# NomaDamas/AutoRAG-Research

Hardware: AMD Instinct MI355X
Metric: queries/sec (higher is better)
Workload: dtype f32

## Files before the change

autorag_research_amd/_native.py:

```python

from __future__ import annotations

import ctypes
import os
from pathlib import Path

import numpy as np

_PKG_DIR = Path(__file__).resolve().parent
LIB_PATH = _PKG_DIR / "libmi355dr.so"

_lib: ctypes.CDLL | None = None

ABI_SYMBOLS = [
    "mi355dr_create", "mi355dr_destroy", "mi355dr_last_error", "mi355dr_version", "mi355dr_reserve",
    "mi355dr_add_rows", "mi355dr_add_rows_device", "mi355dr_size", "mi355dr_dim", "mi355dr_get_rows",
    "mi355dr_update_rows", "mi355dr_update_rows_device", "mi355dr_remove_rows", "mi355dr_live_rows", "mi355dr_compact",
    "mi355dr_search", "mi355dr_search_device", "mi355dr_search_device_async", "mi355dr_search_wait",
    "mi355dr_search_subset", "mi355dr_search_subset_device", "mi355dr_score_subset", "mi355dr_search_mmr", "mi355dr_search_mmr_device", "mi355dr_mmr_select", "mi355dr_merge_groups_device", "mi355dr_search_groups", "mi355dr_search_groups_device", "mi355dr_fuse_lists", "mi355dr_fuse_lists_device", "mi355dr_search_range", "mi355dr_search_range_device",
    "mi355dr_search_rows", "mi355dr_search_rows_device", "mi355dr_search_range_rows", "mi355dr_search_range_rows_device", "mi355dr_view_create", "mi355dr_add_multivec", "mi355dr_size_multivec",
    "mi355dr_search_maxsim", "mi355dr_search_maxsim_device", "mi355dr_search_maxsim_subset", "mi355dr_search_maxsim_subset_device", "mi355dr_maxsim_subset", "mi355dr_maxsim_subset_ex", "mi355dr_add_multivec_device", "mi355dr_gqr_refine", "mi355dr_gqr_refine_maxsim",
    "mi355dr_set_multivec", "mi355dr_set_multivec_device", "mi355dr_live_multivec",
    "mi355dr_add_sparse", "mi355dr_size_sparse", "mi355dr_sparse_df", "mi355dr_search_sparse", "mi355dr_search_sparse_device",
    "mi355dr_search_bm25", "mi355dr_search_bm25_device", "mi355dr_set_sparse", "mi355dr_remove_sparse", "mi355dr_live_sparse",
    "mi355dr_search_sparse_subset", "mi355dr_search_sparse_subset_device", "mi355dr_search_bm25_subset",
    "mi355dr_search_bm25_subset_device", "mi355dr_score_sparse_subset", "mi355dr_score_bm25_subset",
    "mi355dr_gqr_refine_scores", "mi355dr_merge_topk_device", "mi355dr_pack_topk_device",
    "mi355dr_merge_topk_packed_device", "mi355dr_comm_unique_id", "mi355dr_comm_init", "mi355dr_comm_world", "mi355dr_comm_count", "mi355dr_comm_init_custom",
    "mi355dr_search_sharded_device", "mi355dr_search_range_sharded_device", "mi355dr_search_rows_sharded_device",
    "mi355dr_search_range_rows_sharded_device", "mi355dr_search_mmr_sharded_device", "mi355dr_mmr_select_sharded",
    "mi355dr_search_sparse_sharded_device", "mi355dr_search_bm25_sharded_device", "mi355dr_search_sparse_subset_sharded_device",
    "mi355dr_search_bm25_subset_sharded_device", "mi355dr_score_sparse_subset_sharded", "mi355dr_score_bm25_subset_sharded",
    "mi355dr_collapse_lists", "mi355dr_collapse_lists_device", "mi355dr_search_collapsed", "mi355dr_search_collapsed_device",
    "mi355dr_search_collapsed_sharded_device",
    "mi355dr_combine_rows", "mi355dr_combine_rows_device", "mi355dr_search_examples", "mi355dr_search_examples_device",
    "mi355dr_search_feedback", "mi355dr_search_feedback_device",
    "mi355dr_set_option", "mi355dr_get_stat",
    "mi355dr_reset_stats", "mi355dr_timer_start", "mi355dr_timer_stop", "mi355dr_synchronize",
    "mi355dr_dev_alloc", "mi355dr_dev_free", "mi355dr_dev_upload", "mi355dr_dev_download",
    "mi355dr_diag_mfma_stream",
    "mi355dr_debug_screen_dense", "mi355dr_debug_screen_hits", "mi355dr_debug_screen_bound", "mi355dr_debug_i8_state", "mi355dr_debug_rescore",
    "mi355dr_debug_maxsim_pass", "mi355dr_debug_spec_m", "mi355dr_debug_spec_model",
]


ALLGATHER_FN = ctypes.CFUNCTYPE(ctypes.c_int, ctypes.c_void_p, ctypes.c_void_p, ctypes.c_size_t, ctypes.c_void_p, ctypes.c_void_p)


class FuseOpts(ctypes.Structure):

    _fields_ = [("method", ctypes.c_int), ("mode_1", ctypes.c_int), ("mode_2", ctypes.c_int), ("rrf_k", ctypes.c_int),
                ("fetch_k", ctypes.c_int), ("weight", ctypes.c_double), ("min_1", ctypes.c_double), ("min_2", ctypes.c_double)]


class NativeError(RuntimeError):

    def __init__(self, code: int, message: str):
        super().__init__(f"libmi355dr error {code}: {message}")
        self.code = code


def _preload_torch_hip_runtime() -> None:
    import importlib.util
    import sys

    if "torch" in sys.modules:
        return
    try:
        spec = importlib.util.find_spec("torch")
    except (ImportError, ValueError):
        return
    if spec is None or not spec.submodule_search_locations:
        return
    libdir = Path(list(spec.submodule_search_locations)[0]) / "lib"
    for name in ("libhsa-runtime64.so", "libamdhip64.so"):
        f = libdir / name
        if f.exists():
            try:
                ctypes.CDLL(str(f), mode=getattr(os, "RTLD_NOW", 2) | getattr(os, "RTLD_GLOBAL", 0x100))
            except OSError:
                return


def load() -> ctypes.CDLL:
    global _lib
    if _lib is not None:
        return _lib
    if not LIB_PATH.exists():
        raise ImportError(
            f"{LIB_PATH} not found: build it with `python -c 'import __graft_entry__ as g; g.build()'` "
            "(hipcc --offload-arch=gfx950).  There is no CPU fallback for the search path."
        )
    _preload_torch_hip_runtime()
    L = ctypes.CDLL(str(LIB_PATH), mode=getattr(os, "RTLD_NOW", 2))
    vp, c_int, i64 = ctypes.c_void_p, ctypes.c_int, ctypes.c_int64
    f32p, f64p = ctypes.POINTER(ctypes.c_float), ctypes.POINTER(ctypes.c_double)
    i64p, i32p = ctypes.POINTER(ctypes.c_int64), ctypes.POINTER(ctypes.c_int32)
    L.mi355dr_create.restype = c_int
    L.mi355dr_create.argtypes = [ctypes.POINTER(vp), c_int, c_int, c_int]
    L.mi355dr_destroy.restype = None
    L.mi355dr_destroy.argtypes = [vp]
    L.mi355dr_last_error.restype = ctypes.c_char_p
    L.mi355dr_last_error.argtypes = [vp]
    L.mi355dr_version.restype = c_int
    L.mi355dr_reserve.restype = c_int
    L.mi355dr_reserve.argtypes = [vp, i64]
    L.mi355dr_add_rows.restype = c_int
    L.mi355dr_add_rows.argtypes = [vp, f32p, i64]
    L.mi355dr_add_rows_device.restype = c_int
    L.mi355dr_add_rows_device.argtypes = [vp, vp, i64]
    L.mi355dr_update_rows.restype = c_int
    L.mi355dr_update_rows.argtypes = [vp, i64p, f32p, i64]
    L.mi355dr_update_rows_device.restype = c_int
    L.mi355dr_update_rows_device.argtypes = [vp, i64p, vp, i64]
    L.mi355dr_remove_rows.restype = c_int
    L.mi355dr_remove_rows.argtypes = [vp, i64p, i64]
    L.mi355dr_compact.restype = c_int
    L.mi355dr_compact.argtypes = [vp, i64p]
    L.mi355dr_live_rows.restype = i64
    L.mi355dr_live_rows.argtypes = [vp]
    L.mi355dr_size.restype = i64
    L.mi355dr_size.argtypes = [vp]
    L.mi355dr_dim.restype = c_int
    L.mi355dr_dim.argtypes = [vp]
    L.mi355dr_get_rows.restype = c_int
    L.mi355dr_get_rows.argtypes = [vp, i64, i64, f32p]
    L.mi355dr_search.restype = c_int
    L.mi355dr_search.argtypes = [vp, f32p, c_int, c_int, f64p, i64p]
    L.mi355dr_search_device.restype = c_int
    L.mi355dr_search_device.argtypes = [vp, vp, c_int, c_int, vp, vp, vp]
    L.mi355dr_search_device_async.restype = c_int
    L.mi355dr_search_device_async.argtypes = [vp, vp, c_int, c_int, vp, vp, vp, i64p]
    L.mi355dr_search_wait.restype = c_int
    L.mi355dr_search_wait.argtypes = [vp, i64]
    L.mi355dr_search_subset.restype = c_int
    L.mi355dr_search_subset.argtypes = [vp, f32p, c_int, c_int, i64p, i64, f64p, i64p]
    L.mi355dr_search_subset_device.restype = c_int
    L.mi355dr_search_subset_device.argtypes = [vp, vp, c_int, c_int, i64p, i64, vp, vp, vp]
    L.mi355dr_score_subset.restype = c_int
    L.mi355dr_score_subset.argtypes = [vp, f32p, c_int, i64p, c_int, f64p]
    L.mi355dr_search_mmr.restype = c_int
    L.mi355dr_search_mmr.argtypes = [vp, f32p, c_int, c_int, c_int, ctypes.c_double, f64p, i64p]
    L.mi355dr_search_mmr_device.restype = c_int
    L.mi355dr_search_mmr_device.argtypes = [vp, vp, c_int, c_int, c_int, ctypes.c_double, vp, vp, vp]
    L.mi355dr_mmr_select.restype = c_int
    L.mi355dr_mmr_select.argtypes = [vp, f32p, c_int, c_int, i64p, c_int, ctypes.c_double, f64p, i64p]
    L.mi355dr_merge_groups_device.restype = c_int
    L.mi355dr_merge_groups_device.argtypes = [vp, vp, vp, c_int, c_int, i32p, c_int, c_int, vp, vp, vp, vp]
    L.mi355dr_search_groups.restype = c_int
    L.mi355dr_search_groups.argtypes = [vp, f32p, i32p, c_int, c_int, c_int, f64p, i64p, i32p]
    L.mi355dr_search_groups_device.restype = c_int
    L.mi355dr_search_groups_device.argtypes = [vp, vp, i32p, c_int, c_int, c_int, vp, vp, vp, vp]
    fuse_p = ctypes.POINTER(FuseOpts)
    L.mi355dr_fuse_lists_device.restype = c_int
    L.mi355dr_fuse_lists_device.argtypes = [vp, vp, vp, c_int, vp, i64, vp, vp, c_int, vp, i64, c_int, c_int, fuse_p, vp, vp, vp, vp]
    L.mi355dr_fuse_lists.restype = c_int
    L.mi355dr_fuse_lists.argtypes = [vp, f64p, i64p, c_int, i64p, i64, f64p, i64p, c_int, i64p, i64, c_int, c_int, fuse_p, f64p, i64p, i32p]
    L.mi355dr_collapse_lists_device.restype = c_int
    L.mi355dr_collapse_lists_device.argtypes = [vp, vp, vp, c_int, c_int, vp, i64, c_int, c_int, vp, vp, vp, vp, vp, vp, vp]
    L.mi355dr_collapse_lists.restype = c_int
    L.mi355dr_collapse_lists.argtypes = [vp, f64p, i64p, c_int, c_int, i64p, i64, c_int, c_int, f64p, i64p, i64p, i32p, i32p, i32p]
    L.mi355dr_search_collapsed.restype = c_int
    L.mi355dr_search_collapsed.argtypes = [vp, f32p, c_int, c_int, c_int, i64p, i64, c_int, c_int, f64p, i64p, i64p, i32p, i32p]
    L.mi355dr_search_collapsed_device.restype = c_int
    L.mi355dr_search_collapsed_device.argtypes = [vp, vp, c_int, c_int, c_int, vp, i64, c_int, c_int, vp, vp, vp, vp, vp, vp]
    L.mi355dr_search_collapsed_sharded_device.restype = c_int
    L.mi355dr_search_collapsed_sharded_device.argtypes = list(L.mi355dr_search_collapsed_device.argtypes)
    L.mi355dr_search_range.restype = c_int
    L.mi355dr_search_range.argtypes = [vp, f32p, c_int, f64p, c_int, f64p, i64p, i64p]
    L.mi355dr_search_range_device.restype = c_int
    L.mi355dr_search_range_device.argtypes = [vp, vp, c_int, f64p, c_int, vp, vp, vp, vp]
    L.mi355dr_search_rows.restype = c_int
    L.mi355dr_search_rows.argtypes = [vp, i64p, c_int, c_int, c_int, f64p, i64p]
    L.mi355dr_search_rows_device.restype = c_int
    L.mi355dr_search_rows_device.argtypes = [vp, i64p, c_int, c_int, c_int, vp, vp, vp]
    L.mi355dr_search_range_rows.restype = c_int
    L.mi355dr_search_range_rows.argtypes = [vp, i64p, c_int, f64p, c_int, c_int, f64p, i64p, i64p]
    L.mi355dr_search_range_rows_device.restype = c_int
    L.mi355dr_search_range_rows_device.argtypes = [vp, i64p, c_int, f64p, c_int, c_int, vp, vp, vp, vp]
    dbl = ctypes.c_double
    L.mi355dr_combine_rows.restype = c_int
    L.mi355dr_combine_rows.argtypes = [vp, f32p, c_int, i64p, c_int, i64p, c_int, dbl, dbl, dbl, f32p, i32p]
    L.mi355dr_combine_rows_device.restype = c_int
    L.mi355dr_combine_rows_device.argtypes = [vp, vp, c_int, i64p, c_int, i64p, c_int, dbl, dbl, dbl, vp, vp, vp]
    L.mi355dr_search_examples.restype = c_int
    L.mi355dr_search_examples.argtypes = [vp, f32p, c_int, i64p, c_int, i64p, c_int, dbl, dbl, dbl, c_int, c_int, f64p, i64p]
    L.mi355dr_search_examples_device.restype = c_int
    L.mi355dr_search_examples_device.argtypes = [vp, vp, c_int, i64p, c_int, i64p, c_int, dbl, dbl, dbl, c_int, c_int, vp, vp, vp]
    L.mi355dr_search_feedback.restype = c_int
    L.mi355dr_search_feedback.argtypes = [vp, f32p, c_int, c_int, c_int, dbl, dbl, f64p, i64p]
    L.mi355dr_search_feedback_device.restype = c_int
    L.mi355dr_search_feedback_device.argtypes = [vp, vp, c_int, c_int, c_int, dbl, dbl, vp, vp, vp]
    L.mi355dr_view_create.restype = c_int
    L.mi355dr_view_create.argtypes = [vp, i64p, i64, i64p, i64, ctypes.POINTER(vp)]
    L.mi355dr_add_multivec.restype = c_int
    L.mi355dr_add_multivec.argtypes = [vp, f32p, i64p, i64]
    L.mi355dr_size_multivec.restype = i64
    L.mi355dr_size_multivec.argtypes = [vp]
    L.mi355dr_search_maxsim.restype = c_int
    L.mi355dr_search_maxsim.argtypes = [vp, f32p, i32p, c_int, c_int, f32p, i64p]
    L.mi355dr_search_maxsim_device.restype = c_int
    L.mi355dr_search_maxsim_device.argtypes = [vp, vp, i32p, c_int, c_int, vp, vp, vp]
    L.mi355dr_search_maxsim_subset.restype = c_int
    L.mi355dr_search_maxsim_subset.argtypes = [vp, f32p, i32p, c_int, c_int, i64p, i64, f32p, i64p]
    L.mi355dr_search_maxsim_subset_device.restype = c_int
    L.mi355dr_search_maxsim_subset_device.argtypes = [vp, vp, i32p, c_int, c_int, i64p, i64, vp, vp, vp]
    L.mi355dr_maxsim_subset.restype = c_int
    L.mi355dr_maxsim_subset.argtypes = [vp, f32p, i32p, c_int, i64p, c_int, f32p]
    L.mi355dr_maxsim_subset_ex.restype = c_int
    L.mi355dr_maxsim_subset_ex.argtypes = [vp, f32p, i32p, c_int, i64p, c_int, c_int, f32p]
    L.mi355dr_add_multivec_device.restype = c_int
    L.mi355dr_add_multivec_device.argtypes = [vp, vp, i64p, i64]
    L.mi355dr_set_multivec.restype = c_int
    L.mi355dr_set_multivec.argtypes = [vp, i64p, f32p, i64p, i64]
    L.mi355dr_set_multivec_device.restype = c_int
    L.mi355dr_set_multivec_device.argtypes = [vp, i64p, vp, i64p, i64]
    L.mi355dr_live_multivec.restype = i64
    L.mi355dr_live_multivec.argtypes = [vp]
    c_double = ctypes.c_double
    L.mi355dr_add_sparse.restype = c_int
    L.mi355dr_add_sparse.argtypes = [vp, i32p, i64p, i64]
    L.mi355dr_size_sparse.restype = i64
    L.mi355dr_size_sparse.argtypes = [vp]
    L.mi355dr_set_sparse.restype = c_int
    L.mi355dr_set_sparse.argtypes = [vp, i64p, i32p, i64p, i64]
    L.mi355dr_remove_sparse.restype = c_int
    L.mi355dr_remove_sparse.argtypes = [vp, i64p, i64]
    L.mi355dr_live_sparse.restype = i64
    L.mi355dr_live_sparse.argtypes = [vp]
    L.mi355dr_sparse_df.restype = c_int
    L.mi355dr_sparse_df.argtypes = [vp, i32p, i64, i64p]
    L.mi355dr_search_sparse.restype = c_int
    L.mi355dr_search_sparse.argtypes = [vp, i32p, f64p, i32p, c_int, c_int, c_double, c_double, f64p, i64p]
    L.mi355dr_search_sparse_device.restype = c_int
    L.mi355dr_search_sparse_device.argtypes = [vp, i32p, f64p, i32p, c_int, c_int, c_double, c_double, vp, vp, vp]
    L.mi355dr_search_bm25.restype = c_int
    L.mi355dr_search_bm25.argtypes = [vp, i32p, i32p, c_int, c_int, c_double, c_double, f64p, i64p]
    L.mi355dr_search_bm25_device.restype = c_int
    L.mi355dr_search_bm25_device.argtypes = [vp, i32p, i32p, c_int, c_int, c_double, c_double, vp, vp, vp]
    L.mi355dr_search_sparse_subset.restype = c_int
    L.mi355dr_search_sparse_subset.argtypes = [vp, i32p, f64p, i32p, c_int, c_int, c_double, c_double, i64p, i64, f64p, i64p]
    L.mi355dr_search_sparse_subset_device.restype = c_int
    L.mi355dr_search_sparse_subset_device.argtypes = [vp, i32p, f64p, i32p, c_int, c_int, c_double, c_double, i64p, i64, vp, vp, vp]
    L.mi355dr_search_bm25_subset.restype = c_int
    L.mi355dr_search_bm25_subset.argtypes = [vp, i32p, i32p, c_int, c_int, c_double, c_double, i64p, i64, f64p, i64p]
    L.mi355dr_search_bm25_subset_device.restype = c_int
    L.mi355dr_search_bm25_subset_device.argtypes = [vp, i32p, i32p, c_int, c_int, c_double, c_double, i64p, i64, vp, vp, vp]
    L.mi355dr_score_sparse_subset.restype = c_int
    L.mi355dr_score_sparse_subset.argtypes = [vp, i32p, f64p, i32p, c_int, c_double, c_double, i64p, c_int, f64p]
    L.mi355dr_score_bm25_subset.restype = c_int
    L.mi355dr_score_bm25_subset.argtypes = [vp, i32p, i32p, c_int, c_double, c_double, i64p, c_int, f64p]
    L.mi355dr_gqr_refine.restype = c_int
    L.mi355dr_gqr_refine.argtypes = [vp, f64p, c_int, i64p, c_int, f64p, c_int, c_double, c_double, c_double, f64p]
    L.mi355dr_gqr_refine_maxsim.restype = c_int
    L.mi355dr_gqr_refine_maxsim.argtypes = [vp, f64p, i32p, c_int, i64p, c_int, f64p, c_int, c_double, c_double, c_double,
                                            f64p]
    L.mi355dr_gqr_refine_scores.restype = c_int
    L.mi355dr_gqr_refine_scores.argtypes = [vp, f64p, i32p, c_int, c_int, f64p, c_int, c_double, c_double, c_double, f64p]
    L.mi355dr_merge_topk_device.restype = c_int
    L.mi355dr_merge_topk_device.argtypes = [vp, vp, vp, c_int, c_int, c_int, vp, vp, vp]
    L.mi355dr_pack_topk_device.restype = c_int
    L.mi355dr_pack_topk_device.argtypes = [vp, vp, vp, c_int, c_int, vp, vp]
    L.mi355dr_merge_topk_packed_device.restype = c_int
    L.mi355dr_merge_topk_packed_device.argtypes = [vp, vp, c_int, c_int, c_int, vp, vp, vp]
    L.mi355dr_comm_unique_id.restype = c_int
    L.mi355dr_comm_unique_id.argtypes = [vp, ctypes.c_size_t]
    L.mi355dr_comm_init.restype = c_int
    L.mi355dr_comm_init.argtypes = [vp, c_int, c_int, vp, ctypes.c_size_t]
    L.mi355dr_comm_init_custom.restype = c_int
    L.mi355dr_comm_init_custom.argtypes = [vp, c_int, c_int, ALLGATHER_FN, vp]
    L.mi355dr_comm_world.restype = c_int
    L.mi355dr_comm_world.argtypes = [vp]
    L.mi355dr_comm_count.restype = c_int
    L.mi355dr_comm_count.argtypes = [vp, ctypes.POINTER(c_int)]
    L.mi355dr_search_sharded_device.restype = c_int
    L.mi355dr_search_sharded_device.argtypes = [vp, vp, c_int, c_int, vp, vp, vp]
    L.mi355dr_search_range_sharded_device.restype = c_int
    L.mi355dr_search_range_sharded_device.argtypes = [vp, vp, c_int, f64p, c_int, vp, vp, vp, vp]
    L.mi355dr_search_rows_sharded_device.restype = c_int
    L.mi355dr_search_rows_sharded_device.argtypes = [vp, i64p, c_int, c_int, c_int, vp, vp, vp]
    L.mi355dr_search_range_rows_sharded_device.restype = c_int
    L.mi355dr_search_range_rows_sharded_device.argtypes = [vp, i64p, c_int, f64p, c_int, c_int, vp, vp, vp, vp]
    L.mi355dr_search_mmr_sharded_device.restype = c_int
    L.mi355dr_search_mmr_sharded_device.argtypes = [vp, vp, c_int, c_int, c_int, ctypes.c_double, vp, vp, vp]
    L.mi355dr_mmr_select_sharded.restype = c_int
    L.mi355dr_mmr_select_sharded.argtypes = [vp, f32p, c_int, c_int, i64p, c_int, ctypes.c_double, f64p, i64p]
    for local in ("search_sparse_device", "search_bm25_device", "search_sparse_subset_device", "search_bm25_subset_device",
                  "score_sparse_subset", "score_bm25_subset"):
        sharded = local.replace("_device", "_sharded_device") if local.endswith("_device") else local + "_sharded"
        fn = getattr(L, "mi355dr_" + sharded)
        fn.restype = c_int
        fn.argtypes = list(getattr(L, "mi355dr_" + local).argtypes)
    L.mi355dr_set_option.restype = c_int
    L.mi355dr_set_option.argtypes = [vp, ctypes.c_char_p, i64]
    L.mi355dr_get_stat.restype = c_int
    L.mi355dr_get_stat.argtypes = [vp, ctypes.c_char_p, i64p]
    L.mi355dr_reset_stats.restype = c_int
    L.mi355dr_reset_stats.argtypes = [vp]
    L.mi355dr_timer_start.restype = c_int
    L.mi355dr_timer_start.argtypes = [vp]
    L.mi355dr_timer_stop.restype = c_int
    L.mi355dr_timer_stop.argtypes = [vp, f64p]
    L.mi355dr_synchronize.restype = c_int
    L.mi355dr_synchronize.argtypes = [vp]
    L.mi355dr_dev_alloc.restype = c_int
    L.mi355dr_dev_alloc.argtypes = [vp, ctypes.c_size_t, ctypes.POINTER(vp)]
    L.mi355dr_dev_free.restype = c_int
    L.mi355dr_dev_free.argtypes = [vp, vp]
    L.mi355dr_dev_upload.restype = c_int
    L.mi355dr_dev_upload.argtypes = [vp, vp, vp, ctypes.c_size_t]
    L.mi355dr_dev_download.restype = c_int
    L.mi355dr_dev_download.argtypes = [vp, vp, vp, ctypes.c_size_t]
    L.mi355dr_debug_screen_dense.restype = c_int
    L.mi355dr_debug_screen_dense.argtypes = [vp, f32p, c_int, i64, i64, f32p]
    L.mi355dr_debug_screen_hits.restype = c_int
    L.mi355dr_debug_screen_hits.argtypes = [vp, f32p, c_int, i64, i64, f32p, c_int, ctypes.POINTER(c_int), i32p, f32p,
                                            ctypes.POINTER(c_int), ctypes.POINTER(c_int)]
    L.mi355dr_debug_screen_bound.restype = c_int
    L.mi355dr_debug_screen_bound.argtypes = [vp, f32p, c_int, f32p]
    L.mi355dr_debug_i8_state.restype = c_int
    L.mi355dr_debug_i8_state.argtypes = [vp, f32p, c_int, f32p, f32p, i64, i64, f32p, f32p]
    L.mi355dr_debug_rescore.restype = c_int
    L.mi355dr_debug_rescore.argtypes = [vp, f32p, c_int, i32p, i64p, i64, f32p, f64p]
    L.mi355dr_debug_spec_m.restype = c_int
    L.mi355dr_debug_spec_m.argtypes = [c_int]
    L.mi355dr_debug_spec_model.restype = c_int
    L.mi355dr_debug_spec_model.argtypes = [vp, f32p, c_int, c_int, f32p, f32p, f32p, ctypes.POINTER(ctypes.c_double),
                                           ctypes.POINTER(ctypes.c_int64), ctypes.POINTER(c_int), ctypes.POINTER(c_int)]
    L.mi355dr_debug_maxsim_pass.restype = c_int
    L.mi355dr_debug_maxsim_pass.argtypes = [vp, f32p, i32p, c_int, c_int, i64p, i64, c_int, ctypes.POINTER(c_int), f32p, f32p, i32p,
                                            ctypes.POINTER(c_int), f32p, ctypes.POINTER(c_int), ctypes.POINTER(c_int)]
    L.mi355dr_diag_mfma_stream.restype = c_int
    L.mi355dr_diag_mfma_stream.argtypes = [c_int, c_int, ctypes.c_double, ctypes.POINTER(ctypes.c_double)]
    _lib = L
    return L


def diag_mfma_stream(device: int, fmt: str, seconds: float) -> float:
    out = ctypes.c_double(0.0)
    rc = load().mi355dr_diag_mfma_stream(int(device), {"i8": 0, "bf16": 1}[fmt], float(seconds), ctypes.byref(out))
    if rc != 0:
        raise NativeError(rc, "mi355dr_diag_mfma_stream failed")
    return float(out.value)


def check(handle, rc: int) -> None:
    if rc != 0:
        msg = load().mi355dr_last_error(handle)
        raise NativeError(rc, msg.decode("utf-8", "replace") if msg else "")


def f32c(a) -> np.ndarray:
    return np.ascontiguousarray(a, dtype=np.float32)


def ptr(a: np.ndarray, ct):
    return a.ctypes.data_as(ctypes.POINTER(ct))
```

autorag_research_amd/csrc/index.h:

```cpp
#pragma once
#include <climits>
#include <hip/hip_runtime.h>

#include <algorithm>
#include <cmath>
#include <cstdio>
#include <cstring>
#include <mutex>
#include <string>
#include <vector>

#include "dev_common.h"
#include "mi355dr.h"

namespace mi355 {
template <class T, bool Pinned = false>
struct DevBuf {
    T* p = nullptr;
    size_t bytes = 0;
    DevBuf() = default;
    DevBuf(const DevBuf&) = delete;
    DevBuf& operator=(const DevBuf&) = delete;
    ~DevBuf() { release(); }
    void release() {
        if (p) (void)(Pinned ? hipHostFree(p) : hipFree(p));
        p = nullptr;
        bytes = 0;
    }
    hipError_t grow(size_t want) {
        if (want <= bytes) return hipSuccess;
        void* q = nullptr;
        const hipError_t e = Pinned ? hipHostMalloc(&q, want) : hipMalloc(&q, want);
        if (e != hipSuccess) return e;
        release();
        p = (T*)q;
        bytes = want;
        return hipSuccess;
    }
    void swap(DevBuf& o) {
        std::swap(p, o.p);
        std::swap(bytes, o.bytes);
    }
    operator T*() const { return p; }
};
template <class T>
using HostBuf = DevBuf<T, true>;

struct Event {
    hipEvent_t e = nullptr;
    Event() = default;
    Event(const Event&) = delete;
    Event& operator=(const Event&) = delete;
    ~Event() {
        if (e) (void)hipEventDestroy(e);
    }
    hipError_t create(unsigned flags = hipEventDefault) { return e ? hipSuccess : hipEventCreateWithFlags(&e, flags); }
    operator hipEvent_t() const { return e; }
};

struct EventPair {
    hipEvent_t a, b;
    int big;
};
struct EventPairs {
    std::vector<EventPair> v;
    ~EventPairs() {
        for (auto& p : v) {
            (void)hipEventDestroy(p.a);
            (void)hipEventDestroy(p.b);
        }
    }
};
struct MultiVecStore;
struct SparseStore;
struct Pass {
    int k = 0;
    int level = 0;
    bool screening = false;
    bool i8 = false;
    bool wide = false;
    int cap = 0;
    bool speculative = false;
    bool spec_eligible = false;
    int spec_m = 0;
    const char* refused = nullptr;
};
struct Pending {
    bool active = false;
    Event done;
    HostBuf<int> status_host;
    hipStream_t stream = nullptr;
    const float* q_dev = nullptr;
    int B = 0;
    Pass pass;
    double* out_dist = nullptr;
    int64_t* out_rows = nullptr;
};
struct RetryBufs {
    DevBuf<float> q;
    DevBuf<double> dist;
    DevBuf<int64_t> rows;
    DevBuf<int> map;
};
constexpr int kPendingRing = 4;

template <class... Bufs>
hipError_t grow_each(size_t n, Bufs&... bufs) {
    hipError_t e = hipSuccess;
    (void)(((e = bufs.grow(n * sizeof(*bufs.p))) == hipSuccess) && ...);
    return e;
}
struct MmrBufs {
    DevBuf<double> cand_dist;
    DevBuf<int64_t> cand_rows;
    DevBuf<unsigned long long> pairs_dev;
    hipError_t reserve(size_t nb, size_t stride) {
        hipError_t e = grow_each(nb * stride, cand_dist, cand_rows);
        if (!e) e = grow_each(1, pairs_dev);
        return e;
    }
};
struct GroupBufs {
    DevBuf<int32_t> offsets, count;
    DevBuf<double> cand_dist, out_dist;
    DevBuf<int64_t> cand_rows, out_rows;
    hipError_t reserve(size_t G, size_t S, size_t fetch_k, size_t k, bool host) {
        hipError_t e = grow_each(G + 1, offsets);
        if (!e) e = grow_each(S * fetch_k, cand_dist, cand_rows);
        if (!e && host) e = grow_each(G * k, out_dist, out_rows);
        if (!e && host) e = grow_each(G, count);
        return e;
    }
};
struct FuseBufs {
    DevBuf<double> vals[2], out_vals;
    DevBuf<int64_t> ids[2], map[2], out_ids;
    DevBuf<int32_t> count;
    hipError_t reserve(size_t B, const int* w, const int64_t* map_len, size_t k_out) {
        hipError_t e = hipSuccess;
        for (int l = 0; l < 2 && !e; ++l) {
            e = grow_each(B * (size_t)w[l], vals[l], ids[l]);
            if (!e) e = grow_each((size_t)map_len[l], map[l]);
        }
        if (!e) e = grow_each(B * k_out, out_vals, out_ids);
        if (!e) e = grow_each(B, count);
        return e;
    }
};
struct CollapseBufs {
    DevBuf<double> vals, out_vals, cand_dist;
    DevBuf<int64_t> ids, keys, out_ids, out_keys, cand_rows;
    DevBuf<int32_t> out_pos, count, entries, lines, kept;
    DevBuf<float> q_all, q_sub;
    hipError_t reserve_lists(size_t B, size_t w, size_t keys_len, size_t k_out) {
        hipError_t e = grow_each(B * w, vals, ids);
        if (!e) e = grow_each(keys_len, keys);
        if (!e) e = grow_each(B * k_out, out_vals, out_ids, out_keys, out_pos);
        if (!e) e = grow_each(B, count, entries);
        return e;
    }
    hipError_t reserve_search(size_t nb, size_t max_fetch, size_t k, size_t dim, size_t host_keys_len, bool host) {
        hipError_t e = grow_each(nb * max_fetch, cand_dist, cand_rows);
        if (!e) e = grow_each(nb * dim, q_sub);
        if (!e) e = grow_each(nb, lines, kept, entries);
        if (!e && host) e = grow_each(nb * dim, q_all);
        if (!e && host) e = grow_each(host_keys_len, keys);
        if (!e && host) e = grow_each(nb * k, out_keys);
        return e;
    }
    size_t bytes() const {
        return vals.bytes + out_vals.bytes + cand_dist.bytes + ids.bytes + keys.bytes + out_ids.bytes + out_keys.bytes +
               cand_rows.bytes + out_pos.bytes + count.bytes + entries.bytes + lines.bytes + kept.bytes + q_all.bytes +
               q_sub.bytes;
    }
};
struct RangeBufs {
    DevBuf<uint64_t> key, rkey;
    DevBuf<int32_t> row, xfrom;
    DevBuf<unsigned long long> count, stat;
    DevBuf<double> radius, fb_dist;
    DevBuf<int> redo, flag, fb_map;
    DevBuf<int64_t> fb_rows;
    DevBuf<float> fb_q;
    int collect_lds = 0;
    hipError_t reserve(size_t nb, size_t R, size_t m, size_t pairs, size_t dim) {
        hipError_t e = grow_each(nb * R, key, row);
        if (!e) e = grow_each(nb, count, rkey, xfrom, radius, flag, fb_map);
        if (!e) e = grow_each(2, stat);
        if (!e) e = grow_each(2 + 2 * pairs, redo);
        if (!e) e = grow_each(nb * dim, fb_q);
        if (!e) e = grow_each(nb * m, fb_dist, fb_rows);
        return e;
    }
};
struct RowQueryBufs {
    DevBuf<int64_t> ids, pair_row, cand_rows, cand_count;
    DevBuf<float> q, self_dot;
    DevBuf<int> valid;
    DevBuf<int32_t> pair_q;
    DevBuf<double> cand_dist, self_dist, radius;
    DevBuf<unsigned long long> skipped_dev;
    hipError_t reserve(size_t nb, size_t stride, size_t dim, bool range) {
        hipError_t e = grow_each(nb, ids, valid, pair_q, pair_row);
        if (!e) e = grow_each(nb * dim, q);
        if (!e) e = grow_each(nb * stride, cand_dist, cand_rows);
        if (!e) e = grow_each(1, skipped_dev);
        if (!e && range) e = grow_each(nb, cand_count, self_dot, self_dist, radius);
        return e;
    }
};
struct ExampleBufs {
    DevBuf<int64_t> pos, neg, cand_rows;
    DevBuf<float> q, base;
    DevBuf<int> valid;
    DevBuf<double> cand_dist;
    DevBuf<unsigned long long> counters;
    hipError_t reserve(size_t nb, size_t mp, size_t mn, size_t stride, size_t dim, bool own_base) {
        hipError_t e = grow_each(nb * mp, pos);
        if (!e) e = grow_each(nb * mn, neg);
        if (!e) e = grow_each(nb, valid);
        if (!e) e = grow_each(nb * dim, q);
        if (!e) e = grow_each(nb * stride, cand_dist, cand_rows);
        if (!e) e = grow_each(2, counters);
        if (!e && own_base) e = grow_each(nb * dim, base);
        return e;
    }
};
struct ShardBufs {
    DevBuf<int64_t> send, recv;
    DevBuf<float> stage, stage_all;
    DevBuf<unsigned long long> local_skipped;
};
}

struct mi355dr_index {
    int device = 0, dim = 0, dpad = 0, metric = 0;
    hipStream_t stream = nullptr;
    std::mutex mu;
    std::string err;
    mi355dr_index() = default;
    ~mi355dr_index() {
        if (stream) (void)hipStreamDestroy(stream);
    }

    int64_t n = 0, cap_rows = 0;
    mi355::DevBuf<float> rows;
    mi355::DevBuf<uint16_t> shadow;
    mi355::DevBuf<float> nrm2;
    mi355::DevBuf<int32_t> irr_rows;
    mi355::DevBuf<int> irr_count;
    int irr_n = 0;
    mi355::DevBuf<unsigned> n2max_dev;
    float cmax = 0.0f;
    mi355::DevBuf<unsigned> bf16_res2_dev;
    float bf16_ec = 0.00390625f;
    int dpad8 = 0;
    mi355::DevBuf<int8_t> shadow8;
    mi355::DevBuf<uint8_t> flag8;
    mi355::DevBuf<mi355::I8Group> grp8;
    mi355::DevBuf<int32_t> irr8_rows;
    mi355::DevBuf<int> irr8_count;
    int irr8_n = 0;
    mi355::DevBuf<int> dead_count;
    int64_t dead_n = 0;

    bool qstate_ready = false;
    mi355::QueryState st{};
    mi355::DevBuf<void> st_mem[sizeof(mi355::QueryState) / sizeof(void*)];
    mi355::DevBuf<float> qdev;
    mi355::DevBuf<int32_t> cand_row;
    mi355::DevBuf<float> cand_val;
    mi355::DevBuf<int> qlist_dev;
    int* status_or_dev = nullptr;
    mi355::HostBuf<int> status_host;
    mi355::DevBuf<double> out_dist_dev;
    mi355::DevBuf<int64_t> out_rows_dev;
    mi355::DevBuf<int64_t> out_count_dev;
    mi355::DevBuf<unsigned long long> stat_dev;
    mi355::DevBuf<int> prune_skip;
    mi355::DevBuf<int32_t> subset_ids;
    mi355::MmrBufs mmr;
    mi355::GroupBufs grp;
    mi355::FuseBufs fuse;
    mi355::CollapseBufs clp;
    mi355::RangeBufs rng;
    mi355::RowQueryBufs rowq;
    mi355::ExampleBufs exq;
    mi355::ShardBufs shd;
    bool is_view = false;
    mi355::DevBuf<int64_t> view_row_map;
    mi355::DevBuf<int64_t> view_doc_map;
    int64_t view_rows = 0, view_docs = 0;
    int prune_parity = 0;

    int path = 0;
    int screen_dtype = 0;
    int i8_backoff = 0, i8_probation = 0;
    int speculate = 1;
    int64_t spec_min_rows = (int64_t)1 << 20;
    int spec_shift_milli = 0;
    int spec_backoff = 0, spec_probation = 0;
    mi355::DevBuf<float> spec_moments;
    int i8_demoted_k = INT_MAX;
    double i8_min_budget = 0.25;
    mi355::RetryBufs retry[3];
    mi355::Pending pend[mi355::kPendingRing];
    mi355::Pending sub_pend[4];
    int64_t seq_next = 0, seq_done = 0;
    int last_pass_k = 10;
    int maxsim_coop = -1;
    int maxsim_persistent = 0;
    int maxsim_wg = -1;
    int maxsim_tighten = 1;
    int maxsim_aligned = 1;
    int maxsim_wg_min = 8;
    int maxsim_wg_pipe = 1;
    int maxsim_pack8 = -1;
    int maxsim_wg_bps = 4;
    int maxsim_pass_groups = 4;
    int maxsim_screen = 1;
    int maxsim_subset_screen = -1;
    int64_t maxsim_subset_screen_min = 512;
    int64_t row_offset = 0;
    int round_a = 0;
    int screen_rq = 1;
    int screen_stream = 1;
    int prefilter16 = 0;
    int profile = 0;
    int starter = 1;
    int prune_companion = 1;
    int scan_dma = 1;
    int defer_round_b = 1;
    int chunk0_set = 0;
    int64_t chunk0_rows = 1024;
    int64_t chunk_growth = 3;
    int chunk_growth_set = 0;
    int64_t small_chunk_rows = 16384;
    int cap = mi355::kCandCap;
    int cap_set = 0;
    int prune_wide = 1;
    int screen_flush_sync = 1, screen_flush_lanes = 48, screen_flush_alone = 40;
    int wide_inflation_x10 = 100;
    int chunk_taper_x100 = 0;
    int64_t compact_slice_rows = 65536;
    int64_t view_slice_rows = 65536;
    int64_t range_chunk_rows = (int64_t)1 << 21;
    int range_slots = mi355::kSortMax;
    int64_t shard_stage_bytes = (int64_t)256 << 20;
    int64_t starter_rows_wide = 65536;

    int64_t s_screen_launches = 0, s_screen_ns = 0, s_screen_rows = 0, s_fallback_queries = 0, s_chunks = 0,
            s_passes = 0, s_starters = 0;
    int64_t s_big_launches = 0, s_big_ns = 0, s_big_rows = 0;
    int screen_rq_split_tests = 1;
    int64_t debug_park = 0;
    mi355::DevBuf<float> park_thr;
    int screen_drift = 3;
    mi355::DevBuf<int> rq_progress;
    int rq_epoch = 0;
    int64_t s_rq_launches = 0;
    int64_t s_spec_passes = 0, s_spec_miss_queries = 0, s_spec_overflow_queries = 0;
    int64_t s_retry_queries = 0;
    int64_t s_ms_screened = 0, s_ms_candidates = 0, s_ms_fallbacks = 0;
    int64_t s_ms_screen_ns = 0, s_ms_screen_launches = 0, s_ms_exact_ns = 0, s_ms_exact_launches = 0, s_ms_pack_ns = 0;
    int64_t s_ms_packed_launches = 0;
    int64_t s_ms_packed_blocks = 0;
    int64_t s_ms_packed_built = 0;
    int64_t s_ms_set_docs = 0;
    int64_t s_ms_moved_blocks = 0;
    int64_t s_compactions = 0;
    int64_t s_compact_moved_rows = 0;
    int64_t s_subset_searches = 0;
    int64_t s_subset_rows_scored = 0;
    int64_t s_subset_rerun_queries = 0;
    int64_t s_mss_searches = 0, s_mss_docs = 0, s_mss_screened = 0, s_mss_exact = 0, s_mss_fallbacks = 0;
    int64_t s_mmr_searches = 0, s_mmr_queries = 0, s_mmr_pairs = 0;
    int64_t s_group_searches = 0, s_group_subqueries = 0, s_groups_merged = 0;
    int64_t s_fuse_calls = 0, s_fuse_queries = 0;
    int64_t s_collapse_calls = 0, s_collapse_searches = 0, s_collapse_queries = 0, s_collapse_researched = 0, s_collapse_truncated = 0;
    int64_t s_range_searches = 0, s_range_queries = 0, s_range_in_range = 0, s_range_candidates = 0, s_range_rescored = 0,
            s_range_redo_chunks = 0, s_range_fallback_queries = 0;
    int64_t s_rows_searches = 0, s_rows_queries = 0, s_rows_skipped = 0;
    int64_t s_examples_searches = 0, s_examples_queries = 0, s_examples_skipped = 0, s_examples_skipped_slots = 0,
            s_feedback_searches = 0;
    int64_t s_shard_range_searches = 0, s_shard_rows_searches = 0, s_shard_mmr_searches = 0, s_shard_gather_bytes = 0;
    int64_t s_shard_sparse_searches = 0, s_shard_sparse_scores = 0;
    int64_t s_sparse_searches = 0, s_sparse_queries = 0, s_sparse_postings_scored = 0, s_sparse_overflows = 0;
    int sparse_tile_docs = 2048;
    int sparse_cand_cap = 2048;
    int64_t sparse_subset_pairs_max = 2048;
    int64_t s_sparse_subset_searches = 0, s_sparse_subset_scores = 0, s_sparse_subset_pairs = 0, s_sparse_subset_tiles = 0;
    int sparse_overlay_max_pct = 25;
    int64_t s_sparse_full_builds = 0, s_sparse_overlay_builds = 0, s_sparse_sets = 0;
    int64_t s_ms_screen_cols = 0;
    mi355::Event ms_ev[4];
    struct MsScreenForm {
        int family = 0, ncb = 0, waves = 0, bps = 0, pipe = 0, now = 0, grid = 0, reserved = 0;
    } last_screen_form;
    mi355::EventPairs ev_pool, ev_pending;
    mi355::Event t0, t1;

    void* comm = nullptr;
    int comm_rank = 0, comm_world = 0;
    mi355dr_allgather_fn comm_custom = nullptr;
    void* comm_custom_user = nullptr;
    int64_t* comm_packed[2] = {nullptr, nullptr};
    int64_t* comm_packed_all[2] = {nullptr, nullptr};
    hipStream_t comm_stream = nullptr;
    hipEvent_t comm_done[2] = {nullptr, nullptr};
    bool comm_done_armed[2] = {false, false};
    size_t comm_cap = 0;

    mi355::MultiVecStore* mv = nullptr;
    mi355::SparseStore* sp = nullptr;
};


namespace mi355 {

int fail(mi355dr_index* idx, int code, const std::string& msg);
inline int view_refuses(mi355dr_index* idx, const char* what, bool ask_parent = false) {
    return fail(idx, MI355DR_E_INVALID, std::string(what) + (ask_parent ? ": not on a view (it is a read-only snapshot under the parent's ids) -- ask the parent index"
                                                                        : ": a view is read-only"));
}
void multivec_destroy(mi355dr_index* idx);
int multivec_reserve(mi355dr_index* idx, int64_t n_blocks, int64_t n_docs);
int64_t multivec_bytes(const mi355dr_index* idx);
void sparse_destroy(mi355dr_index* idx);
int64_t sparse_bytes(const mi355dr_index* idx);
enum { kSparseStatDocs, kSparseStatTotalLen, kSparseStatPostings, kSparseStatVocab, kSparseStatOverlayPostings, kSparseStatDeadPostings };
int64_t sparse_stat(const mi355dr_index* idx, int which);
int drain_searches(mi355dr_index* idx);
int merge_topk_reserve(mi355dr_index* idx);
int merge_topk_packed(mi355dr_index* idx, const int64_t* packed_all_dev, int world, int B, int k, double* out_dist_dev,
                      int64_t* out_rows_dev, hipStream_t stream);
void comm_destroy(mi355dr_index* idx);
int comm_all_gather(mi355dr_index* idx, const void* send_dev, void* recv_dev, size_t bytes_per_rank, hipStream_t stream);
struct MultiVecView {
    const float* tok;
    const int64_t* blk_off;
    const int64_t* blk_off_host;
    const int32_t* tok_cnt_host;
    int dpad;
    int64_t n_docs;
};
bool multivec_view(const mi355dr_index* idx, MultiVecView* out);

__host__ __device__ inline int ms_perm(int j) {
    constexpr int P[8] = {0, 4, 2, 6, 1, 5, 3, 7};
    return (j & ~7) | P[j & 7];
}

template <class T>
inline void multivec_pack_query_row(const T* src, int d, int dpad, T* dst) {
    for (int c = 0; c < dpad; ++c) {
        const int oc = ms_perm(c);
        dst[c] = oc < d ? src[oc] : T(0);
    }
}

#define HIPCHECK(idx, expr)                                                                              \
    do {                                                                                                 \
        hipError_t e__ = (expr);                                                                         \
        if (e__ != hipSuccess) {                                                                         \
            char buf__[512];                                                                             \
            snprintf(buf__, sizeof(buf__), "%s failed: %s (%s:%d)", #expr, hipGetErrorString(e__), __FILE__, \
                     __LINE__);                                                                          \
            return mi355::fail(idx, e__ == hipErrorOutOfMemory ? MI355DR_E_NOMEM : MI355DR_E_HIP, buf__); \
        }                                                                                                \
    } while (0)

#define CHECK(expr)                          \
    do {                                     \
        int rc__ = (expr);                   \
        if (rc__ != MI355DR_OK) return rc__; \
    } while (0)

inline int64_t round_up(int64_t x, int64_t m) { return (x + m - 1) / m * m; }

}
```

autorag_research_amd/csrc/mi355dr.hip:

```cpp
#include "index.h"
#include "k_prep.h"
#include "k_scan.h"
#include "k_scan_ids.h"
#include "subset_ids.h"
#include "screen_common.h"
#include "k_screen.h"
#include "k_screen256c.h"
#include "k_screen_rq.h"

#define MI355_RQ_FORMS(X) X(1) X(2) X(3) X(4) X(5) X(6)
inline bool screen_rq_has(int ksteps) { return ksteps >= 1 && ksteps <= 6; }
#include "k_screen_stream.h"
#include "k_select.h"
#include "k_prune_wide.h"
#include "k_update.h"
#include "k_compact.h"
#include "k_view.h"
#include "k_block.h"
#include "k_mmr.h"
#include "mmr_order.h"
#include "k_groups.h"
#include "k_fuse.h"
#include "k_collapse.h"
#include "collapse_plan.h"
#include "k_range.h"
#include "k_rows.h"
#include "k_combine.h"
#include "k_shard.h"

#include <functional>

using namespace mi355;

namespace {
std::mutex g_err_mu;
std::string g_err;
}

namespace mi355 {
int fail(mi355dr_index* idx, int code, const std::string& msg) {
    if (idx) idx->err = msg;
    else {
        std::lock_guard<std::mutex> g(g_err_mu);
        g_err = msg;
    }
    return code;
}
}

namespace {


int ensure_capacity(mi355dr_index* idx, int64_t want_rows) {
    if (want_rows <= idx->cap_rows) return MI355DR_OK;
    int64_t new_cap = std::max<int64_t>(want_rows, idx->cap_rows + idx->cap_rows / 2);
    new_cap = round_up(std::max<int64_t>(new_cap, kT2), kT2);
    DevBuf<float> rows, nrm2;
    DevBuf<uint16_t> shadow;
    DevBuf<int8_t> shadow8;
    DevBuf<uint8_t> flag8;
    DevBuf<I8Group> grp8;
    const size_t row_b = (size_t)idx->dim * sizeof(float), sh_b = (size_t)idx->dpad * sizeof(uint16_t), sh8_b = (size_t)idx->dpad8;
    const size_t grp_b = (size_t)(new_cap / kI8GroupRows) * sizeof(I8Group);
    HIPCHECK(idx, rows.grow(new_cap * row_b));
    HIPCHECK(idx, shadow.grow(new_cap * sh_b));
    HIPCHECK(idx, nrm2.grow(new_cap * sizeof(float)));
    HIPCHECK(idx, shadow8.grow(new_cap * sh8_b));
    HIPCHECK(idx, flag8.grow(new_cap));
    HIPCHECK(idx, grp8.grow(grp_b));
    hipStream_t s = idx->stream;
    HIPCHECK(idx, hipMemsetAsync(shadow, 0, new_cap * sh_b, s));
    HIPCHECK(idx, hipMemsetAsync(shadow8, 0, new_cap * sh8_b, s));
    HIPCHECK(idx, hipMemsetAsync(flag8, 0, new_cap, s));
    HIPCHECK(idx, hipMemsetAsync(grp8, 0, grp_b, s));
    if (idx->n > 0) {
        const size_t n = idx->n, live_grp_b = (n + kI8GroupRows - 1) / kI8GroupRows * sizeof(I8Group);
        HIPCHECK(idx, hipMemcpyAsync(rows, idx->rows, n * row_b, hipMemcpyDeviceToDevice, s));
        HIPCHECK(idx, hipMemcpyAsync(shadow, idx->shadow, n * sh_b, hipMemcpyDeviceToDevice, s));
        HIPCHECK(idx, hipMemcpyAsync(nrm2, idx->nrm2, n * sizeof(float), hipMemcpyDeviceToDevice, s));
        HIPCHECK(idx, hipMemcpyAsync(shadow8, idx->shadow8, n * sh8_b, hipMemcpyDeviceToDevice, s));
        HIPCHECK(idx, hipMemcpyAsync(flag8, idx->flag8, n, hipMemcpyDeviceToDevice, s));
        HIPCHECK(idx, hipMemcpyAsync(grp8, idx->grp8, live_grp_b, hipMemcpyDeviceToDevice, s));
    }
    HIPCHECK(idx, hipStreamSynchronize(s));
    idx->rows.swap(rows);
    idx->shadow.swap(shadow);
    idx->nrm2.swap(nrm2);
    idx->shadow8.swap(shadow8);
    idx->flag8.swap(flag8);
    idx->grp8.swap(grp8);
    idx->cap_rows = new_cap;
    return MI355DR_OK;
}

int ensure_qstate(mi355dr_index* idx) {
    if (idx->qstate_ready) return MI355DR_OK;
    const size_t B = kQBlockMax;
    auto own = [&](auto*& view, size_t bytes) {
        DevBuf<void>& mem = idx->st_mem[((char*)&view - (char*)&idx->st) / sizeof(void*)];
        const hipError_t e = mem.grow(bytes);
        view = static_cast<std::remove_reference_t<decltype(view)>>(mem.p);
        return e;
    };
    HIPCHECK(idx, own(idx->st.qn, B * sizeof(float)));
    HIPCHECK(idx, own(idx->st.qhat, B * idx->dpad * sizeof(uint16_t)));
    HIPCHECK(idx, own(idx->st.thr, B * sizeof(float)));
    HIPCHECK(idx, own(idx->st.cnt, B * sizeof(int)));
    HIPCHECK(idx, own(idx->st.best_n, B * sizeof(int)));
    HIPCHECK(idx, own(idx->st.best_key, B * kKMax * sizeof(uint64_t)));
    HIPCHECK(idx, own(idx->st.best_row, B * kKMax * sizeof(int32_t)));
    HIPCHECK(idx, own(idx->st.thr_key, B * sizeof(uint64_t)));
    HIPCHECK(idx, own(idx->st.thr_row, B * sizeof(int32_t)));
    HIPCHECK(idx, own(idx->st.status, (B + 1) * sizeof(int)));
    idx->status_or_dev = idx->st.status + B;
    HIPCHECK(idx, own(idx->st.E, B * sizeof(float)));
    HIPCHECK(idx, own(idx->st.E16, B * sizeof(float)));
    HIPCHECK(idx, own(idx->st.sc, B * sizeof(float)));
    HIPCHECK(idx, own(idx->st.kq, B * sizeof(float)));
    HIPCHECK(idx, idx->rq_progress.grow(kRqProgressWords * sizeof(int)));
    HIPCHECK(idx, hipMemset(idx->rq_progress, 0, kRqProgressWords * sizeof(int)));
    HIPCHECK(idx, own(idx->st.qhat8, B * idx->dpad8));
    HIPCHECK(idx, own(idx->st.carry, B * sizeof(int)));
    HIPCHECK(idx, own(idx->st.thr_used, B * sizeof(float)));
    HIPCHECK(idx, idx->spec_moments.grow(B * kSpecSlabsMax * 2 * sizeof(float)));
    HIPCHECK(idx, idx->qdev.grow(B * idx->dim * sizeof(float)));
    HIPCHECK(idx, idx->cand_row.grow(B * kCandCapWide * sizeof(int32_t)));
    HIPCHECK(idx, idx->cand_val.grow(B * kCandCapWide * sizeof(float)));
    HIPCHECK(idx, idx->qlist_dev.grow(2 * B * sizeof(int)));
    HIPCHECK(idx, idx->status_host.grow((B + 1) * sizeof(int)));
    HIPCHECK(idx, idx->out_dist_dev.grow(B * kKMax * sizeof(double)));
    HIPCHECK(idx, idx->out_rows_dev.grow(B * kKMax * sizeof(int64_t)));
    HIPCHECK(idx, idx->out_count_dev.grow(B * sizeof(int64_t)));
    HIPCHECK(idx, idx->prune_skip.grow((2 + 2 * B) * sizeof(int)));
    HIPCHECK(idx, idx->stat_dev.grow(2 * B * sizeof(unsigned long long)));
    HIPCHECK(idx, hipMemsetAsync(idx->stat_dev, 0, 2 * B * sizeof(unsigned long long), idx->stream));
    if (prune_lds_bytes(idx->dim, kPruneBigThreads, kPruneBigSort, 0) > 160 * 1024 || scan_lds_bytes(idx->dim, 1) > 160 * 1024)
        return fail(idx, MI355DR_E_UNSUPPORTED, "dim too large for the select kernels' LDS budget");
    HIPCHECK(idx, hipFuncSetAttribute((const void*)k_prune<kPruneBigThreads, kPruneBigSort>,
                                      hipFuncAttributeMaxDynamicSharedMemorySize,
                                      (int)prune_lds_bytes(idx->dim, kPruneBigThreads, kPruneBigSort, 0)));
    HIPCHECK(idx, hipFuncSetAttribute((const void*)k_prune<kPruneSmallThreads, kPruneSmallSort>,
                                      hipFuncAttributeMaxDynamicSharedMemorySize,
                                      (int)prune_lds_bytes(idx->dim, kPruneSmallThreads, kPruneSmallSort, idx->dpad)));
    HIPCHECK(idx, hipFuncSetAttribute((const void*)k_prune_wide<2, 32>, hipFuncAttributeMaxDynamicSharedMemorySize,
                                      (int)prune_wide_lds_bytes(idx->dim, 2)));
    {
        int per = kScanQ;
        while (per > 1 && scan_lds_bytes(idx->dim, per) > 150 * 1024) per >>= 1;
        HIPCHECK(idx, hipFuncSetAttribute((const void*)k_scan, hipFuncAttributeMaxDynamicSharedMemorySize,
                                          (int)scan_lds_bytes(idx->dim, per)));
    }
    HIPCHECK(idx, hipFuncSetAttribute((const void*)k_scan32, hipFuncAttributeMaxDynamicSharedMemorySize, kScan32Lds));
    HIPCHECK(idx, hipFuncSetAttribute((const void*)k_scan_ids, hipFuncAttributeMaxDynamicSharedMemorySize,
                                      (int)scan_ids_lds_bytes(idx->dim, kScanQ)));
    HIPCHECK(idx, hipFuncSetAttribute((const void*)k_screen<false>, hipFuncAttributeMaxDynamicSharedMemorySize, kScreenLds));
    HIPCHECK(idx, hipFuncSetAttribute((const void*)k_screen<true>, hipFuncAttributeMaxDynamicSharedMemorySize, kScreenLds));
    {
        const int stream_lds = kStreamQueryBytesMax + kStreamStages * kStreamStageBytes;
        HIPCHECK(idx, hipFuncSetAttribute((const void*)k_screen_stream<false, 32>, hipFuncAttributeMaxDynamicSharedMemorySize, stream_lds));
        HIPCHECK(idx, hipFuncSetAttribute((const void*)k_screen_stream<true, 32>, hipFuncAttributeMaxDynamicSharedMemorySize, stream_lds));
        HIPCHECK(idx, hipFuncSetAttribute((const void*)k_screen_stream<false, 64>, hipFuncAttributeMaxDynamicSharedMemorySize, stream_lds));
        HIPCHECK(idx, hipFuncSetAttribute((const void*)k_screen_stream<true, 64>, hipFuncAttributeMaxDynamicSharedMemorySize, stream_lds));
    }
    HIPCHECK(idx, hipFuncSetAttribute((const void*)k_screen256c<false>, hipFuncAttributeMaxDynamicSharedMemorySize,
                                      kScreen256Lds));
    HIPCHECK(idx, hipFuncSetAttribute((const void*)k_screen256c<true>, hipFuncAttributeMaxDynamicSharedMemorySize,
                                      kScreen256Lds));
#define MI355_RQ_ATTR(KS)                                                                                              \
    HIPCHECK(idx, hipFuncSetAttribute((const void*)k_screen_rq<KS, true, true>, hipFuncAttributeMaxDynamicSharedMemorySize, rq_lds(KS)));
    MI355_RQ_FORMS(MI355_RQ_ATTR)
#undef MI355_RQ_ATTR
    HIPCHECK(idx, hipFuncSetAttribute((const void*)k_screen_rq<6, false, true>, hipFuncAttributeMaxDynamicSharedMemorySize, rq_lds(6)));
    HIPCHECK(idx, hipFuncSetAttribute((const void*)k_merge_topk, hipFuncAttributeMaxDynamicSharedMemorySize,
                                      kSortMax * 12));
    if (mmr_lds_bytes(idx->dim, kMmrMax) > 160 * 1024)
        return fail(idx, MI355DR_E_UNSUPPORTED, "dim too large for the select kernels' LDS budget");
    HIPCHECK(idx, hipFuncSetAttribute((const void*)k_mmr_select, hipFuncAttributeMaxDynamicSharedMemorySize,
                                      (int)mmr_lds_bytes(idx->dim, kMmrMax)));
    HIPCHECK(idx, hipFuncSetAttribute((const void*)k_shard_mmr_select, hipFuncAttributeMaxDynamicSharedMemorySize,
                                      (int)mmr_lds_bytes(idx->dim, kMmrMax)));
    HIPCHECK(idx, hipFuncSetAttribute((const void*)k_merge_groups, hipFuncAttributeMaxDynamicSharedMemorySize,
                                      (int)groups_lds_bytes(kSortMax)));
    HIPCHECK(idx, hipFuncSetAttribute((const void*)k_collapse_lists, hipFuncAttributeMaxDynamicSharedMemorySize,
                                      (int)collapse_lds_bytes(kSortMax)));
    idx->qstate_ready = true;
    return MI355DR_OK;
}

inline float screen_bound(int d) {
    return (float)(std::ldexp(1.0, -7) + std::ldexp(1.0, -15) + 8.0 * d * std::ldexp(1.0, -24));
}

EventPair take_events(mi355dr_index* idx) {
    if (!idx->ev_pool.v.empty()) {
        EventPair p = idx->ev_pool.v.back();
        idx->ev_pool.v.pop_back();
        return p;
    }
    EventPair p{};
    (void)hipEventCreate(&p.a);
    (void)hipEventCreate(&p.b);
    return p;
}

void drain_events(mi355dr_index* idx) {
    std::vector<EventPair> keep;
    for (auto& p : idx->ev_pending.v) {
        if (hipEventQuery(p.b) == hipErrorNotReady) {
            keep.push_back(p);
            continue;
        }
        float ms = 0.f;
        if (hipEventElapsedTime(&ms, p.a, p.b) == hipSuccess) {
            idx->s_screen_ns += (int64_t)(ms * 1e6);
            if (p.big) idx->s_big_ns += (int64_t)(ms * 1e6);
        }
        idx->ev_pool.v.push_back(p);
    }
    idx->ev_pending.v.swap(keep);
}

constexpr double kInflationBf16 = 5.0, kInflationI8 = 16.0;
constexpr double kSmallBlockBudget = 1.6;
constexpr double kInflationI8Wide = 10.0, kInflationBf16Wide = 4.0;
inline bool wide_ok(const mi355dr_index* idx, int k) { return idx->prune_wide && k >= kWideKMin && k <= kWideKMax; }
inline double growth_budget(const mi355dr_index* idx, int k, bool i8) {
    if (wide_ok(idx, k) && idx->path != MI355DR_PATH_SCAN) {
        const int room = std::min(kWideEntries, idx->cap_set ? idx->cap : kCandCapWide);
        return 0.75 * room / ((double)k * (i8 ? idx->wide_inflation_x10 / 10.0 : kInflationBf16Wide)) - 1.0;
    }
    const int room = k < kPruneSmallSort / 2 ? kPruneSmallSort - k : idx->cap;
    return 0.6 * std::min(room, idx->cap) / ((double)k * (i8 ? kInflationI8 : kInflationBf16));
}

inline bool i8_available(const mi355dr_index* idx) { return idx->irr8_n <= kIrrCap; }
constexpr int kStarterKMax = 32;
constexpr int64_t kStarterRows = 16384;
static_assert(kStarterRows / kSlabRows <= kSpecSlabsMax, "the moment scratch holds one entry per slab of the starter's sample");
int64_t starter_sample_rows(const mi355dr_index* idx, const Pass& ps) {
    const int64_t n = idx->n;
    const int64_t rows = std::min<int64_t>(ps.wide ? idx->starter_rows_wide : kStarterRows, n / 4) / kTileM * kTileM;
    const int64_t slabs = (rows + kSlabRows - 1) / kSlabRows;
    const bool take = idx->starter && (ps.k <= kStarterKMax || ps.wide) && ps.level == 0 && idx->chunk0_set == 0 && n >= 4 * 1024 &&
                      slabs <= ps.cap && slabs >= ps.k;
    return take ? rows : 0;
}
Pass decide_pass(const mi355dr_index* idx, int k, int level, bool force_scan, const char* no_screen = nullptr) {
    Pass ps;
    ps.k = k;
    ps.level = level;
    const int path = force_scan ? (int)MI355DR_PATH_SCAN : idx->path;
    if (level > 0) ps.i8 = false;
    else if (idx->screen_dtype == MI355DR_SCREEN_I8) ps.i8 = true;
    else ps.i8 = idx->screen_dtype == MI355DR_SCREEN_AUTO && i8_available(idx) && k < idx->i8_demoted_k &&
                 growth_budget(idx, k, true) >= idx->i8_min_budget;
    const bool screen_possible = ps.i8 ? i8_available(idx) : idx->irr_n <= kIrrCap;
    ps.screening = idx->n > 0 && screen_possible && path != MI355DR_PATH_SCAN;
    ps.wide = ps.screening && wide_ok(idx, k);
    ps.cap = !idx->cap_set && ps.wide ? kCandCapWide : idx->cap;
    if (idx->screen_dtype == MI355DR_SCREEN_I8 && !i8_available(idx) && path != MI355DR_PATH_SCAN)
        ps.refused = "int8 screen unavailable: too many rows outside the residual limit";
    else if (path == MI355DR_PATH_SCREEN && !screen_possible && idx->n > 0) ps.refused = no_screen;
    ps.spec_m = spec_m_of(k);
    ps.spec_eligible = level == 0 && ps.screening && !ps.wide && ps.spec_m > 0 && idx->speculate && idx->n >= idx->spec_min_rows &&
                       kSpecInflation * ps.spec_m * 4 <= 3 * (std::min(kPruneSmallSort, ps.cap) - k) &&
                       starter_sample_rows(idx, ps) > 0;
    ps.speculative = ps.spec_eligible && idx->spec_probation <= 0;
    return ps;
}
inline bool idle_i8(const mi355dr_index* idx) { return decide_pass(idx, idx->last_pass_k, 0, false).i8; }

int launch_prune(mi355dr_index* idx, hipStream_t s, const Pass& ps, int nblocks, const int* qlist, int exact,
                 bool thr_only = false, bool one_wave_only = false, bool defer_b = false, const SpecModel* spec = nullptr) {
    PruneArgs pa{};
    if (spec) pa.spec = *spec;
    pa.thr_only = thr_only ? 1 : 0;
    pa.one_wave_only = one_wave_only ? 1 : 0;
    pa.defer_b = defer_b && idx->defer_round_b ? 1 : 0;
    pa.rows = idx->rows;
    pa.nrm2 = idx->nrm2;
    pa.q = idx->qdev;
    pa.st = idx->st;
    pa.cand_row = idx->cand_row;
    pa.cand_val = idx->cand_val;
    pa.qlist = qlist;
    pa.stat = idx->stat_dev;
    pa.cap = ps.cap;
    pa.d = idx->dim;
    pa.k = ps.k;
    pa.metric = idx->metric;
    pa.exact = exact;
    pa.flag8 = (ps.i8 && (idx->irr8_n > 0 || idx->dead_n > 0)) ? idx->flag8 : nullptr;
    pa.cscale = idx->metric == MI355DR_METRIC_IP ? idx->cmax : 1.0f;
    pa.shadow16 = (ps.i8 && idx->metric == 0 && !exact && idx->prefilter16) ? idx->shadow : nullptr;
    pa.dpad = idx->dpad;
    pa.round_a = idx->round_a;
    if (!exact && ps.wide) {
        pa.shadow16 = nullptr;
        hipLaunchKernelGGL((k_prune_wide<2, 32>), dim3(nblocks), dim3(2 * kWave), prune_wide_lds_bytes(idx->dim, 2), s, pa);
        HIPCHECK(idx, hipGetLastError());
        return MI355DR_OK;
    }
    if (pa.cap > kCandCap) return fail(idx, MI355DR_E_INTERNAL, "general-form prune on a list stride above kCandCap");
    const bool list_mode = qlist == nullptr;
    pa.skip_list = list_mode ? idx->prune_skip : nullptr;
    pa.skip_parity = list_mode ? (idx->prune_parity ^= 1) : 0;
    hipLaunchKernelGGL((k_prune<kPruneSmallThreads, kPruneSmallSort>), dim3(nblocks), dim3(kPruneSmallThreads),
                       prune_lds_bytes(idx->dim, kPruneSmallThreads, kPruneSmallSort, pa.shadow16 ? idx->dpad : 0), s, pa);
    HIPCHECK(idx, hipGetLastError());
    if (one_wave_only) return MI355DR_OK;
    hipLaunchKernelGGL((k_prune<kPruneBigThreads, kPruneBigSort>), dim3(list_mode ? std::min(nblocks, 64) : nblocks),
                       dim3(kPruneBigThreads), prune_lds_bytes(idx->dim, kPruneBigThreads, kPruneBigSort, 0), s, pa);
    HIPCHECK(idx, hipGetLastError());
    return MI355DR_OK;
}

int launch_prep(mi355dr_index* idx, hipStream_t s, int B, int Bpad, int metric, bool i8, int cnt0 = 0) {
    hipLaunchKernelGGL(k_prep_queries, dim3(Bpad), dim3(64), (size_t)idx->dim * sizeof(float), s, idx->qdev, B, idx->dim,
                       idx->dpad, metric, idx->st, idx->dpad8, i8 ? 1 : 0, idx->bf16_ec, idx->status_or_dev,
                       idx->prune_skip, cnt0, idx->metric == MI355DR_METRIC_IP ? idx->cmax : 1.0f);
    idx->prune_parity = 0;
    HIPCHECK(idx, hipGetLastError());
    return MI355DR_OK;
}

inline int screen_tile(int B) { return B > kTileN ? kT2 : kTileM; }

constexpr int kRetryLevels = 2;

enum ScreenKernel { kKernTile = 0, kKernStream = 1, kKern256c = 2, kKernRq = 3 };
inline ScreenKernel screen_kernel_for(const mi355dr_index* idx, bool i8, int B, int64_t rows, bool emit_all) {
    const int tile = (emit_all || rows <= idx->small_chunk_rows) ? kTileM : screen_tile(B);
    const int row_bytes = i8 ? idx->dpad8 : idx->dpad * 2;
    const int ksteps = row_bytes / kRowB;
    if (tile == kT2) return i8 && idx->screen_rq && screen_rq_has(ksteps) ? kKernRq : kKern256c;
    if (!emit_all && idx->screen_stream && B <= 64 && ksteps >= 1 && (B <= 32 ? 32 : 64) * row_bytes <= kStreamQueryBytesMax)
        return kKernStream;
    return kKernTile;
}

int launch_screen(mi355dr_index* idx, hipStream_t s, bool i8, int B, int64_t r0, int64_t r_end, int cap, int emit_mode,
                  int flush_mask, int moment_slabs = 0) {
    const bool emit_all = emit_mode != 0;
    const ScreenKernel kern = screen_kernel_for(idx, i8, B, r_end - r0, emit_all);
    const int tile = kern == kKern256c || kern == kKernRq ? kT2 : kTileM;
    ScreenArgs2 sa{};
    sa.status = idx->st.status;
    sa.shadow = i8 ? (const void*)idx->shadow8 : (const void*)idx->shadow;
    sa.qhat = i8 ? (const void*)idx->st.qhat8 : (const void*)idx->st.qhat;
    sa.thr = idx->st.thr;
    sa.sc = idx->st.sc;
    sa.kq = idx->st.kq;
    sa.grp = idx->grp8;
    sa.flag8 = idx->flag8;
    sa.cnt = idx->st.cnt;
    sa.cand_row = idx->cand_row;
    sa.cand_val = idx->cand_val;
    sa.row_bytes = i8 ? idx->dpad8 : idx->dpad * 2;
    sa.ksteps = sa.row_bytes / kRowB;
    sa.cap = cap;
    sa.ct0 = (int)(r0 / tile);
    sa.n_ctiles = (int)(round_up(r_end, tile) / tile) - sa.ct0;
    sa.n_qtiles = (int)(round_up(B, tile) / tile);
    sa.row_end = r_end;
    sa.row0 = r0;
    sa.emit_all = emit_mode;
    if (moment_slabs > 0) {
        sa.moments = idx->spec_moments;
        sa.moment_slabs = moment_slabs;
    }
    const int64_t grid = round_up(sa.n_ctiles, 8) * sa.n_qtiles;
    switch (kern) {
    case kKernRq: {
        sa.ct0 = (int)(r0 / kRqRows);
        sa.n_ctiles = (int)(round_up(r_end, kRqRows) / kRqRows) - sa.ct0;
        const unsigned g2 = screen_rq_grid(sa.n_ctiles, sa.n_qtiles);
        idx->s_rq_launches++;
        if (idx->debug_park > 0 && r_end - r0 >= idx->debug_park) {
            if (!idx->park_thr) {
                std::vector<float> inf(kQBlockMax, INFINITY);
                HIPCHECK(idx, idx->park_thr.grow(kQBlockMax * sizeof(float)));
                HIPCHECK(idx, hipMemcpy(idx->park_thr, inf.data(), kQBlockMax * sizeof(float), hipMemcpyHostToDevice));
            }
            sa.thr = idx->park_thr;
        }
        sa.progress = idx->rq_progress;
        sa.epoch = idx->rq_epoch = idx->rq_epoch % 4095 + 1;
        if (sa.epoch == 1) HIPCHECK(idx, hipMemsetAsync(idx->rq_progress, 0, kRqProgressWords * sizeof(int), s));
        sa.drift = idx->screen_drift;
        sa.flush_mask = flush_mask;
        sa.flush_alone = idx->screen_flush_alone;
        if (sa.ksteps == 6 && !idx->screen_rq_split_tests) {
            hipLaunchKernelGGL((k_screen_rq<6, false, true>), dim3(g2), dim3(512), rq_lds(6), s, sa);
        } else {
            switch (sa.ksteps) {
#define MI355_RQ_LAUNCH(KS) \
    case KS: hipLaunchKernelGGL((k_screen_rq<KS, true, true>), dim3(g2), dim3(512), rq_lds(KS), s, sa); break;
                MI355_RQ_FORMS(MI355_RQ_LAUNCH)
#undef MI355_RQ_LAUNCH
            }
        }
        break;
    }
    case kKern256c: {
        const unsigned g2 = screen256_grid(sa.n_ctiles, sa.n_qtiles);
        if (i8) hipLaunchKernelGGL((k_screen256c<true>), dim3(g2), dim3(512), kScreen256Lds, s, sa);
        else hipLaunchKernelGGL((k_screen256c<false>), dim3(g2), dim3(512), kScreen256Lds, s, sa);
        break;
    }
    case kKernStream: {
        const int nq = B <= 32 ? 32 : 64;
        const unsigned gs = (unsigned)std::min(sa.n_ctiles, 256);
        const size_t lds = screen_stream_lds(nq, sa.row_bytes);
        if (i8 && nq == 32) hipLaunchKernelGGL((k_screen_stream<true, 32>), dim3(gs), dim3(256), lds, s, (ScreenArgs)sa);
        else if (i8) hipLaunchKernelGGL((k_screen_stream<true, 64>), dim3(gs), dim3(256), lds, s, (ScreenArgs)sa);
        else if (nq == 32) hipLaunchKernelGGL((k_screen_stream<false, 32>), dim3(gs), dim3(256), lds, s, (ScreenArgs)sa);
        else hipLaunchKernelGGL((k_screen_stream<false, 64>), dim3(gs), dim3(256), lds, s, (ScreenArgs)sa);
        break;
    }
    case kKernTile:
        if (i8) hipLaunchKernelGGL(k_screen<true>, dim3((unsigned)grid), dim3(256), kScreenLds, s, (ScreenArgs)sa);
        else hipLaunchKernelGGL(k_screen<false>, dim3((unsigned)grid), dim3(256), kScreenLds, s, (ScreenArgs)sa);
        break;
    }
    HIPCHECK(idx, hipGetLastError());
    if (emit_mode == kEmitAll) {
        const int per_query = (int)(r_end - r0);
        hipLaunchKernelGGL(k_set_counts, dim3((B + 255) / 256), dim3(256), 0, s, idx->st.cnt, B, per_query);
        HIPCHECK(idx, hipGetLastError());
    }
    return MI355DR_OK;
}

struct PassPlan {
    int64_t sample = 0;
    std::vector<int64_t> ends;
    bool emit_all_first = false;
};
PassPlan plan_pass(const mi355dr_index* idx, const Pass& ps, int B, double growth) {
    PassPlan p;
    const int64_t n = idx->n;
    const int cap = ps.cap;
    const bool wide = ps.wide;
    const int tile = screen_tile(B);
    int64_t seen = 0;
    const int64_t starter_rows = starter_sample_rows(idx, ps);
    if (starter_rows > 0) {
        p.sample = starter_rows;
        seen = p.sample;
        if (ps.speculative) {
            p.ends.push_back(n);
            return p;
        }
    } else {
        const int64_t c0 = std::min<int64_t>(n, round_up(std::max<int64_t>(tile, std::min<int64_t>(idx->chunk0_rows, cap)), tile));
        p.emit_all_first = c0 <= cap;
        p.ends.push_back(c0);
        seen = c0;
        if (c0 >= n) return p;
    }
    const double rmax = 1.0 + growth;
    const double span = (double)n / (double)seen;
    int steps = std::max(1, (int)std::ceil(std::log(span) / std::log(rmax) - 0.15));
    const double r = std::pow(span, 1.0 / steps);
    double taper = std::max(1.0, (idx->chunk_taper_x100 > 0 ? idx->chunk_taper_x100 : (wide ? 120 : 100)) / 100.0);
    if (steps > 1 && taper > 1.0) {
        const double room = std::max(1.0, rmax * 1.25 / r);
        taper = std::min(taper, std::pow(room, 2.0 / (steps - 1)));
    } else {
        taper = 1.0;
    }
    double pos = (double)seen;
    int64_t prev = p.sample > 0 ? 0 : seen;
    for (int i = 1; i <= steps; ++i) {
        pos *= r * std::pow(taper, (steps - 1) / 2.0 - (i - 1));
        int64_t end = i == steps ? n : std::min<int64_t>(n, round_up((int64_t)pos, tile));
        if (tile == kT2 && end < n) {
            const int n_qtiles = (int)(round_up(B, kT2) / kT2);
            const int64_t round_rows = (int64_t)8 * (32 / n_qtiles) * kT2;
            const int64_t len = end - prev;
            if (len >= 2 * round_rows) end = std::min<int64_t>(n, prev + (len + round_rows / 2) / round_rows * round_rows);
        }
        if (end <= prev) continue;
        p.ends.push_back(end);
        prev = end;
        if (end >= n) break;
    }
    if (p.ends.empty() || p.ends.back() < n) p.ends.push_back(n);
    return p;
}

inline int starter_count(const PassPlan& p) { return (int)((p.sample + kSlabRows - 1) / kSlabRows); }

inline double normal_quantile(double p) {
    double lo = -40.0, hi = 40.0;
    for (int i = 0; i < 200; ++i) {
        const double mid = 0.5 * (lo + hi);
        if (0.5 * std::erfc(-mid / std::sqrt(2.0)) < p) lo = mid;
        else hi = mid;
    }
    return 0.5 * (lo + hi);
}

SpecModel spec_model(const mi355dr_index* idx, const Pass& ps, const PassPlan& plan, double* zq_out = nullptr) {
    SpecModel sm{};
    sm.moments = idx->spec_moments;
    sm.slabs = starter_count(plan);
    sm.rows = (int)plan.sample;
    const double zq = normal_quantile(1.0 - (double)ps.spec_m / (double)idx->n) + idx->spec_shift_milli / 1000.0;
    sm.zq = (float)zq;
    if (zq_out) *zq_out = zq;
    return sm;
}

PassPlan make_plan(const mi355dr_index* idx, const Pass& ps, int B) {
    const double budget = growth_budget(idx, ps.k, ps.i8);
    double growth = std::max(0.25, std::min((double)idx->chunk_growth, budget));
    if (B <= 64 && ps.level == 0 && idx->chunk_growth_set == 0) growth = std::max(growth, std::min(8.0, budget * kSmallBlockBudget));
    if (ps.level == 1) growth = std::max(0.25, growth * 0.5);
    if (ps.level >= 2) growth = 0.25;
    return plan_pass(idx, ps, B, growth);
}

int run_screen(mi355dr_index* idx, hipStream_t s, const Pass& ps, int B, const PassPlan& plan) {
    int64_t kept_all_below = 0;
    const bool i8 = ps.i8;
    const int side_n = i8 ? idx->irr8_n : idx->irr_n;
    constexpr int kSideMerge = 32;
    bool side_done = false;
    const bool lean = plan.sample > 0 && idx->prune_companion == 0;
    auto timed = [&](bool big, int64_t rows, auto&& launch) -> int {
        EventPair ev{};
        if (idx->profile) {
            ev = take_events(idx);
            HIPCHECK(idx, hipEventRecord(ev.a, s));
        }
        CHECK(launch());
        if (idx->profile) {
            HIPCHECK(idx, hipEventRecord(ev.b, s));
            ev.big = big ? 1 : 0;
            idx->ev_pending.v.push_back(ev);
        }
        idx->s_screen_launches++;
        idx->s_screen_rows += rows;
        if (big) {
            idx->s_big_launches++;
            idx->s_big_rows += rows;
        }
        return MI355DR_OK;
    };
    if (plan.sample > 0) {
        SpecModel sm{};
        if (ps.speculative) {
            sm = spec_model(idx, ps, plan);
            idx->s_spec_passes++;
        }
        CHECK(timed(false, plan.sample, [&] {
            return launch_screen(idx, s, i8, B, 0, plan.sample, ps.cap, kEmitSlabMax, -1, ps.speculative ? sm.slabs : 0);
        }));
        CHECK(launch_prune(idx, s, ps, B, nullptr, 0, true, true, false,
                           ps.speculative ? &sm : nullptr));
        idx->s_starters++;
    }
    int64_t done = 0;
    for (size_t ci = 0; ci < plan.ends.size(); ++ci) {
        const int64_t end = plan.ends[ci];
        const bool emit_all = ci == 0 && plan.emit_all_first;
        if (emit_all) kept_all_below = end;
        const bool big = !emit_all && end - done > idx->small_chunk_rows && screen_tile(B) == kT2;
        const int64_t seen = ci == 0 ? (plan.sample > 0 ? plan.sample : end) : done;
        const double lanes = ps.speculative ? (double)kSpecInflation * ps.spec_m * 4096.0 / (double)idx->n
                                            : 8.0 * ps.k * 4096.0 / (double)std::max<int64_t>(seen, 1);
        int period = 1;
        while (period < 64 && period * 2 * lanes <= idx->screen_flush_lanes) period *= 2;
        const int flush_mask = idx->screen_flush_sync ? period - 1 : -1;
        CHECK(timed(big, end - done, [&] { return launch_screen(idx, s, i8, B, done, end, ps.cap, emit_all ? kEmitAll : 0, flush_mask); }));
        idx->s_chunks++;
        if (end >= idx->n && side_n > 0 && side_n <= kSideMerge) {
            hipLaunchKernelGGL(k_emit_irregular, dim3(B), dim3(64), 0, s, i8 ? idx->irr8_rows : idx->irr_rows, side_n, idx->st,
                               idx->cand_row, idx->cand_val, ps.cap, (int)kept_all_below);
            HIPCHECK(idx, hipGetLastError());
            side_done = true;
        }
        const bool last = end >= idx->n && (side_n == 0 || side_done);
        CHECK(launch_prune(idx, s, ps, B, nullptr, 0, false, lean, !last));
        done = end;
    }
    if (side_n > 0 && !side_done) {
        hipLaunchKernelGGL(k_emit_irregular, dim3(B), dim3(64), 0, s, i8 ? idx->irr8_rows : idx->irr_rows, side_n, idx->st,
                           idx->cand_row, idx->cand_val, ps.cap, (int)kept_all_below);
        HIPCHECK(idx, hipGetLastError());
        CHECK(launch_prune(idx, s, ps, B, nullptr, 0, false, lean));
    }
    idx->s_passes++;
    return MI355DR_OK;
}

int launch_scan(mi355dr_index* idx, hipStream_t s, const int* qlist, int nq, int cap, int64_t r0, int64_t r1,
                const int32_t* ids = nullptr) {
    ScanArgs sa{};
    sa.rows = idx->rows;
    sa.nrm2 = idx->nrm2;
    sa.q = idx->qdev;
    sa.st = idx->st;
    sa.cand_row = idx->cand_row;
    sa.cand_val = idx->cand_val;
    sa.qlist = qlist;
    sa.nq = nq;
    sa.cap = cap;
    sa.d = idx->dim;
    sa.metric = idx->metric;
    sa.row0 = r0;
    sa.row1 = r1;
    const dim3 grid((unsigned)((r1 - r0 + kScanThreads - 1) / kScanThreads));
    const ScanIdsArgs ia{sa, ids};
    if (ids) hipLaunchKernelGGL(k_scan_ids, grid, dim3(kScanThreads), scan_ids_lds_bytes(idx->dim, nq), s, ia);
    else if (idx->dim % kScan32PieceCols == 0 && idx->scan_dma)
        hipLaunchKernelGGL(k_scan32, grid, dim3(kScanThreads), kScan32Lds, s, sa, idx->n);
    else hipLaunchKernelGGL(k_scan, grid, dim3(kScanThreads), scan_lds_bytes(idx->dim, nq), s, sa);
    HIPCHECK(idx, hipGetLastError());
    return MI355DR_OK;
}

int scan_range(mi355dr_index* idx, hipStream_t s, const Pass& ps, int off, int nq, int64_t r0, int64_t r1, const int32_t* ids) {
    CHECK(launch_scan(idx, s, idx->qlist_dev + off, nq, ps.cap, r0, r1, ids));
    return launch_prune(idx, s, ps, nq, idx->qlist_dev + off, 1);
}

int run_scan(mi355dr_index* idx, hipStream_t s, const Pass& ps, const std::vector<int>& qs, int64_t total,
             const int32_t* ids = nullptr) {
    if (qs.empty()) return MI355DR_OK;
    HIPCHECK(idx, hipMemcpyAsync(idx->qlist_dev, qs.data(), qs.size() * sizeof(int), hipMemcpyHostToDevice, s));
    const int nq_all = (int)qs.size(), cap = ps.cap;
    hipLaunchKernelGGL(k_reset_queries, dim3((nq_all + 255) / 256), dim3(256), 0, s, idx->st, idx->qlist_dev, nq_all);
    HIPCHECK(idx, hipGetLastError());
    const int per = kScanQ;
    for (int off = 0; off < nq_all; off += per) {
        const int nq = std::min(per, nq_all - off);
        int64_t done = 0;
        int64_t chunk = std::min<int64_t>(idx->chunk0_rows, cap);
        while (done < total) {
            const int64_t end = std::min<int64_t>(total, done + chunk);
            CHECK(scan_range(idx, s, ps, off, nq, done, end, ids));
            if (end - done > cap) {
                HIPCHECK(idx, hipMemcpyAsync(idx->status_host, idx->st.status, kQBlockMax * sizeof(int),
                                             hipMemcpyDeviceToHost, s));
                HIPCHECK(idx, hipStreamSynchronize(s));
                std::vector<int> redo;
                for (int j = 0; j < nq; ++j)
                    if (idx->status_host[qs[off + j]] & kStOverflow) redo.push_back(qs[off + j]);
                if (!redo.empty()) {
                    const int roff = kQBlockMax;
                    HIPCHECK(idx, hipMemcpyAsync(idx->qlist_dev + roff, redo.data(), redo.size() * sizeof(int),
                                                 hipMemcpyHostToDevice, s));
                    for (int q : redo) idx->status_host[q] &= ~kStOverflow;
                    for (int q : redo)
                        HIPCHECK(idx, hipMemcpyAsync(idx->st.status + q, idx->status_host + q, sizeof(int),
                                                     hipMemcpyHostToDevice, s));
                    for (int64_t p = done; p < end; p += cap)
                        CHECK(scan_range(idx, s, ps, roff, (int)redo.size(), p, std::min<int64_t>(end, p + cap), ids));
                    if (ids) {
                        HIPCHECK(idx, hipStreamSynchronize(s));
                        idx->s_subset_rerun_queries += (int64_t)redo.size();
                    }
                }
            }
            done = end;
            chunk = std::max<int64_t>(chunk, done * (idx->chunk_growth_set ? idx->chunk_growth : 63));
        }
    }
    if (ids) HIPCHECK(idx, hipStreamSynchronize(s));
    else idx->s_fallback_queries += nq_all;
    return MI355DR_OK;
}

int subset_block(mi355dr_index* idx, hipStream_t s, const float* q_dev, int B, int k, int64_t m, double* out_dist_dev,
                 int64_t* out_rows_dev) {
    const Pass ps = decide_pass(idx, k, 0, true);
    idx->last_pass_k = k;
    if (q_dev != idx->qdev)
        HIPCHECK(idx, hipMemcpyAsync(idx->qdev, q_dev, (size_t)B * idx->dim * sizeof(float), hipMemcpyDeviceToDevice, s));
    CHECK(launch_prep(idx, s, B, (int)round_up(B, screen_tile(B)), idx->metric, ps.i8));
    std::vector<int> all(B);
    for (int i = 0; i < B; ++i) all[i] = i;
    if (m > 0) CHECK(run_scan(idx, s, ps, all, m, idx->subset_ids));
    hipLaunchKernelGGL(k_finalize, dim3(B), dim3(64), 0, s, idx->st, k, idx->row_offset, idx->view_row_map.p, out_dist_dev,
                       out_rows_dev, idx->status_or_dev, -1);
    HIPCHECK(idx, hipGetLastError());
    HIPCHECK(idx, hipMemcpyAsync(idx->status_host, idx->st.status, (size_t)kQBlockMax * sizeof(int), hipMemcpyDeviceToHost, s));
    HIPCHECK(idx, hipStreamSynchronize(s));
    for (int i = 0; i < B; ++i)
        if (idx->status_host[i] & kStOverflow)
            return fail(idx, MI355DR_E_INTERNAL, "subset scan: query " + std::to_string(i) + " lost a candidate chunk");
    return MI355DR_OK;
}

int pending_alloc(mi355dr_index* idx, Pending& p) {
    HIPCHECK(idx, p.status_host.grow((kQBlockMax + 1) * sizeof(int)));
    HIPCHECK(idx, p.done.create(hipEventDisableTiming));
    return MI355DR_OK;
}

int enqueue_block(mi355dr_index* idx, hipStream_t s, const float* q_dev, int B, int k, double* out_dist_dev,
                  int64_t* out_rows_dev, Pending& p, int level = 0, bool force_scan = false) {
    CHECK(ensure_qstate(idx));
    CHECK(pending_alloc(idx, p));
    idx->last_pass_k = k;
    if (level == 0 && idx->screen_dtype == MI355DR_SCREEN_AUTO && k >= idx->i8_demoted_k && --idx->i8_probation <= 0)
        idx->i8_demoted_k = INT_MAX;
    const int Bpad = (int)round_up(B, screen_tile(B));
    const Pass ps = decide_pass(idx, k, level, force_scan, "screen path unavailable (metric or too many irregular rows)");
    if (ps.refused) return fail(idx, MI355DR_E_UNSUPPORTED, ps.refused);
    if (idx->spec_probation > 0 && ps.spec_eligible) idx->spec_probation--;
    if (q_dev != idx->qdev)
        HIPCHECK(idx, hipMemcpyAsync(idx->qdev, q_dev, (size_t)B * idx->dim * sizeof(float), hipMemcpyDeviceToDevice, s));
    PassPlan plan;
    if (ps.screening) plan = make_plan(idx, ps, B);
    CHECK(launch_prep(idx, s, B, Bpad, idx->metric, ps.i8, starter_count(plan)));
    if (idx->n > 0) {
        if (ps.screening) {
            CHECK(run_screen(idx, s, ps, B, plan));
        } else {
            std::vector<int> all(B);
            for (int i = 0; i < B; ++i) all[i] = i;
            CHECK(run_scan(idx, s, ps, all, idx->n));
        }
    }
    hipLaunchKernelGGL(k_finalize, dim3(B), dim3(64), 0, s, idx->st, k, idx->row_offset, idx->view_row_map.p, out_dist_dev,
                       out_rows_dev, idx->status_or_dev, ps.speculative && idx->n > 0 ? idx->metric : -1);
    HIPCHECK(idx, hipGetLastError());
    HIPCHECK(idx, hipMemcpyAsync(p.status_host, idx->st.status, (size_t)(kQBlockMax + 1) * sizeof(int), hipMemcpyDeviceToHost, s));
    HIPCHECK(idx, hipEventRecord(p.done, s));
    p.active = true;
    p.stream = s;
    p.q_dev = q_dev;
    p.B = B;
    p.pass = ps;
    p.out_dist = out_dist_dev;
    p.out_rows = out_rows_dev;
    return MI355DR_OK;
}

int search_block(mi355dr_index* idx, hipStream_t s, const float* q_dev, int B, int k, double* out_dist_dev,
                 int64_t* out_rows_dev, int level = 0, bool force_scan = false);

int complete_block(mi355dr_index* idx, Pending& p) {
    if (!p.active) return MI355DR_OK;
    p.active = false;
    HIPCHECK(idx, hipEventSynchronize(p.done));
    drain_events(idx);
    if (!p.pass.screening) {
        for (int i = 0; i < p.B; ++i)
            if (p.status_host[i] & kStOverflow)
                return fail(idx, MI355DR_E_INTERNAL, "exact scan: query " + std::to_string(i) + " lost a candidate chunk");
        return MI355DR_OK;
    }
    if (p.status_host[kQBlockMax] == 0) return MI355DR_OK;
    hipStream_t s = p.stream;
    const int B = p.B, k = p.pass.k, level = p.pass.level;
    std::vector<int> sub;
    int n_todo = 0;
    {
        std::vector<int> retry;
        for (int i = 0; i < B; ++i) {
            const int st = p.status_host[i];
            if (st == 0) continue;
            if (p.pass.speculative && !(st & kStIrregular)) {
                if (st & kStOverflow) idx->s_spec_overflow_queries++;
                else if (st & kStSpecMiss) idx->s_spec_miss_queries++;
            }
            if (level < kRetryLevels && !(st & kStIrregular)) retry.push_back(i);
            else sub.push_back(i);
        }
        n_todo = (int)sub.size();
        sub.insert(sub.end(), retry.begin(), retry.end());
    }
    const int n_sub = (int)sub.size(), n_retry = n_sub - n_todo;
    if (n_sub == 0) return MI355DR_OK;
    RetryBufs& rb = idx->retry[level];
    HIPCHECK(idx, rb.q.grow((size_t)kQBlockMax * idx->dim * sizeof(float)));
    HIPCHECK(idx, rb.dist.grow((size_t)kQBlockMax * kKMax * sizeof(double)));
    HIPCHECK(idx, rb.rows.grow((size_t)kQBlockMax * kKMax * sizeof(int64_t)));
    HIPCHECK(idx, rb.map.grow((size_t)kQBlockMax * sizeof(int)));
    HIPCHECK(idx, hipMemcpyAsync(rb.map, sub.data(), n_sub * sizeof(int), hipMemcpyHostToDevice, s));
    hipLaunchKernelGGL(k_gather_queries, dim3(n_sub), dim3(128), 0, s, p.q_dev, rb.map, idx->dim, rb.q);
    HIPCHECK(idx, hipGetLastError());
    HIPCHECK(idx, hipStreamSynchronize(s));
    if (n_todo > 0) CHECK(search_block(idx, s, rb.q, n_todo, k, rb.dist, rb.rows, level + 1, true));
    if (n_retry > 0) {
        idx->s_retry_queries += n_retry;
        if (p.pass.speculative) {
            if (n_retry * 100 > B && idx->spec_probation <= 0) {
                idx->spec_backoff = idx->spec_backoff == 0 ? 16 : std::min(idx->spec_backoff * 2, 4096);
                idx->spec_probation = idx->spec_backoff;
            }
        } else if (p.pass.i8 && idx->screen_dtype == MI355DR_SCREEN_AUTO && n_retry * 100 > B) {
            idx->i8_demoted_k = std::min(idx->i8_demoted_k, k);
            idx->i8_backoff = idx->i8_backoff == 0 ? 16 : std::min(idx->i8_backoff * 2, 4096);
            idx->i8_probation = idx->i8_backoff;
        }
        CHECK(search_block(idx, s, rb.q + (size_t)n_todo * idx->dim, n_retry, k, rb.dist + (size_t)n_todo * k,
                           rb.rows + (size_t)n_todo * k, level + 1));
    }
    hipLaunchKernelGGL(k_scatter_results, dim3(n_sub), dim3(128), 0, s, rb.dist, rb.rows, rb.map, k, p.out_dist, p.out_rows);
    HIPCHECK(idx, hipGetLastError());
    HIPCHECK(idx, hipStreamSynchronize(s));
    return MI355DR_OK;
}

int complete_until(mi355dr_index* idx, int64_t seq) {
    int rc = MI355DR_OK;
    while (idx->seq_done < seq) {
        const int r = complete_block(idx, idx->pend[idx->seq_done % kPendingRing]);
        if (rc == MI355DR_OK) rc = r;
        idx->seq_done++;
    }
    return rc;
}
int drain_pending(mi355dr_index* idx) { return complete_until(idx, idx->seq_next); }

int search_block(mi355dr_index* idx, hipStream_t s, const float* q_dev, int B, int k, double* out_dist_dev,
                 int64_t* out_rows_dev, int level, bool force_scan) {
    Pending& p = idx->sub_pend[std::min(level, kRetryLevels + 1)];
    CHECK(enqueue_block(idx, s, q_dev, B, k, out_dist_dev, out_rows_dev, p, level, force_scan));
    return complete_block(idx, p);
}

inline size_t merge_lds(int world, int k) {
    size_t np = 1;
    while (np < (size_t)world * k) np <<= 1;
    return np * 12;
}
inline int merge_threads(int world, int k) { return (int64_t)world * k <= 128 ? 64 : 256; }

int launch_merge(mi355dr_index* idx, const double* dist_all, const int64_t* rows_all, int64_t stride, int world, int B, int k,
                 double* out_dist_dev, int64_t* out_rows_dev, void* stream) {
    if (world <= 0 || B < 0 || k <= 0) return fail(idx, MI355DR_E_INVALID, "bad merge shape");
    if ((int64_t)world * k > kSortMax) return fail(idx, MI355DR_E_UNSUPPORTED, "world*k exceeds 4096");
    if (B == 0) return MI355DR_OK;
    HIPCHECK(idx, hipSetDevice(idx->device));
    CHECK(ensure_qstate(idx));
    hipStream_t s = stream ? (hipStream_t)stream : idx->stream;
    hipLaunchKernelGGL(k_merge_topk, dim3(B), dim3(merge_threads(world, k)), merge_lds(world, k), s, dist_all, rows_all, stride,
                       world, B, k, out_dist_dev, out_rows_dev);
    HIPCHECK(idx, hipGetLastError());
    return MI355DR_OK;
}

int upload_and_prep(mi355dr_index* idx, const float* queries, int B, int metric) {
    HIPCHECK(idx, hipSetDevice(idx->device));
    CHECK(drain_pending(idx));
    CHECK(ensure_qstate(idx));
    HIPCHECK(idx, hipMemcpyAsync(idx->qdev, queries, (size_t)B * idx->dim * sizeof(float), hipMemcpyHostToDevice, idx->stream));
    return launch_prep(idx, idx->stream, B, (int)round_up(B, screen_tile(B)), metric, idle_i8(idx));
}

int check_search_args(mi355dr_index* idx, const void* q, int B, int k, const void* od, const void* orow) {
    if (!idx) return fail(nullptr, MI355DR_E_INVALID, "null index");
    if (B < 0 || k <= 0) return fail(idx, MI355DR_E_INVALID, "B must be >= 0 and k > 0");
    if (k > kKMax) return fail(idx, MI355DR_E_UNSUPPORTED, "k exceeds 1024");
    if (B > 0 && (!q || !od || !orow)) return fail(idx, MI355DR_E_INVALID, "null buffer");
    return MI355DR_OK;
}

int check_radii(mi355dr_index* idx, const std::string& what, const double* radius, int B) {
    for (int b = 0; b < B; ++b)
        if (radius[b] != radius[b]) return fail(idx, MI355DR_E_INVALID, what + ": radius " + std::to_string(b) + " is NaN");
    return MI355DR_OK;
}

// ... 117 lines not shown
    mi355dr_index* idx = new mi355dr_index();
    idx->device = device_id;
    idx->dim = dim;
    idx->dpad = (int)round_up(dim, kStepK);
    idx->dpad8 = (int)round_up(dim, kRowB);
    idx->metric = metric;
    hipError_t e = hipSetDevice(device_id);
    if (e == hipSuccess) e = hipStreamCreateWithFlags(&idx->stream, hipStreamNonBlocking);
    auto zeroed = [&](auto& word) {
        if (e == hipSuccess) e = word.grow(4);
        if (e == hipSuccess) e = hipMemset(word, 0, 4);
    };
    if (e == hipSuccess) e = idx->irr_rows.grow(kIrrCap * sizeof(int32_t));
    zeroed(idx->irr_count);
    zeroed(idx->n2max_dev);
    zeroed(idx->bf16_res2_dev);
    if (e == hipSuccess) e = idx->irr8_rows.grow(kIrrCap * sizeof(int32_t));
    zeroed(idx->irr8_count);
    zeroed(idx->dead_count);
    if (e == hipSuccess) e = idx->t0.create();
    if (e == hipSuccess) e = idx->t1.create();
    if (e != hipSuccess) {
        std::string m = std::string("device setup failed: ") + hipGetErrorString(e);
        delete idx;
        return fail(nullptr, MI355DR_E_HIP, m);
    }
    *out = idx;
    return MI355DR_OK;
}

void mi355dr_destroy(mi355dr_index* idx) {
    if (!idx) return;
    (void)hipSetDevice(idx->device);
    (void)drain_pending(idx);
    if (idx->stream) (void)hipStreamSynchronize(idx->stream);
    multivec_destroy(idx);
    sparse_destroy(idx);
    comm_destroy(idx);
    delete idx;
}

int mi355dr_reserve(mi355dr_index* idx, int64_t n_rows) {
    if (!idx) return fail(nullptr, MI355DR_E_INVALID, "null index");
    std::lock_guard<std::mutex> g(idx->mu);
    if (idx->is_view) return view_refuses(idx, "reserve");
    HIPCHECK(idx, hipSetDevice(idx->device));
    if (n_rows < 0) return fail(idx, MI355DR_E_INVALID, "negative row count");
    if (n_rows >= (int64_t)1 << 31) return fail(idx, MI355DR_E_UNSUPPORTED, "more than 2^31-1 rows per index");
    CHECK(drain_pending(idx));
    return ensure_capacity(idx, n_rows);
}

namespace {
constexpr int64_t kBuildSlice = (int64_t)1 << 22;

int build_rows(mi355dr_index* idx, hipStream_t s, int64_t first, int64_t n, const int64_t* ids, bool with_nrm2) {
    for (int64_t r0 = 0; r0 < n; r0 += kBuildSlice) {
        const int64_t m = std::min(kBuildSlice, n - r0), row0 = ids ? 0 : first + r0;
        const int64_t* slice = ids ? ids + r0 : nullptr;
        if (with_nrm2) {
            hipLaunchKernelGGL(k_row_nrm2, dim3((unsigned)((m + kWave - 1) / kWave)), dim3(kWave), 0, s, idx->rows, row0, m,
                               idx->dim, idx->nrm2, idx->n2max_dev, slice);
            HIPCHECK(idx, hipGetLastError());
        }
        hipLaunchKernelGGL(k_build_shadow, dim3((unsigned)m), dim3(256), 0, s, idx->rows, idx->nrm2, row0, m, idx->dim,
                           idx->dpad, idx->shadow, idx->irr_rows, idx->irr_count, idx->bf16_res2_dev,
                           idx->metric == MI355DR_METRIC_IP ? 1 : 0, slice);
        HIPCHECK(idx, hipGetLastError());
    }
    return MI355DR_OK;
}

int build_groups(mi355dr_index* idx, hipStream_t s, int64_t g_first, int64_t n, const int64_t* groups, int64_t n_total,
                 int64_t first_new) {
    for (int64_t g0 = 0; g0 < n; g0 += kBuildSlice) {
        const int64_t m = std::min(kBuildSlice, n - g0);
        hipLaunchKernelGGL(k_build_shadow8, dim3((unsigned)m), dim3(256), 0, s, idx->rows, idx->nrm2, groups ? 0 : g_first + g0,
                           n_total, first_new, idx->dim, idx->dpad8, idx->shadow8, idx->flag8, idx->grp8, idx->irr8_rows,
                           idx->irr8_count, idx->metric == MI355DR_METRIC_IP ? 1 : 0, groups ? groups + g0 : nullptr);
        HIPCHECK(idx, hipGetLastError());
    }
    return MI355DR_OK;
}

int commit_corpus(mi355dr_index* idx, hipStream_t s, bool mutated) {
    int irr = 0, irr8 = 0, dead = 0;
    float res2 = 0.0f, n2max = 0.0f;
    HIPCHECK(idx, hipMemcpyAsync(&irr, idx->irr_count, sizeof(int), hipMemcpyDeviceToHost, s));
    HIPCHECK(idx, hipMemcpyAsync(&irr8, idx->irr8_count, sizeof(int), hipMemcpyDeviceToHost, s));
    if (mutated) HIPCHECK(idx, hipMemcpyAsync(&dead, idx->dead_count, sizeof(int), hipMemcpyDeviceToHost, s));
    HIPCHECK(idx, hipMemcpyAsync(&res2, idx->bf16_res2_dev, sizeof(float), hipMemcpyDeviceToHost, s));
    HIPCHECK(idx, hipMemcpyAsync(&n2max, idx->n2max_dev, sizeof(float), hipMemcpyDeviceToHost, s));
    HIPCHECK(idx, hipStreamSynchronize(s));
    idx->cmax = std::sqrt(n2max) * 1.000001f;
    idx->bf16_ec = std::min(std::sqrt(res2) * 1.001f, 0.00390625f * 1.0001f * (idx->metric == MI355DR_METRIC_IP ? idx->cmax : 1.0f));
    idx->irr_n = irr;
    idx->irr8_n = irr8;
    if (mutated) idx->dead_n = dead;
    return MI355DR_OK;
}
}

static int add_rows_impl(mi355dr_index* idx, const float* rows, int64_t n, hipMemcpyKind kind) {
    if (!idx) return fail(nullptr, MI355DR_E_INVALID, "null index");
    std::lock_guard<std::mutex> g(idx->mu);
    if (idx->is_view) return view_refuses(idx, "add_rows");
    if (n < 0) return fail(idx, MI355DR_E_INVALID, "negative row count");
    if (n == 0) return MI355DR_OK;
    if (!rows) return fail(idx, MI355DR_E_INVALID, "rows is null");
    if (idx->n + n >= (int64_t)1 << 31) return fail(idx, MI355DR_E_UNSUPPORTED, "more than 2^31-1 rows per index");
    HIPCHECK(idx, hipSetDevice(idx->device));
    CHECK(drain_pending(idx));
    CHECK(ensure_capacity(idx, idx->n + n));
    hipStream_t s = idx->stream;
    HIPCHECK(idx, hipMemcpyAsync(idx->rows + idx->n * idx->dim, rows, (size_t)n * idx->dim * sizeof(float), kind, s));
    CHECK(build_rows(idx, s, idx->n, n, nullptr, true));
    const int64_t g_lo = idx->n / kI8GroupRows, g_hi = (idx->n + n + kI8GroupRows - 1) / kI8GroupRows;
    CHECK(build_groups(idx, s, g_lo, g_hi - g_lo, nullptr, idx->n + n, idx->n));
    CHECK(commit_corpus(idx, s, false));
    idx->n += n;
    return MI355DR_OK;
}

int mi355dr_add_rows(mi355dr_index* idx, const float* rows, int64_t n) {
    return add_rows_impl(idx, rows, n, hipMemcpyHostToDevice);
}
int mi355dr_add_rows_device(mi355dr_index* idx, const float* rows_dev, int64_t n) {
    return add_rows_impl(idx, rows_dev, n, hipMemcpyDeviceToDevice);
}

namespace {
constexpr int64_t kMutSlice = (int64_t)1 << 16;

int mutate_rows_impl(mi355dr_index* idx, const int64_t* row_ids, const float* rows, int64_t n, hipMemcpyKind kind, bool remove) {
    if (!idx) return fail(nullptr, MI355DR_E_INVALID, "null index");
    std::lock_guard<std::mutex> g(idx->mu);
    if (idx->is_view) return view_refuses(idx, remove ? "remove_rows" : "update_rows");
    if (n < 0) return fail(idx, MI355DR_E_INVALID, "negative row count");
    if (n == 0) {
        HIPCHECK(idx, hipSetDevice(idx->device));
        return drain_pending(idx);
    }
    if (!row_ids || (!remove && !rows)) return fail(idx, MI355DR_E_INVALID, "null argument");
    std::vector<int64_t> sorted(row_ids, row_ids + n);
    std::sort(sorted.begin(), sorted.end());
    if (sorted.front() < 0 || sorted.back() >= idx->n) return fail(idx, MI355DR_E_INVALID, "row id out of range");
    for (int64_t i = 1; i < n; ++i)
        if (sorted[i] == sorted[i - 1]) return fail(idx, MI355DR_E_INVALID, "duplicated row id " + std::to_string(sorted[i]));
    std::vector<int64_t> groups;
    for (int64_t r : sorted)
        if (groups.empty() || groups.back() != r / kI8GroupRows) groups.push_back(r / kI8GroupRows);
    HIPCHECK(idx, hipSetDevice(idx->device));
    CHECK(drain_pending(idx));
    hipStream_t s = idx->stream;
    DevBuf<void> ids_dev, groups_dev, stage;
    HIPCHECK(idx, ids_dev.grow((size_t)n * sizeof(int64_t)));
    HIPCHECK(idx, groups_dev.grow(groups.size() * sizeof(int64_t)));
    HIPCHECK(idx, hipMemcpyAsync(ids_dev.p, row_ids, (size_t)n * sizeof(int64_t), hipMemcpyHostToDevice, s));
    HIPCHECK(idx, hipMemcpyAsync(groups_dev.p, groups.data(), groups.size() * sizeof(int64_t), hipMemcpyHostToDevice, s));
    if (!remove && kind == hipMemcpyHostToDevice)
        HIPCHECK(idx, stage.grow((size_t)std::min(n, kMutSlice) * idx->dim * sizeof(float)));
    for (int64_t r0 = 0; r0 < n; r0 += kMutSlice) {
        const int64_t m = std::min(kMutSlice, n - r0);
        const int64_t* ids = (const int64_t*)ids_dev.p + r0;
        if (remove) {
            hipLaunchKernelGGL(k_mark_dead, dim3((unsigned)((m + 255) / 256)), dim3(256), 0, s, ids, m, idx->nrm2);
            HIPCHECK(idx, hipGetLastError());
        } else {
            const float* src = rows + r0 * idx->dim;
            if (stage.p) {
                HIPCHECK(idx, hipMemcpyAsync(stage.p, src, (size_t)m * idx->dim * sizeof(float), hipMemcpyHostToDevice, s));
                src = (const float*)stage.p;
            }
            const int vec4 = idx->dim % 4 == 0 && (uintptr_t)src % 16 == 0;
            hipLaunchKernelGGL(k_update_rows, dim3((unsigned)m), dim3(256), 0, s, src, ids, m, idx->dim, vec4, idx->rows);
            HIPCHECK(idx, hipGetLastError());
        }
        CHECK(build_rows(idx, s, 0, m, ids, !remove));
    }
    CHECK(build_groups(idx, s, 0, (int64_t)groups.size(), (const int64_t*)groups_dev.p, idx->n, idx->n));
    HIPCHECK(idx, hipMemsetAsync(idx->irr_count, 0, sizeof(int), s));
    HIPCHECK(idx, hipMemsetAsync(idx->irr8_count, 0, sizeof(int), s));
    HIPCHECK(idx, hipMemsetAsync(idx->dead_count, 0, sizeof(int), s));
    hipLaunchKernelGGL(k_rebuild_side_lists, dim3((unsigned)((idx->n + 255) / 256)), dim3(256), 0, s, idx->nrm2, idx->flag8,
                       (int64_t)0, idx->n, idx->irr_rows, idx->irr_count, idx->irr8_rows, idx->irr8_count, idx->dead_count);
    HIPCHECK(idx, hipGetLastError());
    return commit_corpus(idx, s, true);
}
}

int mi355dr_update_rows(mi355dr_index* idx, const int64_t* row_ids, const float* rows, int64_t n) {
    return mutate_rows_impl(idx, row_ids, rows, n, hipMemcpyHostToDevice, false);
}
int mi355dr_update_rows_device(mi355dr_index* idx, const int64_t* row_ids, const float* rows_dev, int64_t n) {
    return mutate_rows_impl(idx, row_ids, rows_dev, n, hipMemcpyDeviceToDevice, false);
}
int mi355dr_remove_rows(mi355dr_index* idx, const int64_t* row_ids, int64_t n) {
    return mutate_rows_impl(idx, row_ids, nullptr, n, hipMemcpyHostToDevice, true);
}

int mi355dr_compact(mi355dr_index* idx, int64_t* new_of_old) {
    if (!idx) return fail(nullptr, MI355DR_E_INVALID, "null index");
    std::lock_guard<std::mutex> g(idx->mu);
    if (idx->is_view) return view_refuses(idx, "compact");
    HIPCHECK(idx, hipSetDevice(idx->device));
    CHECK(drain_pending(idx));
    const int64_t n_old = idx->n;
    if (idx->dead_n == 0) {
        if (new_of_old)
            for (int64_t r = 0; r < n_old; ++r) new_of_old[r] = r;
        return MI355DR_OK;
    }
    hipStream_t s = idx->stream;
    std::vector<float> n2;
    std::vector<int32_t> src_of_dst;
    int64_t first_dead = n_old;
    try {
        n2.resize((size_t)n_old);
        HIPCHECK(idx, hipMemcpyAsync(n2.data(), idx->nrm2, (size_t)n_old * sizeof(float), hipMemcpyDeviceToHost, s));
        HIPCHECK(idx, hipStreamSynchronize(s));
        for (int64_t r = 0; r < n_old; ++r)
            if (row_is_dead(n2[(size_t)r])) {
                first_dead = r;
                break;
            }
        src_of_dst.reserve((size_t)(n_old - first_dead));
        for (int64_t r = first_dead; r < n_old; ++r)
            if (!row_is_dead(n2[(size_t)r])) src_of_dst.push_back((int32_t)r);
    } catch (const std::bad_alloc&) {
        return fail(idx, MI355DR_E_NOMEM, "compact: out of host memory for the row maps");
    }
    const int64_t n_moved = (int64_t)src_of_dst.size(), n_new = first_dead + n_moved;
    const int64_t slice = std::min(idx->compact_slice_rows, n_moved);
    const size_t row_b = (size_t)idx->dim * sizeof(float);
    DevBuf<int32_t> map_dev;
    DevBuf<float> stage;
    if (n_moved > 0) {
        HIPCHECK(idx, map_dev.grow((size_t)n_moved * sizeof(int32_t)));
        HIPCHECK(idx, stage.grow((size_t)slice * (row_b + sizeof(float))));
        HIPCHECK(idx, hipMemcpyAsync(map_dev.p, src_of_dst.data(), (size_t)n_moved * sizeof(int32_t), hipMemcpyHostToDevice, s));
    }
    float* stage_n2 = stage.p + slice * idx->dim;
    const int vec4 = idx->dim % 4 == 0 && (uintptr_t)idx->rows.p % 16 == 0 && (uintptr_t)stage.p % 16 == 0;
    for (int64_t j0 = 0; j0 < n_moved; j0 += slice) {
        const int64_t m = std::min(slice, n_moved - j0), dst0 = first_dead + j0;
        hipLaunchKernelGGL(k_compact_gather, dim3((unsigned)((m + kCompactWaves - 1) / kCompactWaves)), dim3(64 * kCompactWaves),
                           0, s, idx->rows, idx->nrm2, map_dev.p + j0, m, idx->dim, vec4, stage.p, stage_n2);
        HIPCHECK(idx, hipGetLastError());
        HIPCHECK(idx, hipMemcpyAsync(idx->rows + dst0 * idx->dim, stage.p, (size_t)m * row_b, hipMemcpyDeviceToDevice, s));
        HIPCHECK(idx, hipMemcpyAsync(idx->nrm2 + dst0, stage_n2, (size_t)m * sizeof(float), hipMemcpyDeviceToDevice, s));
    }
    const int64_t tail_end = std::min(round_up(n_old, kT2), idx->cap_rows), tail = tail_end - n_new;
    const int64_t g_tail = (n_new + kI8GroupRows - 1) / kI8GroupRows, g_end = tail_end / kI8GroupRows;
    if (tail > 0) {
        HIPCHECK(idx, hipMemsetAsync(idx->nrm2 + n_new, 0, (size_t)tail * sizeof(float), s));
        HIPCHECK(idx, hipMemsetAsync(idx->shadow + n_new * idx->dpad, 0, (size_t)tail * idx->dpad * sizeof(uint16_t), s));
        HIPCHECK(idx, hipMemsetAsync(idx->shadow8 + n_new * idx->dpad8, 0, (size_t)tail * idx->dpad8, s));
        HIPCHECK(idx, hipMemsetAsync(idx->flag8 + n_new, 0, (size_t)tail, s));
    }
    if (g_end > g_tail) HIPCHECK(idx, hipMemsetAsync(idx->grp8 + g_tail, 0, (size_t)(g_end - g_tail) * sizeof(I8Group), s));
    CHECK(build_rows(idx, s, first_dead, n_moved, nullptr, false));
    const int64_t g_lo = first_dead / kI8GroupRows;
    CHECK(build_groups(idx, s, g_lo, g_tail - g_lo, nullptr, n_new, n_new));
    HIPCHECK(idx, hipMemsetAsync(idx->irr_count, 0, sizeof(int), s));
    HIPCHECK(idx, hipMemsetAsync(idx->irr8_count, 0, sizeof(int), s));
    HIPCHECK(idx, hipMemsetAsync(idx->dead_count, 0, sizeof(int), s));
    if (n_new > 0) {
        hipLaunchKernelGGL(k_rebuild_side_lists, dim3((unsigned)((n_new + 255) / 256)), dim3(256), 0, s, idx->nrm2, idx->flag8,
                           (int64_t)0, n_new, idx->irr_rows, idx->irr_count, idx->irr8_rows, idx->irr8_count, idx->dead_count);
        HIPCHECK(idx, hipGetLastError());
    }
    CHECK(commit_corpus(idx, s, true));
    idx->n = n_new;
    idx->i8_demoted_k = INT_MAX;
    idx->i8_backoff = idx->i8_probation = 0;
    idx->spec_backoff = idx->spec_probation = 0;
    idx->s_compactions += n_moved > 0;
    idx->s_compact_moved_rows += n_moved;
    if (new_of_old) {
        int64_t next = 0;
        for (int64_t r = 0; r < n_old; ++r) new_of_old[r] = row_is_dead(n2[(size_t)r]) ? -1 : next++;
    }
    return MI355DR_OK;
}

namespace {
#define VIEWCHECK(parent, view, expr)                                                         \
    do {                                                                                      \
        int rc__ = (expr);                                                                    \
        if (rc__ != MI355DR_OK) return fail(parent, rc__, "view_create: " + (view)->err);     \
    } while (0)

int view_local_ids(mi355dr_index* parent, const int64_t* ids, int64_t m, int64_t n, std::vector<int32_t>& out) {
    try {
        subset_prepare_ids(ids, m, parent->row_offset, n, out);
    } catch (const std::bad_alloc&) {
        return fail(parent, MI355DR_E_NOMEM, "view_create: out of host memory for the id list");
    }
    return MI355DR_OK;
}

int view_upload_map(mi355dr_index* parent, const std::vector<int32_t>& local, DevBuf<int64_t>& map) {
    if (local.empty()) return MI355DR_OK;
    std::vector<int64_t> global;
    try {
        global.resize(local.size());
    } catch (const std::bad_alloc&) {
        return fail(parent, MI355DR_E_NOMEM, "view_create: out of host memory for the id map");
    }
    for (size_t j = 0; j < local.size(); ++j) global[j] = (int64_t)local[j] + parent->row_offset;
    HIPCHECK(parent, map.grow(global.size() * sizeof(int64_t)));
    HIPCHECK(parent, hipMemcpy(map.p, global.data(), global.size() * sizeof(int64_t), hipMemcpyHostToDevice));
    return MI355DR_OK;
}

int view_build(mi355dr_index* parent, mi355dr_index* view, const int64_t* row_ids, int64_t m_rows, const int64_t* doc_ids,
               int64_t m_docs) {
    hipStream_t s = parent->stream;
    const int d = parent->dim;
    const size_t row_b = (size_t)d * sizeof(float);
    const int64_t slice = parent->view_slice_rows;
    std::vector<int32_t> rows, docs;
    CHECK(view_local_ids(parent, row_ids, m_rows, parent->n, rows));
    DevBuf<int32_t> ids_dev;
    if (!rows.empty()) {
        HIPCHECK(parent, ids_dev.grow(rows.size() * sizeof(int32_t)));
        HIPCHECK(parent, hipMemcpyAsync(ids_dev.p, rows.data(), rows.size() * sizeof(int32_t), hipMemcpyHostToDevice, s));
        HIPCHECK(parent, hipStreamSynchronize(s));
    }
    if (!rows.empty() && parent->dead_n > 0) {
        const int64_t m = (int64_t)rows.size();
        DevBuf<float> n2_dev;
        std::vector<float> n2;
        try {
            n2.resize((size_t)m);
        } catch (const std::bad_alloc&) {
            return fail(parent, MI355DR_E_NOMEM, "view_create: out of host memory for the listed rows' norms");
        }
        HIPCHECK(parent, n2_dev.grow((size_t)m * sizeof(float)));
        hipLaunchKernelGGL(k_view_gather_nrm2, dim3((unsigned)((m + 255) / 256)), dim3(256), 0, s, parent->nrm2.p, ids_dev.p, m, n2_dev.p);
        HIPCHECK(parent, hipGetLastError());
        HIPCHECK(parent, hipMemcpyAsync(n2.data(), n2_dev.p, (size_t)m * sizeof(float), hipMemcpyDeviceToHost, s));
        HIPCHECK(parent, hipStreamSynchronize(s));
        int64_t keep = 0;
        for (int64_t j = 0; j < m; ++j)
            if (!row_is_dead(n2[(size_t)j])) rows[(size_t)keep++] = rows[(size_t)j];
        if (keep < m) {
            rows.resize((size_t)keep);
            if (keep > 0) {
                HIPCHECK(parent, hipMemcpyAsync(ids_dev.p, rows.data(), (size_t)keep * sizeof(int32_t), hipMemcpyHostToDevice, s));
                HIPCHECK(parent, hipStreamSynchronize(s));
            }
        }
    }
    MultiVecView pv{};
    if (m_docs > 0 && multivec_view(parent, &pv)) {
        CHECK(view_local_ids(parent, doc_ids, m_docs, pv.n_docs, docs));
        docs.erase(std::remove_if(docs.begin(), docs.end(), [&](int32_t i) { return pv.tok_cnt_host[i] <= 0; }), docs.end());
    }
    const int64_t n_rows = (int64_t)rows.size(), n_docs = (int64_t)docs.size();
    int64_t tok_total = 0, tok_longest = 0, blk_total = 0;
    for (int32_t i : docs) {
        const int64_t T = pv.tok_cnt_host[i];
        tok_total += T;
        tok_longest = std::max(tok_longest, T);
        blk_total += (T + kMsBlkRows - 1) / kMsBlkRows;
    }
    const int64_t stage_rows = std::max(std::min(slice, n_rows), std::max(std::min(slice, tok_total), tok_longest));
    DevBuf<float> stage;
    if (stage_rows > 0) HIPCHECK(parent, stage.grow((size_t)stage_rows * row_b));
    if (n_rows > 0) {
        VIEWCHECK(parent, view, mi355dr_reserve(view, n_rows));
        const int vec4 = d % 4 == 0 && (uintptr_t)parent->rows.p % 16 == 0 && (uintptr_t)stage.p % 16 == 0;
        for (int64_t j0 = 0; j0 < n_rows; j0 += slice) {
            const int64_t m = std::min(slice, n_rows - j0);
            hipLaunchKernelGGL(k_view_gather_rows, dim3((unsigned)((m + kViewWaves - 1) / kViewWaves)), dim3(64 * kViewWaves), 0, s,
                               parent->rows.p, ids_dev.p + j0, m, d, vec4, stage.p);
            HIPCHECK(parent, hipGetLastError());
            HIPCHECK(parent, hipStreamSynchronize(s));
            VIEWCHECK(parent, view, mi355dr_add_rows_device(view, stage.p, m));
        }
        CHECK(view_upload_map(parent, rows, view->view_row_map));
    }
    if (n_docs > 0) {
        VIEWCHECK(parent, view, multivec_reserve(view, blk_total, n_docs));
        std::vector<ViewTokBlock> blocks;
        std::vector<int64_t> offsets;
        DevBuf<ViewTokBlock> blocks_dev;
        for (int64_t i0 = 0, i1; i0 < n_docs; i0 = i1) {
            blocks.clear();
            offsets.assign(1, 0);
            try {
                for (i1 = i0; i1 < n_docs && (i1 == i0 || offsets.back() + pv.tok_cnt_host[docs[(size_t)i1]] <= slice); ++i1) {
                    const int64_t T = pv.tok_cnt_host[docs[(size_t)i1]], blk0 = pv.blk_off_host[docs[(size_t)i1]];
                    for (int64_t t = 0; t < T; t += kMsBlkRows)
                        blocks.push_back(ViewTokBlock{blk0 + t / kMsBlkRows, offsets.back() + t, (int32_t)std::min<int64_t>(kMsBlkRows, T - t), 0});
                    offsets.push_back(offsets.back() + T);
                }
            } catch (const std::bad_alloc&) {
                return fail(parent, MI355DR_E_NOMEM, "view_create: out of host memory for a slice's block table");
            }
            HIPCHECK(parent, blocks_dev.grow(blocks.size() * sizeof(ViewTokBlock)));
            HIPCHECK(parent, hipMemcpyAsync(blocks_dev.p, blocks.data(), blocks.size() * sizeof(ViewTokBlock), hipMemcpyHostToDevice, s));
            hipLaunchKernelGGL(k_view_gather_toks, dim3((unsigned)blocks.size()), dim3(64 * kViewWaves), 0, s, pv.tok, blocks_dev.p, d,
                               pv.dpad, stage.p);
            HIPCHECK(parent, hipGetLastError());
            HIPCHECK(parent, hipStreamSynchronize(s));
            VIEWCHECK(parent, view, mi355dr_add_multivec_device(view, stage.p, offsets.data(), i1 - i0));
        }
        CHECK(view_upload_map(parent, docs, view->view_doc_map));
    }
    view->view_rows = n_rows;
    view->view_docs = n_docs;
    return MI355DR_OK;
}
}

int mi355dr_view_create(mi355dr_index* parent, const int64_t* row_ids, int64_t m_rows, const int64_t* doc_ids, int64_t m_docs,
                        mi355dr_index** out_view) {
    if (out_view) *out_view = nullptr;
    if (!parent) return fail(nullptr, MI355DR_E_INVALID, "null index");
    if (!out_view) return fail(parent, MI355DR_E_INVALID, "view_create: out_view is null");
    if (m_rows < 0 || m_docs < 0 || (m_rows > 0 && !row_ids) || (m_docs > 0 && !doc_ids))
        return fail(parent, MI355DR_E_INVALID, "view_create: counts must be >= 0 and a list with a count not null");
    std::lock_guard<std::mutex> g(parent->mu);
    if (parent->is_view) return view_refuses(parent, "view_create", true);
    HIPCHECK(parent, hipSetDevice(parent->device));
    CHECK(drain_pending(parent));
    mi355dr_index* view = nullptr;
// ... 1518 lines not shown
    std::vector<int32_t> pq;
    std::vector<int64_t> pr, first, ordered_rows, mine, all;
    std::vector<double> got, ordered_dist;
    std::vector<MmrCand> list;
    PairBufs bufs;
    for (int b0 = 0; b0 < B && m > 0; b0 += kQBlockMax) {
        const int nb = std::min(kQBlockMax, B - b0);
        const size_t plane = (size_t)nb * m;
        try {
            pr.clear();
            first.assign(1, 0);
            for (int b = 0; b < nb; ++b) {
                mmr_unique_rows(cand_rows + (int64_t)(b0 + b) * m, m, idx->row_offset, idx->n, pr);
                first.push_back((int64_t)pr.size());
            }
            pq.resize(pr.size());
            for (int b = 0; b < nb; ++b) std::fill(pq.begin() + first[b], pq.begin() + first[b + 1], b);
            got.resize(pr.size());
            mine.assign(2 * plane, -1);
            all.resize(2 * plane * world);
            ordered_dist.assign(plane, (double)NAN);
            ordered_rows.assign(plane, -1);
        } catch (const std::bad_alloc&) {
            return fail(idx, MI355DR_E_NOMEM, "mmr_select_sharded: out of host memory for the candidate lists");
        }
        CHECK(shard_reserve_words(idx, 2 * plane));
        const int64_t n_pairs = (int64_t)pr.size();
        if (n_pairs > 0)
            CHECK(rescore_host_pairs(idx, bufs, queries + (int64_t)b0 * idx->dim, nb, pq.data(), pr.data(), n_pairs, nullptr, got.data()));
        for (int b = 0; b < nb; ++b)
            for (int64_t i = first[b]; i < first[b + 1]; ++i) {
                const size_t at = (size_t)b * m + (size_t)(i - first[b]);
                mine[at] = pr[i] + idx->row_offset;
                memcpy(&mine[plane + at], &got[i], sizeof(double));
            }
        HIPCHECK(idx, hipMemcpyAsync(idx->shd.send.p, mine.data(), 2 * plane * sizeof(int64_t), hipMemcpyHostToDevice, s));
        CHECK(shard_gather(idx, s, idx->shd.send.p, idx->shd.recv.p, 2 * plane * sizeof(int64_t)));
        HIPCHECK(idx, hipMemcpyAsync(all.data(), idx->shd.recv.p, 2 * plane * world * sizeof(int64_t), hipMemcpyDeviceToHost, s));
        HIPCHECK(idx, hipStreamSynchronize(s));
        try {
            for (int b = 0; b < nb; ++b) {
                list.clear();
                for (int r = 0; r < world; ++r) {
                    const int64_t* rr = all.data() + (size_t)r * 2 * plane + (size_t)b * m;
                    for (int j = 0; j < m && (int)list.size() < m; ++j) {
                        if (rr[j] < 0) continue;
                        double dist;
                        memcpy(&dist, rr + plane + j, sizeof(double));
                        list.push_back(MmrCand{dist, rr[j]});
                    }
                }
                mmr_order(list.data(), (int64_t)list.size());
                for (size_t j = 0; j < list.size(); ++j) {
                    ordered_dist[(size_t)b * m + j] = list[j].dist;
                    ordered_rows[(size_t)b * m + j] = list[j].row;
                }
            }
        } catch (const std::bad_alloc&) {
            return fail(idx, MI355DR_E_NOMEM, "mmr_select_sharded: out of host memory for the candidate lists");
        }
        HIPCHECK(idx, hipMemcpyAsync(idx->mmr.cand_dist.p, ordered_dist.data(), plane * sizeof(double), hipMemcpyHostToDevice, s));
        HIPCHECK(idx, hipMemcpyAsync(idx->mmr.cand_rows.p, ordered_rows.data(), plane * sizeof(int64_t), hipMemcpyHostToDevice, s));
        const BlockOut<int64_t> o = block_outputs(idx, io, b0);
        CHECK(shard_mmr_block(idx, s, nb, m, k, lambda, o.dist, o.rows));
        CHECK(block_return(idx, io, b0, nb, o));
        HIPCHECK(idx, hipStreamSynchronize(s));
    }
    HIPCHECK(idx, hipStreamSynchronize(s));
    return shard_mmr_finish(idx, B);
}

int mi355dr_merge_topk_device(mi355dr_index* idx, const double* dist_all_dev, const int64_t* rows_all_dev, int world,
                              int B, int k, double* out_dist_dev, int64_t* out_rows_dev, void* stream) {
    if (!idx) return fail(nullptr, MI355DR_E_INVALID, "null index");
    std::lock_guard<std::mutex> g(idx->mu);
    return launch_merge(idx, dist_all_dev, rows_all_dev, (int64_t)B * k, world, B, k, out_dist_dev, out_rows_dev, stream);
}

int mi355dr_pack_topk_device(mi355dr_index* idx, const double* dist_dev, const int64_t* rows_dev, int B, int k,
                             int64_t* packed_dev, void* stream) {
    if (!idx || !dist_dev || !rows_dev || !packed_dev) return fail(idx, MI355DR_E_INVALID, "null argument");
    std::lock_guard<std::mutex> g(idx->mu);
    if (B < 0 || k <= 0) return fail(idx, MI355DR_E_INVALID, "bad shape");
    HIPCHECK(idx, hipSetDevice(idx->device));
    hipStream_t s = stream ? (hipStream_t)stream : idx->stream;
    const size_t bytes = (size_t)B * k * 8;
    if (bytes) {
        HIPCHECK(idx, hipMemcpyAsync(packed_dev, dist_dev, bytes, hipMemcpyDeviceToDevice, s));
        HIPCHECK(idx, hipMemcpyAsync(packed_dev + (size_t)B * k, rows_dev, bytes, hipMemcpyDeviceToDevice, s));
    }
    return MI355DR_OK;
}

int mi355dr_merge_topk_packed_device(mi355dr_index* idx, const int64_t* packed_all_dev, int world, int B, int k,
                                     double* out_dist_dev, int64_t* out_rows_dev, void* stream) {
    if (!idx) return fail(nullptr, MI355DR_E_INVALID, "null index");
    std::lock_guard<std::mutex> g(idx->mu);
    return merge_topk_packed(idx, packed_all_dev, world, B, k, out_dist_dev, out_rows_dev, (hipStream_t)stream);
}

namespace {
using Index = mi355dr_index;

struct Field {
    int Index::*i = nullptr;
    int64_t Index::*l = nullptr;
    double Index::*x100 = nullptr;
    bool is_switch = false;
    constexpr Field(int Index::*p, bool is_switch = false) : i(p), is_switch(is_switch) {}
    constexpr Field(int64_t Index::*p) : l(p) {}
    constexpr Field(double Index::*p) : x100(p) {}
    void set(Index* idx, int64_t v) const {
        if (i) idx->*i = is_switch ? v != 0 : (int)v;
        else if (l) idx->*l = v;
        else idx->*x100 = (double)v / 100.0;
    }
};
constexpr bool kSwitch = true;

struct Option {
    const char* key;
    Field field;
    int64_t lo = INT64_MIN, hi = INT64_MAX;
    void (*then)(Index*) = nullptr;
    int64_t gap_lo = 0, gap_hi = 0;
};
const Option kOptions[] = {
    {"path", &Index::path, 0, 2},
    {"screen_dtype", &Index::screen_dtype, 0, 2, [](Index* x) {
         x->i8_demoted_k = INT_MAX;
         x->i8_backoff = x->i8_probation = 0;
     }},
    {"i8_min_budget_x100", &Index::i8_min_budget, 1, 1000},
    {"maxsim_screen", {&Index::maxsim_screen, kSwitch}},
    {"maxsim_coop", &Index::maxsim_coop, -1, 1},
    {"maxsim_persistent", {&Index::maxsim_persistent, kSwitch}},
    {"maxsim_wg", &Index::maxsim_wg, -1, 2},
    {"maxsim_tighten", {&Index::maxsim_tighten, kSwitch}},
    {"maxsim_aligned", {&Index::maxsim_aligned, kSwitch}},
    {"maxsim_wg_min", &Index::maxsim_wg_min, 8, 9},
    {"maxsim_wg_pipe", {&Index::maxsim_wg_pipe, kSwitch}},
    {"maxsim_pack8", &Index::maxsim_pack8, -1, 1},
    {"maxsim_wg_bps", &Index::maxsim_wg_bps, 2, 4, nullptr, 2, 4},
    {"maxsim_pass_groups", &Index::maxsim_pass_groups, 1, 4},
    {"maxsim_subset_screen", &Index::maxsim_subset_screen, -1, 1},
    {"maxsim_subset_screen_min", &Index::maxsim_subset_screen_min, 0},
    {"row_offset", &Index::row_offset},
    {"profile", {&Index::profile, kSwitch}},
    {"chunk0_rows", &Index::chunk0_rows, 1, INT64_MAX, [](Index* x) { x->chunk0_set = 1; }},
    {"starter", {&Index::starter, kSwitch}},
    {"prune_companion", {&Index::prune_companion, kSwitch}},
    {"speculate", {&Index::speculate, kSwitch}, INT64_MIN, INT64_MAX, [](Index* x) { x->spec_backoff = x->spec_probation = 0; }},
    {"spec_min_rows", &Index::spec_min_rows, 0},
    {"spec_shift_milli", &Index::spec_shift_milli, -20000, 20000},
    {"scan_dma", {&Index::scan_dma, kSwitch}},
    {"defer_round_b", {&Index::defer_round_b, kSwitch}},
    {"chunk_growth", &Index::chunk_growth, 1, INT64_MAX, [](Index* x) { x->chunk_growth_set = 1; }},
    {"screen_stream", {&Index::screen_stream, kSwitch}},
    {"screen_rq", {&Index::screen_rq, kSwitch}},
    {"debug_park_thresholds", &Index::debug_park},
    {"screen_rq_split_tests", {&Index::screen_rq_split_tests, kSwitch}},
    {"screen_drift", &Index::screen_drift, 0, 1024},
    {"small_chunk_rows", &Index::small_chunk_rows, 0},
    {"round_a", &Index::round_a, 0, 64},
    {"prefilter16", {&Index::prefilter16, kSwitch}},
    {"cand_cap", &Index::cap, 16, kCandCap, [](Index* x) { x->cap_set = 1; }},
    {"prune_wide", {&Index::prune_wide, kSwitch}},
    {"screen_flush_sync", {&Index::screen_flush_sync, kSwitch}},
    {"screen_flush_lanes", &Index::screen_flush_lanes, 1, 64},
    {"screen_flush_alone", &Index::screen_flush_alone, 8, 60},
    {"wide_inflation_x10", &Index::wide_inflation_x10, 20, 400},
    {"chunk_taper_x100", &Index::chunk_taper_x100, 0, 300, nullptr, 0, 100},
    {"starter_rows_wide", &Index::starter_rows_wide, 4096, 262144},
    {"compact_slice_rows", &Index::compact_slice_rows, 32, (int64_t)1 << 22},
    {"view_slice_rows", &Index::view_slice_rows, 32, (int64_t)1 << 22},
    {"range_chunk_rows", &Index::range_chunk_rows, 256, (int64_t)1 << 31},
    {"range_slots", &Index::range_slots, 16, kSortMax},
    {"sparse_tile_docs", &Index::sparse_tile_docs, 256, 8192},
    {"sparse_cand_cap", &Index::sparse_cand_cap, 16, 2048},
    {"sparse_overlay_max_pct", &Index::sparse_overlay_max_pct, 0, 100},
    {"sparse_subset_pairs_max", &Index::sparse_subset_pairs_max, 0, 2048},
    {"shard_stage_bytes", &Index::shard_stage_bytes, 1},
};

struct Stat {
    const char* key;
    int64_t Index::*counter;
    bool reset;
    int64_t (*value)(const Index*) = nullptr;
};
const Stat kStats[] = {
    {"screen_launches", &Index::s_screen_launches, true},
    {"screen_ns", &Index::s_screen_ns, true},
    {"screen_rows", &Index::s_screen_rows, true},
    {"screen256_launches", &Index::s_big_launches, true},
    {"screen_rq_launches", &Index::s_rq_launches, true},
    {"screen256_ns", &Index::s_big_ns, true},
    {"screen256_rows", &Index::s_big_rows, true},
    {"fallback_queries", &Index::s_fallback_queries, true},
    {"chunks", &Index::s_chunks, true},
    {"passes", &Index::s_passes, true},
    {"starters", &Index::s_starters, true},
    {"retry_queries", &Index::s_retry_queries, true},
    {"spec_passes", &Index::s_spec_passes, true},
    {"spec_miss_queries", &Index::s_spec_miss_queries, true},
    {"spec_overflow_queries", &Index::s_spec_overflow_queries, true},
    {"spec_suspended", nullptr, false, [](const Index* x) -> int64_t { return x->spec_probation > 0 ? 1 : 0; }},
    {"maxsim_screened", &Index::s_ms_screened, true},
    {"maxsim_candidates", &Index::s_ms_candidates, true},
    {"maxsim_fallbacks", &Index::s_ms_fallbacks, true},
    {"maxsim_screen_ns", &Index::s_ms_screen_ns, true},
    {"maxsim_pack_ns", &Index::s_ms_pack_ns, true},
    {"maxsim_screen_launches", &Index::s_ms_screen_launches, true},
    {"maxsim_exact_ns", &Index::s_ms_exact_ns, true},
    {"maxsim_exact_launches", &Index::s_ms_exact_launches, true},
    {"maxsim_screen_cols", &Index::s_ms_screen_cols, true},
    {"maxsim_packed_launches", &Index::s_ms_packed_launches, true},
    {"maxsim_packed_blocks", &Index::s_ms_packed_blocks, false},
    {"maxsim_packed_built", &Index::s_ms_packed_built, false},
    {"maxsim_set_docs", &Index::s_ms_set_docs, true},
    {"maxsim_moved_blocks", &Index::s_ms_moved_blocks, true},
    {"subset_searches", &Index::s_subset_searches, true},
    {"subset_rows_scored", &Index::s_subset_rows_scored, true},
    {"subset_rerun_queries", &Index::s_subset_rerun_queries, true},
    {"maxsim_subset_searches", &Index::s_mss_searches, true},
    {"maxsim_subset_docs", &Index::s_mss_docs, true},
    {"maxsim_subset_screened", &Index::s_mss_screened, true},
    {"maxsim_subset_exact", &Index::s_mss_exact, true},
    {"maxsim_subset_fallbacks", &Index::s_mss_fallbacks, true},
    {"mmr_searches", &Index::s_mmr_searches, true},
    {"mmr_queries", &Index::s_mmr_queries, true},
    {"mmr_pairs_scored", &Index::s_mmr_pairs, true},
    {"group_searches", &Index::s_group_searches, true},
    {"group_subqueries", &Index::s_group_subqueries, true},
    {"groups_merged", &Index::s_groups_merged, true},
    {"fuse_calls", &Index::s_fuse_calls, true},
    {"fuse_queries", &Index::s_fuse_queries, true},
    {"collapse_calls", &Index::s_collapse_calls, true},
    {"collapse_searches", &Index::s_collapse_searches, true},
    {"collapse_queries", &Index::s_collapse_queries, true},
    {"collapse_researched", &Index::s_collapse_researched, true},
    {"collapse_truncated", &Index::s_collapse_truncated, true},
    {"range_searches", &Index::s_range_searches, true},
    {"range_queries", &Index::s_range_queries, true},
    {"range_in_range", &Index::s_range_in_range, true},
    {"range_candidates", &Index::s_range_candidates, true},
    {"range_rescored", &Index::s_range_rescored, true},
    {"range_redo_chunks", &Index::s_range_redo_chunks, true},
    {"range_fallback_queries", &Index::s_range_fallback_queries, true},
    {"rows_searches", &Index::s_rows_searches, true},
    {"rows_queries", &Index::s_rows_queries, true},
    {"rows_skipped", &Index::s_rows_skipped, true},
    {"examples_searches", &Index::s_examples_searches, true},
    {"examples_queries", &Index::s_examples_queries, true},
    {"examples_skipped", &Index::s_examples_skipped, true},
    {"examples_skipped_slots", &Index::s_examples_skipped_slots, true},
    {"feedback_searches", &Index::s_feedback_searches, true},
    {"sharded_range_searches", &Index::s_shard_range_searches, true},
    {"sharded_rows_searches", &Index::s_shard_rows_searches, true},
    {"sharded_mmr_searches", &Index::s_shard_mmr_searches, true},
    {"shard_gather_bytes", &Index::s_shard_gather_bytes, true},
    {"sharded_sparse_searches", &Index::s_shard_sparse_searches, true},
    {"sharded_sparse_scores", &Index::s_shard_sparse_scores, true},
    {"sparse_searches", &Index::s_sparse_searches, true},
    {"sparse_queries", &Index::s_sparse_queries, true},
    {"sparse_postings_scored", &Index::s_sparse_postings_scored, true},
    {"sparse_overflows", &Index::s_sparse_overflows, true},
    {"sparse_full_builds", &Index::s_sparse_full_builds, true},
    {"sparse_overlay_builds", &Index::s_sparse_overlay_builds, true},
    {"sparse_sets", &Index::s_sparse_sets, true},
    {"sparse_subset_searches", &Index::s_sparse_subset_searches, true},
    {"sparse_subset_scores", &Index::s_sparse_subset_scores, true},
    {"sparse_subset_pairs", &Index::s_sparse_subset_pairs, true},
    {"sparse_subset_tiles", &Index::s_sparse_subset_tiles, true},
    {"sparse_overlay_postings", nullptr, false, [](const Index* x) -> int64_t { return sparse_stat(x, kSparseStatOverlayPostings); }},
    {"sparse_dead_postings", nullptr, false, [](const Index* x) -> int64_t { return sparse_stat(x, kSparseStatDeadPostings); }},
    {"sparse_docs", nullptr, false, [](const Index* x) -> int64_t { return sparse_stat(x, kSparseStatDocs); }},
    {"sparse_total_len", nullptr, false, [](const Index* x) -> int64_t { return sparse_stat(x, kSparseStatTotalLen); }},
    {"sparse_postings", nullptr, false, [](const Index* x) -> int64_t { return sparse_stat(x, kSparseStatPostings); }},
    {"sparse_vocab", nullptr, false, [](const Index* x) -> int64_t { return sparse_stat(x, kSparseStatVocab); }},
    {"compactions", &Index::s_compactions, true},
    {"compact_moved_rows", &Index::s_compact_moved_rows, true},
    {"view", nullptr, false, [](const Index* x) -> int64_t { return x->is_view ? 1 : 0; }},
    {"view_rows", &Index::view_rows, false},
    {"view_docs", &Index::view_docs, false},
    {"i8_demoted", nullptr, false, [](const Index* x) -> int64_t { return x->i8_demoted_k != INT_MAX ? 1 : 0; }},
    {"i8_demoted_k", nullptr, false, [](const Index* x) -> int64_t { return x->i8_demoted_k == INT_MAX ? 0 : x->i8_demoted_k; }},
    {"irregular_rows", nullptr, false, [](const Index* x) -> int64_t { return x->irr_n; }},
    {"loose_rows", nullptr, false, [](const Index* x) -> int64_t { return x->irr8_n; }},
    {"dead_rows", nullptr, false, [](const Index* x) -> int64_t { return x->dead_n; }},
    {"screen_dtype_active", nullptr, false, [](const Index* x) -> int64_t { return idle_i8(x) ? MI355DR_SCREEN_I8 : MI355DR_SCREEN_BF16; }},
    {"hbm_bytes_resident", nullptr, false, [](const Index* x) -> int64_t {
         return x->cap_rows * ((int64_t)x->dim * 4 + (int64_t)x->dpad * 2 + (int64_t)x->dpad8 + 5) +
                x->cap_rows / kI8GroupRows * (int64_t)sizeof(I8Group) + multivec_bytes(x) +
                (int64_t)(x->view_row_map.bytes + x->view_doc_map.bytes) +
                sparse_bytes(x) + (int64_t)x->clp.bytes();
     }},
};
}

int mi355dr_debug_spec_m(int k) { return spec_m_of(k); }

int mi355dr_set_option(mi355dr_index* idx, const char* key, int64_t value) {
    if (!idx || !key) return fail(idx, MI355DR_E_INVALID, "null argument");
    std::lock_guard<std::mutex> g(idx->mu);
    if (idx->seq_done < idx->seq_next) {
        HIPCHECK(idx, hipSetDevice(idx->device));
        CHECK(drain_pending(idx));
    }
    if (idx->is_view && strcmp(key, "row_offset") == 0) return view_refuses(idx, "option row_offset");
    for (const Option& o : kOptions) {
        if (strcmp(o.key, key) != 0) continue;
        if (value < o.lo || value > o.hi || (value > o.gap_lo && value < o.gap_hi)) {
            std::string range = o.hi == INT64_MAX ? " must be >= " + std::to_string(o.lo)
                                                  : " must be in [" + std::to_string(o.lo) + ", " + std::to_string(o.hi) + "]";
            if (o.gap_lo < o.gap_hi) range += ", not between " + std::to_string(o.gap_lo) + " and " + std::to_string(o.gap_hi);
            return fail(idx, MI355DR_E_INVALID, o.key + range);
        }
        if (strcmp(key, "sparse_tile_docs") == 0 && (value & (value - 1)) != 0)
            return fail(idx, MI355DR_E_INVALID, "sparse_tile_docs must be a power of two");
        if (strcmp(key, "sparse_subset_pairs_max") == 0 && value > idx->sparse_cand_cap)
            return fail(idx, MI355DR_E_INVALID, "sparse_subset_pairs_max must not exceed sparse_cand_cap");
        o.field.set(idx, value);
        if (o.then) o.then(idx);
        return MI355DR_OK;
    }
    return fail(idx, MI355DR_E_INVALID, std::string("unknown option: ") + key);
}

int mi355dr_get_stat(mi355dr_index* idx, const char* key, int64_t* out) {
    if (!idx || !key || !out) return fail(idx, MI355DR_E_INVALID, "null argument");
    std::lock_guard<std::mutex> g(idx->mu);
    const std::string k(key);
    if (k == "candidates" || k == "rescored") {
        unsigned long long v[2] = {0, 0};
        if (idx->stat_dev) {
            std::vector<unsigned long long> per(2 * kQBlockMax);
            HIPCHECK(idx, hipSetDevice(idx->device));
            HIPCHECK(idx, hipMemcpy(per.data(), idx->stat_dev, per.size() * sizeof(unsigned long long), hipMemcpyDeviceToHost));
            for (int i = 0; i < kQBlockMax; ++i) {
                v[0] += per[2 * i];
                v[1] += per[2 * i + 1];
            }
        }
        *out = (int64_t)(k == "candidates" ? v[0] : v[1]);
        return MI355DR_OK;
    }
    for (const Stat& st : kStats) {
        if (k != st.key) continue;
        *out = st.counter ? idx->*st.counter : st.value(idx);
        return MI355DR_OK;
    }
    return fail(idx, MI355DR_E_INVALID, "unknown stat: " + k);
}

int mi355dr_reset_stats(mi355dr_index* idx) {
    if (!idx) return fail(nullptr, MI355DR_E_INVALID, "null index");
    std::lock_guard<std::mutex> g(idx->mu);
    for (const Stat& st : kStats)
        if (st.reset) idx->*st.counter = 0;
    if (idx->stat_dev) {
        HIPCHECK(idx, hipSetDevice(idx->device));
        HIPCHECK(idx, hipMemset(idx->stat_dev, 0, 2 * kQBlockMax * sizeof(unsigned long long)));
    }
    return MI355DR_OK;
}

int mi355dr_timer_start(mi355dr_index* idx) {
    if (!idx) return fail(nullptr, MI355DR_E_INVALID, "null index");
    HIPCHECK(idx, hipSetDevice(idx->device));
    HIPCHECK(idx, hipEventRecord(idx->t0, idx->stream));
    return MI355DR_OK;
}
int mi355dr_timer_stop(mi355dr_index* idx, double* elapsed_ms) {
    if (!idx || !elapsed_ms) return fail(idx, MI355DR_E_INVALID, "null argument");
    HIPCHECK(idx, hipSetDevice(idx->device));
    HIPCHECK(idx, hipEventRecord(idx->t1, idx->stream));
    HIPCHECK(idx, hipEventSynchronize(idx->t1));
    float ms = 0.f;
    HIPCHECK(idx, hipEventElapsedTime(&ms, idx->t0, idx->t1));
    *elapsed_ms = ms;
    return MI355DR_OK;
}
int mi355dr_synchronize(mi355dr_index* idx) {
    if (!idx) return fail(nullptr, MI355DR_E_INVALID, "null index");
    HIPCHECK(idx, hipSetDevice(idx->device));
    HIPCHECK(idx, hipStreamSynchronize(idx->stream));
    return MI355DR_OK;
}

int mi355dr_dev_alloc(mi355dr_index* idx, size_t bytes, void** out) {
    if (!idx || !out) return fail(idx, MI355DR_E_INVALID, "null argument");
    HIPCHECK(idx, hipSetDevice(idx->device));
    HIPCHECK(idx, hipMalloc(out, bytes ? bytes : 1));
    return MI355DR_OK;
}
int mi355dr_dev_free(mi355dr_index* idx, void* p) {
    if (!idx) return fail(nullptr, MI355DR_E_INVALID, "null index");
    HIPCHECK(idx, hipSetDevice(idx->device));
    if (p) HIPCHECK(idx, hipFree(p));
    return MI355DR_OK;
}
int mi355dr_dev_upload(mi355dr_index* idx, void* dst_dev, const void* src_host, size_t bytes) {
    if (!idx) return fail(nullptr, MI355DR_E_INVALID, "null index");
    HIPCHECK(idx, hipSetDevice(idx->device));
    HIPCHECK(idx, hipMemcpy(dst_dev, src_host, bytes, hipMemcpyHostToDevice));
    return MI355DR_OK;
}
int mi355dr_dev_download(mi355dr_index* idx, void* dst_host, const void* src_dev, size_t bytes) {
    if (!idx) return fail(nullptr, MI355DR_E_INVALID, "null index");
    HIPCHECK(idx, hipSetDevice(idx->device));
    HIPCHECK(idx, hipMemcpy(dst_host, src_dev, bytes, hipMemcpyDeviceToHost));
    return MI355DR_OK;
}

int mi355dr_debug_screen_dense(mi355dr_index* idx, const float* queries, int B, int64_t row0, int64_t n, float* out_t) {
    if (!idx || !queries || !out_t) return fail(idx, MI355DR_E_INVALID, "null argument");
    std::lock_guard<std::mutex> g(idx->mu);
    if (B <= 0 || B > kQBlockMax || n <= 0 || n > kCandCap || row0 < 0 || row0 % screen_tile(B) != 0 || row0 + n > idx->n)
        return fail(idx, MI355DR_E_INVALID,
                    "debug_screen_dense: need 1<=B<=1024, 1<=n<=2048, row0 a multiple of the tile (128; 256 if B>128)");
    CHECK(upload_and_prep(idx, queries, B, 2));
    hipStream_t s = idx->stream;
    const bool i8 = idle_i8(idx);
    CHECK(launch_screen(idx, s, i8, B, row0, row0 + n, kCandCap, 0, -1));
    std::vector<int> cnt(B);
    std::vector<int32_t> crow((size_t)B * kCandCap);
    std::vector<float> cval((size_t)B * kCandCap);
    HIPCHECK(idx, hipMemcpyAsync(cnt.data(), idx->st.cnt, B * sizeof(int), hipMemcpyDeviceToHost, s));
    HIPCHECK(idx, hipMemcpyAsync(crow.data(), idx->cand_row, crow.size() * sizeof(int32_t), hipMemcpyDeviceToHost, s));
    HIPCHECK(idx, hipMemcpyAsync(cval.data(), idx->cand_val, cval.size() * sizeof(float), hipMemcpyDeviceToHost, s));
    std::vector<uint8_t> flag(n, 0);
    if (i8) HIPCHECK(idx, hipMemcpyAsync(flag.data(), idx->flag8 + row0, n, hipMemcpyDeviceToHost, s));
    HIPCHECK(idx, hipStreamSynchronize(s));
    for (int64_t i = 0; i < (int64_t)B * n; ++i) out_t[i] = NAN;
    for (int b = 0; b < B; ++b) {
        const int c = std::min(cnt[b], kCandCap);
        for (int j = 0; j < c; ++j) {
            const int64_t r = crow[(size_t)b * kCandCap + j] - row0;
            if (r >= 0 && r < n && !flag[r]) out_t[(int64_t)b * n + r] = cval[(size_t)b * kCandCap + j];
        }
    }
    return MI355DR_OK;
}

int mi355dr_debug_screen_hits(mi355dr_index* idx, const float* queries, int B, int64_t row0, int64_t n, const float* thr,
                              int cap, int* out_count, int32_t* out_rows, float* out_vals, int* out_status, int* out_kernel) {
    if (!idx || !queries || !thr || !out_count || !out_rows || !out_vals || !out_status || !out_kernel)
        return fail(idx, MI355DR_E_INVALID, "null argument");
    std::lock_guard<std::mutex> g(idx->mu);
    if (B <= 0 || B > kQBlockMax || n <= 0 || row0 < 0 || row0 % screen_tile(B) != 0 || row0 + n > idx->n || cap < 16 ||
        cap > kCandCapWide)
        return fail(idx, MI355DR_E_INVALID,
                    "debug_screen_hits: need 1<=B<=1024, n>=1, row0 a multiple of the tile (128; 256 if B>128), 16<=cap<=4096");
    for (int b = 0; b < B; ++b)
        if (!(thr[b] < INFINITY))
            return fail(idx, MI355DR_E_INVALID, "debug_screen_hits: thresholds must be finite or -inf");
    CHECK(upload_and_prep(idx, queries, B, 2));
    hipStream_t s = idx->stream;
    HIPCHECK(idx, hipMemcpyAsync(idx->st.thr, thr, (size_t)B * sizeof(float), hipMemcpyHostToDevice, s));
    const bool i8 = idle_i8(idx);
    *out_kernel = (int)screen_kernel_for(idx, i8, B, n, false);
    CHECK(launch_screen(idx, s, i8, B, row0, row0 + n, cap, 0, idx->screen_flush_sync ? 1 : -1));
    HIPCHECK(idx, hipMemcpyAsync(out_count, idx->st.cnt, (size_t)B * sizeof(int), hipMemcpyDeviceToHost, s));
    HIPCHECK(idx, hipMemcpyAsync(out_status, idx->st.status, (size_t)B * sizeof(int), hipMemcpyDeviceToHost, s));
    HIPCHECK(idx, hipMemcpyAsync(out_rows, idx->cand_row, (size_t)B * cap * sizeof(int32_t), hipMemcpyDeviceToHost, s));
    HIPCHECK(idx, hipMemcpyAsync(out_vals, idx->cand_val, (size_t)B * cap * sizeof(float), hipMemcpyDeviceToHost, s));
    std::vector<uint8_t> flag;
    if (i8) {
        flag.resize((size_t)n);
        HIPCHECK(idx, hipMemcpyAsync(flag.data(), idx->flag8 + row0, (size_t)n, hipMemcpyDeviceToHost, s));
    }
    HIPCHECK(idx, hipStreamSynchronize(s));
    if (!flag.empty())
        for (int b = 0; b < B; ++b) {
            const int c = std::min(std::max(out_count[b], 0), cap);
            for (int j = 0; j < c; ++j) {
                int32_t& r = out_rows[(size_t)b * cap + j];
                if (r >= row0 && r < row0 + n && flag[(size_t)(r - row0)]) r = -1 - r;
            }
        }
    return MI355DR_OK;
}

int mi355dr_debug_screen_bound(mi355dr_index* idx, const float* queries, int B, float* out_E) {
    if (!idx || !queries || !out_E) return fail(idx, MI355DR_E_INVALID, "null argument");
    std::lock_guard<std::mutex> g(idx->mu);
    if (B <= 0 || B > kQBlockMax) return fail(idx, MI355DR_E_INVALID, "need 1<=B<=1024");
    CHECK(upload_and_prep(idx, queries, B, idx->metric));
    hipStream_t s = idx->stream;
    HIPCHECK(idx, hipMemcpyAsync(out_E, idx->st.E, (size_t)B * sizeof(float), hipMemcpyDeviceToHost, s));
    HIPCHECK(idx, hipStreamSynchronize(s));
    return MI355DR_OK;
}

int mi355dr_debug_i8_state(mi355dr_index* idx, const float* queries, int B, float* out_sq, float* out_kq, int64_t g0,
                           int64_t n_groups, float* out_step, float* out_err) {
    if (!idx || !queries || !out_sq || !out_kq || !out_step || !out_err) return fail(idx, MI355DR_E_INVALID, "null argument");
    std::lock_guard<std::mutex> g(idx->mu);
    if (B <= 0 || B > kQBlockMax) return fail(idx, MI355DR_E_INVALID, "need 1<=B<=1024");
    if (g0 < 0 || n_groups < 0 || (g0 + n_groups) * kI8GroupRows > idx->cap_rows)
        return fail(idx, MI355DR_E_INVALID, "group range outside the index");
    if (!idle_i8(idx)) return fail(idx, MI355DR_E_UNSUPPORTED, "the int8 screen is not active");
    CHECK(upload_and_prep(idx, queries, B, idx->metric));
    hipStream_t s = idx->stream;
    HIPCHECK(idx, hipMemcpyAsync(out_sq, idx->st.sc, (size_t)B * sizeof(float), hipMemcpyDeviceToHost, s));
    HIPCHECK(idx, hipMemcpyAsync(out_kq, idx->st.kq, (size_t)B * sizeof(float), hipMemcpyDeviceToHost, s));
    std::vector<I8Group> gr((size_t)n_groups);
    if (n_groups > 0)
        HIPCHECK(idx, hipMemcpyAsync(gr.data(), idx->grp8 + g0, (size_t)n_groups * sizeof(I8Group), hipMemcpyDeviceToHost, s));
    HIPCHECK(idx, hipStreamSynchronize(s));
    for (int64_t i = 0; i < n_groups; ++i) {
        out_step[i] = gr[(size_t)i].step;
        out_err[i] = gr[(size_t)i].err;
    }
    return MI355DR_OK;
}

int mi355dr_debug_spec_model(mi355dr_index* idx, const float* queries, int B, int k, float* out_moments, float* out_thr_rigorous,
                             float* out_thr_used, double* out_zq, int64_t* out_sample_rows, int* out_slabs, int* out_i8) {
    if (!idx || !queries || !out_moments || !out_thr_rigorous || !out_thr_used || !out_zq || !out_sample_rows || !out_slabs ||
        !out_i8)
        return fail(idx, MI355DR_E_INVALID, "null argument");
    std::lock_guard<std::mutex> g(idx->mu);
    if (B <= 0 || B > kQBlockMax || k <= 0 || k > kKMax) return fail(idx, MI355DR_E_INVALID, "need 1<=B<=1024, 1<=k<=1024");
    HIPCHECK(idx, hipSetDevice(idx->device));
    CHECK(drain_pending(idx));
    CHECK(ensure_qstate(idx));
    const Pass ps = decide_pass(idx, k, 0, false, "screen path unavailable (metric or too many irregular rows)");
    if (ps.refused) return fail(idx, MI355DR_E_UNSUPPORTED, ps.refused);
    if (!ps.speculative) return fail(idx, MI355DR_E_UNSUPPORTED, "debug_spec_model: a pass at this k would not speculate");
    idx->last_pass_k = k;
    hipStream_t s = idx->stream;
    const PassPlan plan = make_plan(idx, ps, B);
    const SpecModel sm = spec_model(idx, ps, plan, out_zq);
    const int Bpad = (int)round_up(B, screen_tile(B));
    std::vector<unsigned long long> stat_before(2 * (size_t)kQBlockMax);
    const size_t stat_bytes = stat_before.size() * sizeof(unsigned long long);
    HIPCHECK(idx, hipMemcpyAsync(stat_before.data(), idx->stat_dev, stat_bytes, hipMemcpyDeviceToHost, s));
    HIPCHECK(idx, hipStreamSynchronize(s));
    const auto heads = [&]() -> int {
        for (int model = 0; model < 2; ++model) {
            HIPCHECK(idx, hipMemcpyAsync(idx->qdev, queries, (size_t)B * idx->dim * sizeof(float), hipMemcpyHostToDevice, s));
            CHECK(launch_prep(idx, s, B, Bpad, idx->metric, ps.i8, starter_count(plan)));
            CHECK(launch_screen(idx, s, ps.i8, B, 0, plan.sample, ps.cap, kEmitSlabMax, -1, model ? sm.slabs : 0));
            CHECK(launch_prune(idx, s, ps, B, nullptr, 0, true, true, false,
                               model ? &sm : nullptr));
            if (!model)
                HIPCHECK(idx, hipMemcpyAsync(out_thr_rigorous, idx->st.thr, (size_t)B * sizeof(float), hipMemcpyDeviceToHost, s));
        }
        HIPCHECK(idx, hipMemcpyAsync(out_thr_used, idx->st.thr_used, (size_t)B * sizeof(float), hipMemcpyDeviceToHost, s));
        HIPCHECK(idx, hipMemcpyAsync(out_moments, idx->spec_moments, (size_t)B * sm.slabs * 2 * sizeof(float), hipMemcpyDeviceToHost, s));
        return MI355DR_OK;
    };
    const int rc = heads();
    const hipError_t put_back = hipMemcpyAsync(idx->stat_dev, stat_before.data(), stat_bytes, hipMemcpyHostToDevice, s);
    const hipError_t done = hipStreamSynchronize(s);
    CHECK(rc);
    HIPCHECK(idx, put_back);
    HIPCHECK(idx, done);
    *out_sample_rows = plan.sample;
    *out_slabs = sm.slabs;
    *out_i8 = ps.i8 ? 1 : 0;
    return MI355DR_OK;
}

int mi355dr_debug_rescore(mi355dr_index* idx, const float* queries, int B, const int32_t* pair_q,
                          const int64_t* pair_row, int64_t n_pairs, float* out_dot, double* out_dist) {
    if (!idx || !queries || !pair_q || !pair_row || !out_dot || !out_dist)
        return fail(idx, MI355DR_E_INVALID, "null argument");
    std::lock_guard<std::mutex> g(idx->mu);
    if (B <= 0 || B > kQBlockMax || n_pairs <= 0) return fail(idx, MI355DR_E_INVALID, "bad shape");
    for (int64_t i = 0; i < n_pairs; ++i)
        if (pair_q[i] < 0 || pair_q[i] >= B || pair_row[i] < 0 || pair_row[i] >= idx->n)
            return fail(idx, MI355DR_E_INVALID, "pair out of range");
    PairBufs bufs;
    return rescore_host_pairs(idx, bufs, queries, B, pair_q, pair_row, n_pairs, out_dot, out_dist);
}


}
```

autorag_research_amd/index.py:

```python

from __future__ import annotations

import ctypes
from typing import NamedTuple

import numpy as np

from . import _native
from ._native import NativeError, check, f32c, ptr

METRICS = {"cosine": 0, "ip": 1}
PATHS = {"auto": 0, "screen": 1, "scan": 2}
SCREEN_DTYPES = {"auto": 0, "bf16": 1, "i8": 2}
FUSE_METHODS = {"rrf": 0, "mm": 1, "tmm": 2, "z": 3, "dbsf": 4}
FUSE_MODES = {"one_minus": 0, "negate": 1, "as_is": 2}


COLLAPSE_TRUNCATED = 1
COLLAPSE_FETCH_MULT = 1


class CollapsedLists(NamedTuple):

    vals: np.ndarray
# ... 1241 lines not shown
            self._h, ptr(z, ctypes.c_double), ptr(counts, ctypes.c_int32), z.shape[0], z.shape[1],
            ptr(comp, ctypes.c_double), int(n_steps), float(learning_rate), float(temperature), float(mixture_alpha),
            ptr(out, ctypes.c_double)))
        return out

    def set_option(self, key: str, value: int | str) -> None:
        if key == "path" and isinstance(value, str):
            value = PATHS[value]
        if key == "screen_dtype" and isinstance(value, str):
            value = SCREEN_DTYPES[value]
        check(self._h, self._lib.mi355dr_set_option(self._h, key.encode(), int(value)))

    def stat(self, key: str) -> int:
        out = ctypes.c_int64(0)
        check(self._h, self._lib.mi355dr_get_stat(self._h, key.encode(), ctypes.byref(out)))
        return int(out.value)

    def reset_stats(self) -> None:
        check(self._h, self._lib.mi355dr_reset_stats(self._h))

    def timer_start(self) -> None:
        check(self._h, self._lib.mi355dr_timer_start(self._h))

    def timer_stop(self) -> float:
        ms = ctypes.c_double(0.0)
        check(self._h, self._lib.mi355dr_timer_stop(self._h, ctypes.byref(ms)))
        return float(ms.value)

    def synchronize(self) -> None:
        check(self._h, self._lib.mi355dr_synchronize(self._h))

    def dev_alloc(self, nbytes: int) -> int:
        p = ctypes.c_void_p()
        check(self._h, self._lib.mi355dr_dev_alloc(self._h, int(nbytes), ctypes.byref(p)))
        return int(p.value)

    def dev_free(self, p: int) -> None:
        check(self._h, self._lib.mi355dr_dev_free(self._h, ctypes.c_void_p(int(p))))

    def dev_upload(self, dst: int, arr: np.ndarray) -> None:
        arr = np.ascontiguousarray(arr)
        check(self._h, self._lib.mi355dr_dev_upload(self._h, ctypes.c_void_p(int(dst)),
                                                    ctypes.c_void_p(arr.ctypes.data), arr.nbytes))

    def dev_download(self, src: int, arr: np.ndarray) -> None:
        assert arr.flags["C_CONTIGUOUS"]
        check(self._h, self._lib.mi355dr_dev_download(self._h, ctypes.c_void_p(arr.ctypes.data),
                                                      ctypes.c_void_p(int(src)), arr.nbytes))

    def debug_screen_dense(self, queries, row0: int, n: int) -> np.ndarray:
        q = f32c(queries)
        out = np.empty((q.shape[0], n), dtype=np.float32)
        check(self._h, self._lib.mi355dr_debug_screen_dense(self._h, ptr(q, ctypes.c_float), q.shape[0], int(row0),
                                                            int(n), ptr(out, ctypes.c_float)))
        return out

    def debug_screen_hits(self, queries, row0: int, n: int, thr, cap: int = 2048) -> dict:
        q = f32c(queries)
        B = q.shape[0]
        t = f32c(thr)
        if t.shape != (B,):
            raise ValueError("thr must hold one threshold per query")
        count = np.empty(B, dtype=np.int32)
        status = np.empty(B, dtype=np.int32)
        rows = np.empty((B, cap), dtype=np.int32)
        vals = np.empty((B, cap), dtype=np.float32)
        kernel = ctypes.c_int(-1)
        check(self._h, self._lib.mi355dr_debug_screen_hits(self._h, ptr(q, ctypes.c_float), B, int(row0), int(n),
                                                           ptr(t, ctypes.c_float), int(cap), ptr(count, ctypes.c_int),
                                                           ptr(rows, ctypes.c_int32), ptr(vals, ctypes.c_float),
                                                           ptr(status, ctypes.c_int), ctypes.byref(kernel)))
        held = np.arange(cap)[None, :] < np.minimum(count, cap)[:, None]
        flagged = held & (rows < 0)
        keep = held & ~flagged
        return {"kernel": int(kernel.value), "count": count, "status": status, "dropped": flagged.sum(axis=1),
                "q": np.nonzero(keep)[0].astype(np.int32), "row": rows[keep], "val": vals[keep]}

    MS_FORMS = ("none", "generic", "d128", "d128_packed", "wg", "wg_packed", "list_generic", "list_d128")

    def debug_maxsim_pass(self, qtok, q_offsets, k: int, doc_ids=None, list_cap: int = 8192) -> dict:
        qtok = f32c(qtok).reshape(-1, self.dim)
        q_offsets = np.ascontiguousarray(q_offsets, dtype=np.int32)
        B = q_offsets.shape[0] - 1
        ids = None if doc_ids is None else self._row_ids(doc_ids)
        n_docs = self.n_docs()
        live = np.full(max(B, 1), -1, dtype=np.int32)
        screen = np.empty((max(B, 1), max(n_docs, 1)), dtype=np.float32)
        two_e = np.empty(max(B, 1), dtype=np.float32)
        lists = np.full((3, max(B, 1), list_cap), -1, dtype=np.int32)
        ctl = np.zeros((3, max(B, 1), 2), dtype=np.int32)
        sd = np.full((max(B, 1), list_cap), np.nan, dtype=np.float32)
        form = np.zeros(8, dtype=np.int32)
        info = np.zeros(4, dtype=np.int32)
        check(self._h, self._lib.mi355dr_debug_maxsim_pass(
            self._h, ptr(qtok, ctypes.c_float), ptr(q_offsets, ctypes.c_int32), B, int(k),
            None if ids is None else ptr(ids, ctypes.c_int64), 0 if ids is None else ids.shape[0], int(list_cap),
            ptr(live, ctypes.c_int), ptr(screen, ctypes.c_float), ptr(two_e, ctypes.c_float), ptr(lists, ctypes.c_int32),
            ptr(ctl, ctypes.c_int), ptr(sd, ctypes.c_float), ptr(form, ctypes.c_int), ptr(info, ctypes.c_int)))
        n_live, cap = int(info[0]), int(info[1])
        out = {"live": live[:B], "two_e": two_e[:n_live],
               "screen": screen.reshape(-1)[:n_live * n_docs].reshape(n_live, n_docs),
               "form": {"family": self.MS_FORMS[int(form[0])], "ncb": int(form[1]), "waves": int(form[2]), "bps": int(form[3]),
                        "pipe": int(form[4]), "now": int(form[5]), "grid": int(form[6])},
               "cand_cap": cap, "tighten_max": int(info[3]), "lists": None}
        if info[2]:
            out["lists"] = {}
            for sec, name in enumerate(("wide", "starter", "final")):
                rows = []
                for r in range(n_live):
                    held = min(int(ctl[sec, r, 0]), cap, list_cap)
                    e = {"ids": lists[sec, r, :held].copy(), "count": int(ctl[sec, r, 0]), "overflow": int(ctl[sec, r, 1])}
                    if sec == 0:
                        e["sd"] = sd[r, :held].copy()
                    rows.append(e)
                out["lists"][name] = rows
        return out

    def debug_i8_state(self, queries, g0: int, n_groups: int) -> tuple[np.ndarray, np.ndarray, np.ndarray, np.ndarray]:
        q = f32c(queries)
        sq = np.empty(q.shape[0], dtype=np.float32)
        kq = np.empty(q.shape[0], dtype=np.float32)
        st = np.empty(n_groups, dtype=np.float32)
        er = np.empty(n_groups, dtype=np.float32)
        check(self._h, self._lib.mi355dr_debug_i8_state(self._h, ptr(q, ctypes.c_float), q.shape[0], ptr(sq, ctypes.c_float),
                                                        ptr(kq, ctypes.c_float), int(g0), int(n_groups),
                                                        ptr(st, ctypes.c_float), ptr(er, ctypes.c_float)))
        return sq, kq, st, er

    def debug_screen_bound(self, queries) -> np.ndarray:
        q = f32c(queries)
        out = np.empty(q.shape[0], dtype=np.float32)
        check(self._h, self._lib.mi355dr_debug_screen_bound(self._h, ptr(q, ctypes.c_float), q.shape[0],
                                                            ptr(out, ctypes.c_float)))
        return out

    def debug_spec_model(self, queries, k: int) -> dict:
        q = f32c(queries)
        B = q.shape[0]
        moments = np.empty((B, 256, 2), dtype=np.float32)
        rigorous = np.empty(B, dtype=np.float32)
        used = np.empty(B, dtype=np.float32)
        zq = ctypes.c_double(0.0)
        rows = ctypes.c_int64(0)
        slabs = ctypes.c_int(0)
        i8 = ctypes.c_int(0)
        check(self._h, self._lib.mi355dr_debug_spec_model(self._h, ptr(q, ctypes.c_float), B, int(k), ptr(moments, ctypes.c_float),
                                                          ptr(rigorous, ctypes.c_float), ptr(used, ctypes.c_float),
                                                          ctypes.byref(zq), ctypes.byref(rows), ctypes.byref(slabs),
                                                          ctypes.byref(i8)))
        n = int(slabs.value)
        return {"moments": moments.reshape(-1)[:B * n * 2].reshape(B, n, 2).copy(), "thr_rigorous": rigorous, "thr_used": used,
                "zq": float(zq.value), "sample_rows": int(rows.value), "i8": bool(i8.value)}

    def debug_rescore(self, queries, pair_q, pair_row) -> tuple[np.ndarray, np.ndarray]:
        q = f32c(queries)
        pq = np.ascontiguousarray(pair_q, dtype=np.int32)
        pr = np.ascontiguousarray(pair_row, dtype=np.int64)
        dot = np.empty(pq.shape[0], dtype=np.float32)
        dist = np.empty(pq.shape[0], dtype=np.float64)
        check(self._h, self._lib.mi355dr_debug_rescore(self._h, ptr(q, ctypes.c_float), q.shape[0],
                                                       ptr(pq, ctypes.c_int32), ptr(pr, ctypes.c_int64), pq.shape[0],
                                                       ptr(dot, ctypes.c_float), ptr(dist, ctypes.c_double)))
        return dot, dist
```

include/mi355dr.h:

```cpp
#ifndef MI355DR_H
#define MI355DR_H

#include <stddef.h>
#include <stdint.h>

#ifdef __cplusplus
extern "C" {
#endif

typedef struct mi355dr_index mi355dr_index;

enum {
    MI355DR_OK = 0,
    MI355DR_E_INVALID = -1,
    MI355DR_E_HIP = -2,
    MI355DR_E_NOMEM = -3,
    MI355DR_E_UNSUPPORTED = -4,
    MI355DR_E_INTERNAL = -5
};

enum { MI355DR_METRIC_COSINE = 0, MI355DR_METRIC_IP = 1 };

enum {
    MI355DR_PATH_AUTO = 0,
// ... 135 lines not shown
int mi355dr_search_bm25(mi355dr_index* idx, const int32_t* q_tokens, const int32_t* q_offsets , int B, int k, double k1,
                        double b, double* out_dist, int64_t* out_rows);
int mi355dr_search_bm25_device(mi355dr_index* idx, const int32_t* q_tokens, const int32_t* q_offsets, int B, int k, double k1,
                               double b, double* out_dist_dev, int64_t* out_rows_dev, void* stream);
int mi355dr_search_sparse_subset(mi355dr_index* idx, const int32_t* q_terms, const double* q_weights, const int32_t* q_offsets,
                                 int B, int k, double k1, double b, const int64_t* doc_ids , int64_t m,
                                 double* out_dist , int64_t* out_rows );
int mi355dr_search_sparse_subset_device(mi355dr_index* idx, const int32_t* q_terms, const double* q_weights, const int32_t* q_offsets,
                                        int B, int k, double k1, double b, const int64_t* doc_ids , int64_t m,
                                        double* out_dist_dev, int64_t* out_rows_dev, void* stream);
int mi355dr_search_bm25_subset(mi355dr_index* idx, const int32_t* q_tokens, const int32_t* q_offsets, int B, int k, double k1,
                               double b, const int64_t* doc_ids , int64_t m, double* out_dist, int64_t* out_rows);
int mi355dr_search_bm25_subset_device(mi355dr_index* idx, const int32_t* q_tokens, const int32_t* q_offsets, int B, int k, double k1,
                                      double b, const int64_t* doc_ids , int64_t m, double* out_dist_dev,
                                      int64_t* out_rows_dev, void* stream);
int mi355dr_score_sparse_subset(mi355dr_index* idx, const int32_t* q_terms, const double* q_weights, const int32_t* q_offsets,
                                int B, double k1, double b, const int64_t* doc_ids , int m,
                                double* out_dist );
int mi355dr_score_bm25_subset(mi355dr_index* idx, const int32_t* q_tokens, const int32_t* q_offsets, int B, double k1, double b,
                              const int64_t* doc_ids , int m, double* out_dist );

#define MI355DR_FUSE_RRF 0
#define MI355DR_FUSE_CC_MM 1
#define MI355DR_FUSE_CC_TMM 2
#define MI355DR_FUSE_CC_Z 3
#define MI355DR_FUSE_CC_DBSF 4
#define MI355DR_FUSE_ONE_MINUS 0
#define MI355DR_FUSE_NEGATE 1
#define MI355DR_FUSE_AS_IS 2
typedef struct {
    int method;
    int mode_1, mode_2;
    int rrf_k, fetch_k;
    double weight, min_1, min_2;
} mi355dr_fuse_opts;
int mi355dr_fuse_lists_device(mi355dr_index* idx, const double* vals1_dev, const int64_t* ids1_dev, int w1, const int64_t* map1_dev,
                              int64_t map1_len, const double* vals2_dev, const int64_t* ids2_dev, int w2, const int64_t* map2_dev,
                              int64_t map2_len, int B, int k_out, const mi355dr_fuse_opts* opts, double* out_vals_dev,
                              int64_t* out_ids_dev, int32_t* out_count_dev , void* stream);
int mi355dr_fuse_lists(mi355dr_index* idx, const double* vals1, const int64_t* ids1, int w1, const int64_t* map1, int64_t map1_len,
                       const double* vals2, const int64_t* ids2, int w2, const int64_t* map2, int64_t map2_len, int B, int k_out,
                       const mi355dr_fuse_opts* opts, double* out_vals, int64_t* out_ids, int32_t* out_count );

#define MI355DR_COLLAPSE_TRUNCATED 1
int mi355dr_collapse_lists_device(mi355dr_index* idx, const double* vals_dev, const int64_t* ids_dev, int w, int B,
                                  const int64_t* keys_dev , int64_t keys_len, int cap, int k_out,
                                  double* out_vals_dev, int64_t* out_ids_dev, int64_t* out_keys_dev ,
                                  int32_t* out_pos_dev , int32_t* out_count_dev ,
                                  int32_t* out_entries_dev , void* stream);
int mi355dr_collapse_lists(mi355dr_index* idx, const double* vals, const int64_t* ids, int w, int B, const int64_t* keys,
                           int64_t keys_len, int cap, int k_out, double* out_vals, int64_t* out_ids, int64_t* out_keys,
                           int32_t* out_pos, int32_t* out_count, int32_t* out_entries);
int mi355dr_search_collapsed(mi355dr_index* idx, const float* queries, int B, int k, int cap, const int64_t* keys ,
                             int64_t keys_len, int fetch_k, int max_fetch, double* out_dist, int64_t* out_rows,
                             int64_t* out_keys , int32_t* out_count ,
                             int32_t* out_state );
int mi355dr_search_collapsed_device(mi355dr_index* idx, const float* queries_dev, int B, int k, int cap, const int64_t* keys_dev,
                                    int64_t keys_len, int fetch_k, int max_fetch, double* out_dist_dev, int64_t* out_rows_dev,
                                    int64_t* out_keys_dev, int32_t* out_count_dev, int32_t* out_state_dev, void* stream);
int mi355dr_search_collapsed_sharded_device(mi355dr_index* idx, const float* queries_dev, int B, int k, int cap,
                                            const int64_t* keys_dev, int64_t keys_len, int fetch_k, int max_fetch,
                                            double* out_dist_dev, int64_t* out_rows_dev, int64_t* out_keys_dev,
                                            int32_t* out_count_dev, int32_t* out_state_dev, void* stream);

int mi355dr_gqr_refine(mi355dr_index* idx, const double* queries, int B, const int64_t* cand_rows, int P,
                       const double* comp_dist, int n_steps, double learning_rate, double temperature,
                       double mixture_alpha, double* out_scores);
int mi355dr_gqr_refine_maxsim(mi355dr_index* idx, const double* qtok, const int32_t* q_offsets, int B,
                              const int64_t* doc_ids, int P, const double* comp_dist, int n_steps, double learning_rate,
                              double temperature, double mixture_alpha, double* out_scores);
int mi355dr_gqr_refine_scores(mi355dr_index* idx, const double* primary_scores, const int32_t* counts, int B, int P,
                              const double* comp_dist, int n_steps, double learning_rate, double temperature,
                              double mixture_alpha, double* out_scores);

int mi355dr_merge_topk_device(mi355dr_index* idx, const double* dist_all_dev, const int64_t* rows_all_dev, int world,
                              int B, int k, double* out_dist_dev, int64_t* out_rows_dev, void* stream);

int mi355dr_pack_topk_device(mi355dr_index* idx, const double* dist_dev, const int64_t* rows_dev, int B, int k,
                             int64_t* packed_dev, void* stream);
int mi355dr_merge_topk_packed_device(mi355dr_index* idx, const int64_t* packed_all_dev, int world, int B, int k,
                                     double* out_dist_dev, int64_t* out_rows_dev, void* stream);

int mi355dr_comm_unique_id(void* out_128_bytes, size_t len);
int mi355dr_comm_init(mi355dr_index* idx, int rank, int world, const void* nccl_unique_id, size_t id_len);
int mi355dr_comm_world(const mi355dr_index* idx);
int mi355dr_comm_count(mi355dr_index* idx, int* out);
typedef int (*mi355dr_allgather_fn)(const void* send_dev, void* recv_dev, size_t bytes_per_rank, void* stream, void* user);
int mi355dr_comm_init_custom(mi355dr_index* idx, int rank, int world, mi355dr_allgather_fn fn, void* user);
int mi355dr_search_sharded_device(mi355dr_index* idx, const float* queries_dev, int B, int k, double* out_dist_dev,
                                  int64_t* out_rows_dev, void* stream);

int mi355dr_search_range_sharded_device(mi355dr_index* idx, const float* queries_dev, int B, const double* radius ,
                                        int max_results, double* out_dist_dev, int64_t* out_rows_dev, int64_t* out_count_dev,
                                        void* stream);
int mi355dr_search_rows_sharded_device(mi355dr_index* idx, const int64_t* row_ids , int B, int k, int flags,
                                       double* out_dist_dev, int64_t* out_rows_dev, void* stream);
int mi355dr_search_range_rows_sharded_device(mi355dr_index* idx, const int64_t* row_ids , int B,
                                             const double* radius , int max_results, int flags,
                                             double* out_dist_dev, int64_t* out_rows_dev, int64_t* out_count_dev, void* stream);
int mi355dr_search_mmr_sharded_device(mi355dr_index* idx, const float* queries_dev, int B, int k, int fetch_k, double lambda,
                                      double* out_dist_dev, int64_t* out_rows_dev, void* stream);
int mi355dr_mmr_select_sharded(mi355dr_index* idx, const float* queries, int B, int k, const int64_t* cand_rows ,
                               int m, double lambda, double* out_dist, int64_t* out_rows);

int mi355dr_search_sparse_sharded_device(mi355dr_index* idx, const int32_t* q_terms, const double* q_weights, const int32_t* q_offsets,
                                         int B, int k, double k1, double b, double* out_dist_dev, int64_t* out_rows_dev, void* stream);
int mi355dr_search_bm25_sharded_device(mi355dr_index* idx, const int32_t* q_tokens, const int32_t* q_offsets, int B, int k, double k1,
                                       double b, double* out_dist_dev, int64_t* out_rows_dev, void* stream);
int mi355dr_search_sparse_subset_sharded_device(mi355dr_index* idx, const int32_t* q_terms, const double* q_weights,
                                                const int32_t* q_offsets, int B, int k, double k1, double b,
                                                const int64_t* doc_ids , int64_t m, double* out_dist_dev,
                                                int64_t* out_rows_dev, void* stream);
int mi355dr_search_bm25_subset_sharded_device(mi355dr_index* idx, const int32_t* q_tokens, const int32_t* q_offsets, int B, int k,
                                              double k1, double b, const int64_t* doc_ids , int64_t m,
                                              double* out_dist_dev, int64_t* out_rows_dev, void* stream);
int mi355dr_score_sparse_subset_sharded(mi355dr_index* idx, const int32_t* q_terms, const double* q_weights, const int32_t* q_offsets,
                                        int B, double k1, double b, const int64_t* doc_ids , int m,
                                        double* out_dist );
int mi355dr_score_bm25_subset_sharded(mi355dr_index* idx, const int32_t* q_tokens, const int32_t* q_offsets, int B, double k1, double b,
                                      const int64_t* doc_ids , int m, double* out_dist );

int mi355dr_set_option(mi355dr_index* idx, const char* key, int64_t value);
int mi355dr_get_stat(mi355dr_index* idx, const char* key, int64_t* out);
int mi355dr_reset_stats(mi355dr_index* idx);
int mi355dr_timer_start(mi355dr_index* idx);
int mi355dr_timer_stop(mi355dr_index* idx, double* elapsed_ms);
int mi355dr_synchronize(mi355dr_index* idx);

int mi355dr_dev_alloc(mi355dr_index* idx, size_t bytes, void** out);
int mi355dr_dev_free(mi355dr_index* idx, void* p);
int mi355dr_dev_upload(mi355dr_index* idx, void* dst_dev, const void* src_host, size_t bytes);
int mi355dr_dev_download(mi355dr_index* idx, void* dst_host, const void* src_dev, size_t bytes);

int mi355dr_debug_screen_dense(mi355dr_index* idx, const float* queries, int B, int64_t row0, int64_t n, float* out_t);
int mi355dr_debug_screen_hits(mi355dr_index* idx, const float* queries, int B, int64_t row0, int64_t n, const float* thr,
                              int cap, int* out_count, int32_t* out_rows, float* out_vals, int* out_status, int* out_kernel);
#define MI355DR_MS_FORM_NONE 0
#define MI355DR_MS_FORM_GENERIC 1
#define MI355DR_MS_FORM_D128 2
#define MI355DR_MS_FORM_D128_PACKED 3
#define MI355DR_MS_FORM_WG 4
#define MI355DR_MS_FORM_WG_PACKED 5
#define MI355DR_MS_FORM_LIST_GENERIC 6
#define MI355DR_MS_FORM_LIST_D128 7
int mi355dr_debug_maxsim_pass(mi355dr_index* idx, const float* qtok, const int32_t* q_offsets, int B, int k, const int64_t* doc_ids,
                              int64_t m, int list_cap, int* out_live, float* out_screen, float* out_two_e, int32_t* out_lists,
                              int* out_ctl, float* out_wide_sd, int* out_form, int* out_info);
int mi355dr_debug_screen_bound(mi355dr_index* idx, const float* queries, int B, float* out_E);
int mi355dr_debug_i8_state(mi355dr_index* idx, const float* queries, int B, float* out_sq, float* out_kq, int64_t g0,
                           int64_t n_groups, float* out_step, float* out_err);
int mi355dr_debug_spec_m(int k);
int mi355dr_debug_spec_model(mi355dr_index* idx, const float* queries, int B, int k, float* out_moments, float* out_thr_rigorous,
                             float* out_thr_used, double* out_zq, int64_t* out_sample_rows, int* out_slabs, int* out_i8);
int mi355dr_debug_rescore(mi355dr_index* idx, const float* queries, int B, const int32_t* pair_q,
                          const int64_t* pair_row, int64_t n_pairs, float* out_dot, double* out_dist);

int mi355dr_diag_mfma_stream(int device, int format, double seconds, double* out_tops);

#ifdef __cplusplus
}
#endif
#endif
```

Measured before the change: 169,500.

## Derive speculative thresholds from stored sample covariance instead of scanning starter rows

Adds a cached covariance matrix and mean of the starter sample rows, built once on the device in bf16 and invalidated on updates or compaction. The speculative starter pass then computes each query's score mean and variance as q·mean and qᵀΣq with an MFMA kernel, instead of screening the sample rows and pruning them. The goal is to remove the per-batch screen and prune work on the sample. In exchange it costs a dpad² covariance build, extra device memory, and a bf16 approximation of the variance. A debug entry point is added to compare the two models.

```diff
diff --git a/autorag_research_amd/_native.py b/autorag_research_amd/_native.py
--- a/autorag_research_amd/_native.py
+++ b/autorag_research_amd/_native.py
@@ -40,7 +40,7 @@
     "mi355dr_dev_alloc", "mi355dr_dev_free", "mi355dr_dev_upload", "mi355dr_dev_download",
     "mi355dr_diag_mfma_stream",
     "mi355dr_debug_screen_dense", "mi355dr_debug_screen_hits", "mi355dr_debug_screen_bound", "mi355dr_debug_i8_state", "mi355dr_debug_rescore",
-    "mi355dr_debug_maxsim_pass", "mi355dr_debug_spec_m", "mi355dr_debug_spec_model",
+    "mi355dr_debug_maxsim_pass", "mi355dr_debug_spec_m", "mi355dr_debug_spec_model", "mi355dr_debug_spec_head",
 ]
 
 
@@ -327,6 +327,9 @@
     L.mi355dr_debug_spec_model.restype = c_int
     L.mi355dr_debug_spec_model.argtypes = [vp, f32p, c_int, c_int, f32p, f32p, f32p, ctypes.POINTER(ctypes.c_double),
                                            ctypes.POINTER(ctypes.c_int64), ctypes.POINTER(c_int), ctypes.POINTER(c_int)]
+    L.mi355dr_debug_spec_head.restype = c_int
+    L.mi355dr_debug_spec_head.argtypes = [vp, f32p, c_int, c_int, f32p, f32p, f32p, ctypes.POINTER(ctypes.c_double),
+                                          ctypes.POINTER(ctypes.c_int64), ctypes.POINTER(c_int)]
     L.mi355dr_debug_maxsim_pass.restype = c_int
     L.mi355dr_debug_maxsim_pass.argtypes = [vp, f32p, i32p, c_int, c_int, i64p, i64, c_int, ctypes.POINTER(c_int), f32p, f32p, i32p,
                                             ctypes.POINTER(c_int), f32p, ctypes.POINTER(c_int), ctypes.POINTER(c_int)]
diff --git a/autorag_research_amd/csrc/index.h b/autorag_research_amd/csrc/index.h
--- a/autorag_research_amd/csrc/index.h
+++ b/autorag_research_amd/csrc/index.h
@@ -83,6 +83,7 @@
     bool speculative = false;
     bool spec_eligible = false;
     int spec_m = 0;
+    bool spec_stored = false;
     const char* refused = nullptr;
 };
 struct Pending {
@@ -301,6 +302,12 @@
     int spec_shift_milli = 0;
     int spec_backoff = 0, spec_probation = 0;
     mi355::DevBuf<float> spec_moments;
+    int spec_head = -1;
+    mi355::DevBuf<uint16_t> spec_cov;
+    mi355::DevBuf<float> spec_mean;
+    mi355::DevBuf<float> spec_head_out;
+    int64_t spec_stored_rows = 0;
+    bool spec_stored_dirty = false;
     int i8_demoted_k = INT_MAX;
     double i8_min_budget = 0.25;
     mi355::RetryBufs retry[3];
@@ -360,6 +367,7 @@
     int rq_epoch = 0;
     int64_t s_rq_launches = 0;
     int64_t s_spec_passes = 0, s_spec_miss_queries = 0, s_spec_overflow_queries = 0;
+    int64_t s_spec_moment_builds = 0;
     int64_t s_retry_queries = 0;
     int64_t s_ms_screened = 0, s_ms_candidates = 0, s_ms_fallbacks = 0;
     int64_t s_ms_screen_ns = 0, s_ms_screen_launches = 0, s_ms_exact_ns = 0, s_ms_exact_launches = 0, s_ms_pack_ns = 0;
diff --git a/autorag_research_amd/csrc/k_spec_moments.h b/autorag_research_amd/csrc/k_spec_moments.h
--- /dev/null
+++ b/autorag_research_amd/csrc/k_spec_moments.h
@@ -0,0 +1,177 @@
+#pragma once
+#include "k_select.h"
+#include "screen_common.h"
+
+namespace mi355 {
+
+constexpr int kSpecHeadQ = 32;
+constexpr int kSpecHeadWaves = 8;
+constexpr int kSpecHeadDpadMax = 2048;
+__host__ __device__ inline int spec_head_ksteps(int dpad) { return (dpad / 64 + 3) / 4 * 4; }
+__host__ __device__ inline size_t spec_head_row_bytes(int dpad) { return (size_t)spec_head_ksteps(dpad) * 128 + 16; }
+__host__ __device__ inline size_t spec_head_lds_bytes(int dpad) {
+    return kSpecHeadQ * spec_head_row_bytes(dpad) + 2 * kSpecHeadWaves * kSpecHeadQ * sizeof(float);
+}
+
+__host__ __device__ inline int64_t spec_cov_index(int i, int j, int dpad) {
+    const int T = dpad / 64;
+    const int jb = i >> 5, row = i & 31, t = j >> 6, c = (j >> 3) & 7, e = j & 7;
+    return ((((int64_t)(jb * T + t) * 4 + (c >> 1)) * 64 + 32 * (c & 1) + row) << 3) + e;
+}
+
+constexpr int kSpecBuildTile = 32;
+constexpr int kSpecBuildRows = 64;
+
+__global__ __launch_bounds__(256) void k_spec_moments_build(const uint16_t* __restrict__ shadow, int dpad, int rows,
+                                                            uint16_t* __restrict__ cov, float* __restrict__ mean) {
+    __shared__ float A[kSpecBuildRows][kSpecBuildTile + 1];
+    __shared__ float Bt[kSpecBuildRows][kSpecBuildTile + 1];
+    const int i0 = blockIdx.y * kSpecBuildTile, j0 = blockIdx.x * kSpecBuildTile;
+    const int t = threadIdx.x, ti = t >> 4, tj = t & 15;
+    double acc[2][2] = {{0.0, 0.0}, {0.0, 0.0}}, sa[2] = {0.0, 0.0}, sb[2] = {0.0, 0.0};
+    for (int r0 = 0; r0 < rows; r0 += kSpecBuildRows) {
+        for (int e = t; e < kSpecBuildRows * kSpecBuildTile; e += 256) {
+            const int r = e >> 5, c = e & 31;
+            float x = 0.0f, y = 0.0f;
+            if (r0 + r < rows) {
+                x = bf16_bits_to_f32(shadow[(int64_t)(r0 + r) * dpad + i0 + c]);
+                y = bf16_bits_to_f32(shadow[(int64_t)(r0 + r) * dpad + j0 + c]);
+            }
+            A[r][c] = x == x ? x : 0.0f;
+            Bt[r][c] = y == y ? y : 0.0f;
+        }
+        __syncthreads();
+        for (int r = 0; r < kSpecBuildRows; ++r) {
+            const double a0 = A[r][2 * ti], a1 = A[r][2 * ti + 1], b0 = Bt[r][2 * tj], b1 = Bt[r][2 * tj + 1];
+            acc[0][0] = fma(a0, b0, acc[0][0]);
+            acc[0][1] = fma(a0, b1, acc[0][1]);
+            acc[1][0] = fma(a1, b0, acc[1][0]);
+            acc[1][1] = fma(a1, b1, acc[1][1]);
+            sa[0] += a0;
+            sa[1] += a1;
+            sb[0] += b0;
+            sb[1] += b1;
+        }
+        __syncthreads();
+    }
+    const double inv = 1.0 / (double)rows;
+#pragma unroll
+    for (int u = 0; u < 2; ++u) {
+#pragma unroll
+        for (int v = 0; v < 2; ++v) {
+            const double c = acc[u][v] * inv - (sa[u] * inv) * (sb[v] * inv);
+            cov[spec_cov_index(i0 + 2 * ti + u, j0 + 2 * tj + v, dpad)] = f32_to_bf16_rn((float)c);
+        }
+        if (blockIdx.x == 0 && tj == 0) mean[i0 + 2 * ti + u] = (float)(sa[u] * inv);
+    }
+}
+
+struct SpecHeadArgs {
+    QueryState st;
+    const uint16_t* cov;
+    const float* mean;
+    int B, dpad, metric;
+    float zq;
+    float* out_stats;
+};
+
+__global__ __launch_bounds__(64 * kSpecHeadWaves) void k_spec_head(SpecHeadArgs a) {
+    extern __shared__ __attribute__((aligned(16))) char smem[];
+    const int tid = threadIdx.x;
+    const int lane = tid & 63;
+    const int wave = __builtin_amdgcn_readfirstlane(tid >> 6);
+    const int q0 = blockIdx.x * kSpecHeadQ;
+    const int rb = (int)spec_head_row_bytes(a.dpad);
+    float* part = (float*)(smem + kSpecHeadQ * rb);
+    {
+        const int pieces = spec_head_ksteps(a.dpad) * 8;
+        for (int e = tid; e < kSpecHeadQ * pieces; e += 64 * kSpecHeadWaves) {
+            const int r = e / pieces, c = e - r * pieces;
+            uint4 v = make_uint4(0u, 0u, 0u, 0u);
+            if (c * 8 < a.dpad) v = *(const uint4*)(a.st.qhat + (int64_t)(q0 + r) * a.dpad + c * 8);
+            *(uint4*)(smem + r * rb + c * 16) = v;
+        }
+    }
+    __syncthreads();
+    const int T = a.dpad / kStepK;
+    const int G = spec_head_ksteps(a.dpad) / 4;
+    const int row = lane & 31, g = lane >> 5;
+    const char* qrow = smem + row * rb;
+    float e2 = 0.0f, mu = 0.0f;
+    for (int jb = wave; jb < a.dpad / 32; jb += kSpecHeadWaves) {
+        const char* cblk = (const char*)a.cov + ((int64_t)jb * T * 4 * 64 + lane) * 16;
+        f32x16 acc;
+#pragma unroll
+        for (int r = 0; r < 16; ++r) acc[r] = 0.0f;
+        bf16x8 f0[16], f1[16];
+        auto load = [&](bf16x8(&f)[16], int gi) {
+            gi = min(gi, G - 1);
+#pragma unroll
+            for (int u = 0; u < 4; ++u) {
+                const int t = min(gi * 4 + u, T - 1);
+#pragma unroll
+                for (int kk = 0; kk < 4; ++kk) f[u * 4 + kk] = *(const bf16x8*)(cblk + (t * 4 + kk) * 1024);
+            }
+        };
+        auto mma = [&](const bf16x8(&f)[16], int gi) {
+#pragma unroll
+            for (int u = 0; u < 4; ++u)
+#pragma unroll
+                for (int kk = 0; kk < 4; ++kk) {
+                    const bf16x8 fb = *(const bf16x8*)(qrow + (gi * 4 + u) * kRowB + ((2 * kk + g) << 4));
+                    acc = __builtin_amdgcn_mfma_f32_32x32x16_bf16(f[u * 4 + kk], fb, acc, 0, 0, 0);
+                }
+        };
+        load(f0, 0);
+        for (int gi = 0; gi < G; gi += 2) {
+            load(f1, gi + 1);
+            __builtin_amdgcn_sched_barrier(0);
+            mma(f0, gi);
+            __builtin_amdgcn_sched_barrier(0);
+            load(f0, gi + 2);
+            __builtin_amdgcn_sched_barrier(0);
+            if (gi + 1 < G) mma(f1, gi + 1);
+            __builtin_amdgcn_sched_barrier(0);
+        }
+#pragma unroll
+        for (int r = 0; r < 16; ++r) {
+            const int j = jb * 32 + (r & 3) + 8 * (r >> 2) + 4 * g;
+            const float qv = bf16_bits_to_f32(*(const uint16_t*)(qrow + j * 2));
+            e2 = __builtin_fmaf(acc[r], qv, e2);
+            mu = __builtin_fmaf(qv, a.mean[j], mu);
+        }
+    }
+    e2 += __shfl_xor(e2, 32, kWave);
+    mu += __shfl_xor(mu, 32, kWave);
+    if (lane < 32) {
+        part[wave * kSpecHeadQ + lane] = e2;
+        part[(kSpecHeadWaves + wave) * kSpecHeadQ + lane] = mu;
+    }
+    __syncthreads();
+    const int q = q0 + lane;
+    if (wave != 0 || lane >= kSpecHeadQ || q >= a.B) return;
+    float var_f = 0.0f, mean_f = 0.0f;
+#pragma unroll
+    for (int w = 0; w < kSpecHeadWaves; ++w) {
+        var_f += part[w * kSpecHeadQ + lane];
+        mean_f += part[(kSpecHeadWaves + w) * kSpecHeadQ + lane];
+    }
+    const double sd = sqrt(var_f > 0.0f ? (double)var_f : 0.0);
+    if (a.out_stats) {
+        a.out_stats[2 * q] = mean_f;
+        a.out_stats[2 * q + 1] = (float)sd;
+    }
+    if (a.st.status[q] & kStIrregular) return;
+    const float t_model = (float)((double)mean_f + sd * (double)a.zq);
+    const float nq = a.st.qn[q];
+    float thr = __builtin_inff();
+    if (fabsf(t_model) < __builtin_inff()) {
+        const double dist_t = a.metric == 0 ? 1.0 - (double)t_model : -(double)t_model * sqrt((double)nq);
+        const float thr_model = screen_threshold(a.metric, dist_t, a.st.E[q], nq);
+        if (fabsf(thr_model) < __builtin_inff()) thr = thr_model;
+    }
+    a.st.thr[q] = thr;
+    a.st.thr_used[q] = thr;
+}
+
+}
diff --git a/autorag_research_amd/csrc/mi355dr.hip b/autorag_research_amd/csrc/mi355dr.hip
--- a/autorag_research_amd/csrc/mi355dr.hip
+++ b/autorag_research_amd/csrc/mi355dr.hip
@@ -12,6 +12,7 @@
 inline bool screen_rq_has(int ksteps) { return ksteps >= 1 && ksteps <= 6; }
 #include "k_screen_stream.h"
 #include "k_select.h"
+#include "k_spec_moments.h"
 #include "k_prune_wide.h"
 #include "k_update.h"
 #include "k_compact.h"
@@ -173,6 +174,9 @@
     HIPCHECK(idx, hipFuncSetAttribute((const void*)k_screen_rq<6, false, true>, hipFuncAttributeMaxDynamicSharedMemorySize, rq_lds(6)));
     HIPCHECK(idx, hipFuncSetAttribute((const void*)k_merge_topk, hipFuncAttributeMaxDynamicSharedMemorySize,
                                       kSortMax * 12));
+    if (idx->dpad <= kSpecHeadDpadMax)
+        HIPCHECK(idx, hipFuncSetAttribute((const void*)k_spec_head, hipFuncAttributeMaxDynamicSharedMemorySize,
+                                          (int)spec_head_lds_bytes(idx->dpad)));
     if (mmr_lds_bytes(idx->dim, kMmrMax) > 160 * 1024)
         return fail(idx, MI355DR_E_UNSUPPORTED, "dim too large for the select kernels' LDS budget");
     HIPCHECK(idx, hipFuncSetAttribute((const void*)k_mmr_select, hipFuncAttributeMaxDynamicSharedMemorySize,
@@ -234,6 +238,7 @@
 }
 
 inline bool i8_available(const mi355dr_index* idx) { return idx->irr8_n <= kIrrCap; }
+constexpr int kSpecHeadDpadAuto = 2048;
 constexpr int kStarterKMax = 32;
 constexpr int64_t kStarterRows = 16384;
 static_assert(kStarterRows / kSlabRows <= kSpecSlabsMax, "the moment scratch holds one entry per slab of the starter's sample");
@@ -266,6 +271,7 @@
                        kSpecInflation * ps.spec_m * 4 <= 3 * (std::min(kPruneSmallSort, ps.cap) - k) &&
                        starter_sample_rows(idx, ps) > 0;
     ps.speculative = ps.spec_eligible && idx->spec_probation <= 0;
+    ps.spec_stored = ps.speculative && idx->spec_head != 0 && idx->dpad <= (idx->spec_head > 0 ? kSpecHeadDpadMax : kSpecHeadDpadAuto);
     return ps;
 }
 inline bool idle_i8(const mi355dr_index* idx) { return decide_pass(idx, idx->last_pass_k, 0, false).i8; }
@@ -436,6 +442,7 @@
     int64_t sample = 0;
     std::vector<int64_t> ends;
     bool emit_all_first = false;
+    bool stored_head = false;
 };
 PassPlan plan_pass(const mi355dr_index* idx, const Pass& ps, int B, double growth) {
     PassPlan p;
@@ -449,6 +456,7 @@
         p.sample = starter_rows;
         seen = p.sample;
         if (ps.speculative) {
+            p.stored_head = ps.spec_stored;
             p.ends.push_back(n);
             return p;
         }
@@ -490,7 +498,7 @@
     return p;
 }
 
-inline int starter_count(const PassPlan& p) { return (int)((p.sample + kSlabRows - 1) / kSlabRows); }
+inline int starter_count(const PassPlan& p) { return p.stored_head ? 0 : (int)((p.sample + kSlabRows - 1) / kSlabRows); }
 
 inline double normal_quantile(double p) {
     double lo = -40.0, hi = 40.0;
@@ -511,6 +519,36 @@
     sm.zq = (float)zq;
     if (zq_out) *zq_out = zq;
     return sm;
+}
+
+int ensure_spec_stored(mi355dr_index* idx, hipStream_t s, int64_t sample, bool count) {
+    if (idx->spec_cov && !idx->spec_stored_dirty && idx->spec_stored_rows == sample) return MI355DR_OK;
+    HIPCHECK(idx, idx->spec_cov.grow((size_t)idx->dpad * idx->dpad * sizeof(uint16_t)));
+    HIPCHECK(idx, idx->spec_mean.grow((size_t)idx->dpad * sizeof(float)));
+    const unsigned tiles = (unsigned)(idx->dpad / kSpecBuildTile);
+    hipLaunchKernelGGL(k_spec_moments_build, dim3(tiles, tiles), dim3(256), 0, s, idx->shadow.p, idx->dpad, (int)sample,
+                       idx->spec_cov.p, idx->spec_mean.p);
+    HIPCHECK(idx, hipGetLastError());
+    idx->spec_stored_rows = sample;
+    idx->spec_stored_dirty = false;
+    if (count) idx->s_spec_moment_builds++;
+    return MI355DR_OK;
+}
+
+int launch_spec_head(mi355dr_index* idx, hipStream_t s, int B, const SpecModel& sm, float* out_stats = nullptr) {
+    SpecHeadArgs ha{};
+    ha.st = idx->st;
+    ha.cov = idx->spec_cov;
+    ha.mean = idx->spec_mean;
+    ha.B = B;
+    ha.dpad = idx->dpad;
+    ha.metric = idx->metric;
+    ha.zq = sm.zq;
+    ha.out_stats = out_stats;
+    hipLaunchKernelGGL(k_spec_head, dim3((unsigned)((B + kSpecHeadQ - 1) / kSpecHeadQ)), dim3(64 * kSpecHeadWaves),
+                       spec_head_lds_bytes(idx->dpad), s, ha);
+    HIPCHECK(idx, hipGetLastError());
+    return MI355DR_OK;
 }
 
 PassPlan make_plan(const mi355dr_index* idx, const Pass& ps, int B) {
@@ -555,11 +593,15 @@
             sm = spec_model(idx, ps, plan);
             idx->s_spec_passes++;
         }
-        CHECK(timed(false, plan.sample, [&] {
-            return launch_screen(idx, s, i8, B, 0, plan.sample, ps.cap, kEmitSlabMax, -1, ps.speculative ? sm.slabs : 0);
-        }));
-        CHECK(launch_prune(idx, s, ps, B, nullptr, 0, true, true, false,
-                           ps.speculative ? &sm : nullptr));
+        if (plan.stored_head) {
+            CHECK(launch_spec_head(idx, s, B, sm));
+        } else {
+            CHECK(timed(false, plan.sample, [&] {
+                return launch_screen(idx, s, i8, B, 0, plan.sample, ps.cap, kEmitSlabMax, -1, ps.speculative ? sm.slabs : 0);
+            }));
+            CHECK(launch_prune(idx, s, ps, B, nullptr, 0, true, true, false,
+                               ps.speculative ? &sm : nullptr));
+        }
         idx->s_starters++;
     }
     int64_t done = 0;
@@ -716,6 +758,7 @@
         HIPCHECK(idx, hipMemcpyAsync(idx->qdev, q_dev, (size_t)B * idx->dim * sizeof(float), hipMemcpyDeviceToDevice, s));
     PassPlan plan;
     if (ps.screening) plan = make_plan(idx, ps, B);
+    if (plan.stored_head) CHECK(ensure_spec_stored(idx, s, plan.sample, true));
     CHECK(launch_prep(idx, s, B, Bpad, idx->metric, ps.i8, starter_count(plan)));
     if (idx->n > 0) {
         if (ps.screening) {
@@ -1139,6 +1182,7 @@
         if (groups.empty() || groups.back() != r / kI8GroupRows) groups.push_back(r / kI8GroupRows);
     HIPCHECK(idx, hipSetDevice(idx->device));
     CHECK(drain_pending(idx));
+    if (sorted.front() < idx->spec_stored_rows) idx->spec_stored_dirty = true;
     hipStream_t s = idx->stream;
     DevBuf<void> ids_dev, groups_dev, stage;
     HIPCHECK(idx, ids_dev.grow((size_t)n * sizeof(int64_t)));
@@ -1262,6 +1306,7 @@
     idx->i8_demoted_k = INT_MAX;
     idx->i8_backoff = idx->i8_probation = 0;
     idx->spec_backoff = idx->spec_probation = 0;
+    idx->spec_stored_dirty = true;
     idx->s_compactions += n_moved > 0;
     idx->s_compact_moved_rows += n_moved;
     if (new_of_old) {
@@ -3086,6 +3131,7 @@
     {"prune_companion", {&Index::prune_companion, kSwitch}},
     {"speculate", {&Index::speculate, kSwitch}, INT64_MIN, INT64_MAX, [](Index* x) { x->spec_backoff = x->spec_probation = 0; }},
     {"spec_min_rows", &Index::spec_min_rows, 0},
+    {"spec_head", &Index::spec_head, -1, 1},
     {"spec_shift_milli", &Index::spec_shift_milli, -20000, 20000},
     {"scan_dma", {&Index::scan_dma, kSwitch}},
     {"defer_round_b", {&Index::defer_round_b, kSwitch}},
@@ -3139,6 +3185,7 @@
     {"spec_passes", &Index::s_spec_passes, true},
     {"spec_miss_queries", &Index::s_spec_miss_queries, true},
     {"spec_overflow_queries", &Index::s_spec_overflow_queries, true},
+    {"spec_moment_builds", &Index::s_spec_moment_builds, true},
     {"spec_suspended", nullptr, false, [](const Index* x) -> int64_t { return x->spec_probation > 0 ? 1 : 0; }},
     {"maxsim_screened", &Index::s_ms_screened, true},
     {"maxsim_candidates", &Index::s_ms_candidates, true},
@@ -3228,7 +3275,8 @@
          return x->cap_rows * ((int64_t)x->dim * 4 + (int64_t)x->dpad * 2 + (int64_t)x->dpad8 + 5) +
                 x->cap_rows / kI8GroupRows * (int64_t)sizeof(I8Group) + multivec_bytes(x) +
                 (int64_t)(x->view_row_map.bytes + x->view_doc_map.bytes) +
-                sparse_bytes(x) + (int64_t)x->clp.bytes();
+                sparse_bytes(x) + (int64_t)x->clp.bytes() +
+                (int64_t)(x->spec_cov.bytes + x->spec_mean.bytes);
      }},
 };
 }
@@ -3461,9 +3509,10 @@
     HIPCHECK(idx, hipSetDevice(idx->device));
     CHECK(drain_pending(idx));
     CHECK(ensure_qstate(idx));
-    const Pass ps = decide_pass(idx, k, 0, false, "screen path unavailable (metric or too many irregular rows)");
+    Pass ps = decide_pass(idx, k, 0, false, "screen path unavailable (metric or too many irregular rows)");
     if (ps.refused) return fail(idx, MI355DR_E_UNSUPPORTED, ps.refused);
     if (!ps.speculative) return fail(idx, MI355DR_E_UNSUPPORTED, "debug_spec_model: a pass at this k would not speculate");
+    ps.spec_stored = false;
     idx->last_pass_k = k;
     hipStream_t s = idx->stream;
     const PassPlan plan = make_plan(idx, ps, B);
@@ -3499,6 +3548,73 @@
     return MI355DR_OK;
 }
 
+int mi355dr_debug_spec_head(mi355dr_index* idx, const float* queries, int B, int k, float* out_mean, float* out_sd,
+                            float* out_thr_used, double* out_zq, int64_t* out_sample_rows, int* out_stored) {
+    if (!idx || !queries || !out_mean || !out_sd || !out_thr_used || !out_zq || !out_sample_rows || !out_stored)
+        return fail(idx, MI355DR_E_INVALID, "null argument");
+    std::lock_guard<std::mutex> g(idx->mu);
+    if (B <= 0 || B > kQBlockMax || k <= 0 || k > kKMax) return fail(idx, MI355DR_E_INVALID, "need 1<=B<=1024, 1<=k<=1024");
+    HIPCHECK(idx, hipSetDevice(idx->device));
+    CHECK(drain_pending(idx));
+    CHECK(ensure_qstate(idx));
+    const Pass ps = decide_pass(idx, k, 0, false, "screen path unavailable (metric or too many irregular rows)");
+    if (ps.refused) return fail(idx, MI355DR_E_UNSUPPORTED, ps.refused);
+    if (!ps.speculative) return fail(idx, MI355DR_E_UNSUPPORTED, "debug_spec_head: a pass at this k would not speculate");
+    idx->last_pass_k = k;
+    hipStream_t s = idx->stream;
+    const PassPlan plan = make_plan(idx, ps, B);
+    const SpecModel sm = spec_model(idx, ps, plan, out_zq);
+    const int Bpad = (int)round_up(B, screen_tile(B));
+    *out_sample_rows = plan.sample;
+    *out_stored = plan.stored_head ? 1 : 0;
+    HIPCHECK(idx, hipMemcpyAsync(idx->qdev, queries, (size_t)B * idx->dim * sizeof(float), hipMemcpyHostToDevice, s));
+    if (plan.stored_head) {
+        std::vector<float> stats(2 * (size_t)B);
+        HIPCHECK(idx, idx->spec_head_out.grow(2 * (size_t)kQBlockMax * sizeof(float)));
+        CHECK(ensure_spec_stored(idx, s, plan.sample, false));
+        CHECK(launch_prep(idx, s, B, Bpad, idx->metric, ps.i8, 0));
+        CHECK(launch_spec_head(idx, s, B, sm, idx->spec_head_out));
+        HIPCHECK(idx, hipMemcpyAsync(stats.data(), idx->spec_head_out, stats.size() * sizeof(float), hipMemcpyDeviceToHost, s));
+        HIPCHECK(idx, hipMemcpyAsync(out_thr_used, idx->st.thr_used, (size_t)B * sizeof(float), hipMemcpyDeviceToHost, s));
+        HIPCHECK(idx, hipStreamSynchronize(s));
+        for (int b = 0; b < B; ++b) {
+            out_mean[b] = stats[2 * (size_t)b];
+            out_sd[b] = stats[2 * (size_t)b + 1];
+        }
+        return MI355DR_OK;
+    }
+    std::vector<unsigned long long> stat_before(2 * (size_t)kQBlockMax);
+    const size_t stat_bytes = stat_before.size() * sizeof(unsigned long long);
+    std::vector<float> moments((size_t)B * sm.slabs * 2);
+    HIPCHECK(idx, hipMemcpyAsync(stat_before.data(), idx->stat_dev, stat_bytes, hipMemcpyDeviceToHost, s));
+    HIPCHECK(idx, hipStreamSynchronize(s));
+    const auto head = [&]() -> int {
+        CHECK(launch_prep(idx, s, B, Bpad, idx->metric, ps.i8, starter_count(plan)));
+        CHECK(launch_screen(idx, s, ps.i8, B, 0, plan.sample, ps.cap, kEmitSlabMax, -1, sm.slabs));
+        CHECK(launch_prune(idx, s, ps, B, nullptr, 0, true, true, false, &sm));
+        HIPCHECK(idx, hipMemcpyAsync(out_thr_used, idx->st.thr_used, (size_t)B * sizeof(float), hipMemcpyDeviceToHost, s));
+        HIPCHECK(idx, hipMemcpyAsync(moments.data(), idx->spec_moments, moments.size() * sizeof(float), hipMemcpyDeviceToHost, s));
+        return MI355DR_OK;
+    };
+    const int rc = head();
+    const hipError_t put_back = hipMemcpyAsync(idx->stat_dev, stat_before.data(), stat_bytes, hipMemcpyHostToDevice, s);
+    const hipError_t done = hipStreamSynchronize(s);
+    CHECK(rc);
+    HIPCHECK(idx, put_back);
+    HIPCHECK(idx, done);
+    for (int b = 0; b < B; ++b) {
+        double s1 = 0.0, s2 = 0.0;
+        for (int i = 0; i < sm.slabs; ++i) {
+            s1 += (double)moments[((size_t)b * sm.slabs + i) * 2];
+            s2 += (double)moments[((size_t)b * sm.slabs + i) * 2 + 1];
+        }
+        const double mean = s1 / (double)sm.rows, var = s2 / (double)sm.rows - mean * mean;
+        out_mean[b] = (float)mean;
+        out_sd[b] = (float)std::sqrt(var > 0.0 ? var : 0.0);
+    }
+    return MI355DR_OK;
+}
+
 int mi355dr_debug_rescore(mi355dr_index* idx, const float* queries, int B, const int32_t* pair_q,
                           const int64_t* pair_row, int64_t n_pairs, float* out_dot, double* out_dist) {
     if (!idx || !queries || !pair_q || !pair_row || !out_dot || !out_dist)
diff --git a/autorag_research_amd/index.py b/autorag_research_amd/index.py
--- a/autorag_research_amd/index.py
+++ b/autorag_research_amd/index.py
@@ -1417,6 +1417,21 @@
         return {"moments": moments.reshape(-1)[:B * n * 2].reshape(B, n, 2).copy(), "thr_rigorous": rigorous, "thr_used": used,
                 "zq": float(zq.value), "sample_rows": int(rows.value), "i8": bool(i8.value)}
 
+    def debug_spec_head(self, queries, k: int) -> dict:
+        q = f32c(queries)
+        B = q.shape[0]
+        mean = np.empty(B, dtype=np.float32)
+        sd = np.empty(B, dtype=np.float32)
+        used = np.empty(B, dtype=np.float32)
+        zq = ctypes.c_double(0.0)
+        rows = ctypes.c_int64(0)
+        stored = ctypes.c_int(0)
+        check(self._h, self._lib.mi355dr_debug_spec_head(self._h, ptr(q, ctypes.c_float), B, int(k), ptr(mean, ctypes.c_float),
+                                                         ptr(sd, ctypes.c_float), ptr(used, ctypes.c_float), ctypes.byref(zq),
+                                                         ctypes.byref(rows), ctypes.byref(stored)))
+        return {"mean": mean, "sd": sd, "thr_used": used, "zq": float(zq.value), "sample_rows": int(rows.value),
+                "stored": bool(stored.value)}
+
     def debug_rescore(self, queries, pair_q, pair_row) -> tuple[np.ndarray, np.ndarray]:
         q = f32c(queries)
         pq = np.ascontiguousarray(pair_q, dtype=np.int32)
diff --git a/include/mi355dr.h b/include/mi355dr.h
--- a/include/mi355dr.h
+++ b/include/mi355dr.h
@@ -311,6 +311,8 @@
 int mi355dr_debug_spec_m(int k);
 int mi355dr_debug_spec_model(mi355dr_index* idx, const float* queries, int B, int k, float* out_moments, float* out_thr_rigorous,
                              float* out_thr_used, double* out_zq, int64_t* out_sample_rows, int* out_slabs, int* out_i8);
+int mi355dr_debug_spec_head(mi355dr_index* idx, const float* queries, int B, int k, float* out_mean, float* out_sd,
+                            float* out_thr_used, double* out_zq, int64_t* out_sample_rows, int* out_stored);
 int mi355dr_debug_rescore(mi355dr_index* idx, const float* queries, int B, const int32_t* pair_q,
                           const int64_t* pair_row, int64_t n_pairs, float* out_dot, double* out_dist);
 
```

Result: no change. 170,800, median of 6 (+0.8%).
